# fnothaft/adam

Hardware: AMD Instinct MI355X
Metric: BQSR bases/sec (observe+apply) at 1/2/4/8 MI355X; % HBM roofline (higher is better)
Workload: dtype u8 in, int64 counts, f64 recalibration; 1 GPU; cfg2: synthetic 10M x 100 bp reads, 1 read group, no known sites (per GPU); reads_per_gpu=10000000, bases_per_gpu=1000000000, reads_total=10000000, read_groups=1, known_sites=0, parallelism=dp1: read shards per GPU, RCCL int64 table all-reduce

## Files before the change

### adam_amd/_capi.py

```python
from __future__ import annotations

import ctypes
import os
import threading

_HERE = os.path.dirname(os.path.abspath(__file__))
LIB_PATH = os.environ.get("ADAM_BQSR_LIB") or os.path.join(_HERE, "libadam_bqsr.so")

BQSR_OK = 0
STAGE_RESET, STAGE_KERNEL, STAGE_FOLD, STAGE_PREP, STAGE_LUT, STAGE_NO_LUT = 1, 2, 4, 8, 16, 32
STATUS_NAMES = ["OK", "NULL_RG", "MD_PARSE", "CIGAR_SHORT", "BAD_REVCOMP_BASE", "EMPTY_TABLE", "MISSING_KEY",
                "QUAL_RANGE", "NULL_FIELD", "SEQ_SHORT", "CIGAR_INVALID", "INVALID_ARG", "DEVICE", "UNSUPPORTED",
                "SAM_PARSE", "PILEUP", "ATTRIBUTE"]
(NULL_RG, MD_PARSE, CIGAR_SHORT, BAD_REVCOMP_BASE, EMPTY_TABLE, MISSING_KEY, QUAL_RANGE, NULL_FIELD, SEQ_SHORT,
 CIGAR_INVALID, INVALID_ARG, DEVICE, UNSUPPORTED, SAM_PARSE, PILEUP, ATTRIBUTE) = range(1, 17)
MPILEUP_STATUS_NAMES = ["UNSORTED", "REFERENCE_CONFLICT"]
UNSORTED, REFERENCE_CONFLICT = 17, 18

EXPORTS = [
    "bqsr_abi_version", "bqsr_last_error", "bqsr_last_error_read", "bqsr_status_name", "bqsr_context_create",
    "bqsr_context_destroy", "bqsr_context_tune", "bqsr_sites_create", "bqsr_sites_destroy", "bqsr_batch_create", "bqsr_batch_destroy",
    "bqsr_batch_reads", "bqsr_batch_bases", "bqsr_batch_dims", "bqsr_batch_relayout", "bqsr_batch_layout_times", "bqsr_batch_wrap_device", "bqsr_table_words",
    "bqsr_table_create", "bqsr_table_destroy", "bqsr_table_dims", "bqsr_table_device_ptr", "bqsr_table_download",
    "bqsr_table_upload", "bqsr_observe", "bqsr_observe_records", "bqsr_table_merge", "bqsr_finalize",
    "bqsr_lut_destroy", "bqsr_lut_stats", "bqsr_lut_shifts", "bqsr_apply", "bqsr_apply_records",
    "bqsr_stage_records", "bqsr_staged_destroy", "bqsr_staged_bytes", "bqsr_staged_reads", "bqsr_staged_bases",
    "bqsr_batch_create_staged", "bqsr_batch_upload_async", "bqsr_em_fold_async", "bqsr_batch_em_copy_async",
    "bqsr_finalize_device", "bqsr_observe_stage", "bqsr_apply_stage", "bqsr_job_reset_async", "bqsr_job_result", "bqsr_copy_async",
    "bqsr_job_errors_export_async", "bqsr_job_errors_import_async", "bqsr_job_status_async", "bqsr_job_status_get",
    "bqsr_copy_dyn_async", "bqsr_compact_outputs_async", "bqsr_batch_exception_count_ptr",
    "bqsr_batch_fold_stats",
    "bqsr_sort_order", "bqsr_sam_sort",
    "bqsr_sam_flagstat", "bqsr_flagstat_arrow", "bqsr_flagstat_arrow_device",
    "bqsr_bgzf_inflate", "bqsr_sam_bam_form", "bqsr_sam_markdup_path",
    "bqsr_sam_pileup_prepare", "bqsr_sam_pileup_columns", "bqsr_arrow_pileup_prepare", "bqsr_arrow_pileup_columns",
    "bqsr_pileup_kernel_times",
    "bqsr_sam_mpileup_prepare", "bqsr_sam_mpileup_text", "bqsr_arrow_mpileup_prepare", "bqsr_arrow_mpileup_text",
    "bqsr_mpileup_kernel_times",
    "bqsr_sam_realign_targets_prepare", "bqsr_sam_realign_targets_fetch", "bqsr_arrow_realign_targets_prepare",
    "bqsr_arrow_realign_targets_fetch", "bqsr_realign_targets_kernel_times",
    "bqsr_pileup_agg_create", "bqsr_pileup_agg_destroy", "bqsr_pileup_agg_add_host", "bqsr_sam_pileup_agg_add",
    "bqsr_arrow_pileup_agg_add", "bqsr_pileup_agg_run", "bqsr_pileup_agg_fetch", "bqsr_pileup_agg_kernel_times",
    "bqsr_sam_bam_prepare", "bqsr_sam_bam_records", "bqsr_sam_bam_header", "bqsr_bgzf_compress",
    "bqsr_bam_kernel_times",
    "bqsr_bgzf_deflate", "bqsr_bgzf_deflate_host", "bqsr_sam_bam_members", "bqsr_deflate_code_lengths",
    "bqsr_bgzf_deflate_times",
    "bqsr_compare_create", "bqsr_compare_destroy", "bqsr_compare_check_terms", "bqsr_compare_sam", "bqsr_compare_sides",
    "bqsr_compare_values", "bqsr_compare_baseqs", "bqsr_compare_rows", "bqsr_compare_kernel_times",
    "bqsr_sam_tag_counts", "bqsr_arrow_tag_counts", "bqsr_sam_tag_values", "bqsr_arrow_tag_values",
    "bqsr_tag_values_fetch", "bqsr_tags_kernel_times",
]


class NativeLibraryMissing(RuntimeError):
    pass


class BQSRError(RuntimeError):

    def __init__(self, status: int, message: str = "", read: int = -1):
        names = STATUS_NAMES + MPILEUP_STATUS_NAMES
        name = names[status] if 0 <= status < len(names) else str(status)
        super().__init__("%s: %s" % (name, message))
        self.status = status
        self.name = name
        self.read = read


class Dims(ctypes.Structure):
    _fields_ = [("n_rg", ctypes.c_int32), ("max_len", ctypes.c_int32)]


class FinalStats(ctypes.Structure):
    _fields_ = [("average_reported_error", ctypes.c_double), ("global_error", ctypes.c_double),
                ("global_obs", ctypes.c_int64), ("global_mm", ctypes.c_int64), ("n_groups", ctypes.c_int32)]


class FoldStats(ctypes.Structure):
    _fields_ = [("n_tiles", ctypes.c_int64), ("stream_used", ctypes.c_int64), ("stream_cap", ctypes.c_int64),
                ("lds_stream", ctypes.c_int64), ("n_blocks", ctypes.c_int32), ("reads_per_tile", ctypes.c_int32),
                ("cand_blocks", ctypes.c_int32), ("nobase_blocks", ctypes.c_int32),
                ("nobase_between", ctypes.c_int32), ("tileless_blocks", ctypes.c_int32),
                ("longest_run", ctypes.c_int32), ("capped_blocks", ctypes.c_int32),
                ("segs_total", ctypes.c_int32), ("segs_run", ctypes.c_int32), ("segs_event", ctypes.c_int32),
                ("segs_global", ctypes.c_int32), ("segs_refused", ctypes.c_int32), ("lds_segs", ctypes.c_int32)]


class DeviceReads(ctypes.Structure):
    _fields_ = [("n_reads", ctypes.c_int64), ("n_slots", ctypes.c_int64), ("meta", ctypes.c_void_p),
                ("align", ctypes.c_void_p), ("qual", ctypes.c_void_p), ("bases", ctypes.c_void_p),
                ("cigar", ctypes.c_void_p), ("md", ctypes.c_void_p), ("dims", Dims),
                ("slots_aligned", ctypes.c_int32)]


vp, i32, i64, dbl = ctypes.c_void_p, ctypes.c_int32, ctypes.c_int64, ctypes.c_double
pp, i64p, dblp = ctypes.POINTER(vp), ctypes.POINTER(i64), ctypes.POINTER(dbl)

_lib = None
_lock = threading.Lock()


def lib():
    global _lib
    if _lib is not None:
        return _lib
    with _lock:
        if _lib is not None:
            return _lib
        if not os.path.exists(LIB_PATH):
            raise NativeLibraryMissing("%s is not built; run __graft_entry__.build()" % LIB_PATH)
        try:
            import torch
            if torch.cuda.is_available():
                torch.cuda.init()
        except ImportError:
            pass
        L = ctypes.CDLL(LIB_PATH)
        sig = {
            "bqsr_abi_version": (ctypes.c_int, []),
            "bqsr_last_error": (ctypes.c_char_p, []),
            "bqsr_last_error_read": (i64, []),
            "bqsr_status_name": (ctypes.c_char_p, [ctypes.c_int]),
            "bqsr_context_create": (ctypes.c_int, [ctypes.c_int, pp]),
            "bqsr_context_destroy": (None, [vp]),
            "bqsr_context_tune": (ctypes.c_int, [vp, ctypes.c_int, i64]),
            "bqsr_batch_relayout": (ctypes.c_int, [vp, vp, ctypes.POINTER(dbl)]),
            "bqsr_batch_layout_times": (ctypes.c_int, [vp, ctypes.POINTER(dbl), ctypes.POINTER(dbl)]),
            "bqsr_sites_create": (ctypes.c_int, [vp, vp, vp, vp, i32, pp]),
            "bqsr_sites_destroy": (None, [vp]),
            "bqsr_batch_create": (ctypes.c_int, [vp, vp, vp, pp]),
            "bqsr_batch_destroy": (None, [vp]),
            "bqsr_batch_reads": (i64, [vp]),
            "bqsr_batch_bases": (i64, [vp]),
            "bqsr_batch_slots": (i64, [vp]),
            "bqsr_batch_dims": (Dims, [vp]),
            "bqsr_batch_wrap_device": (ctypes.c_int, [vp, ctypes.POINTER(DeviceReads), pp]),
            "bqsr_stage_records": (ctypes.c_int, [vp, vp, pp]),
            "bqsr_staged_destroy": (None, [vp]),
            "bqsr_staged_bytes": (i64, [vp]),
            "bqsr_staged_reads": (i64, [vp]),
            "bqsr_staged_bases": (i64, [vp]),
            "bqsr_batch_create_staged": (ctypes.c_int, [vp, vp, pp]),
            "bqsr_batch_upload_async": (ctypes.c_int, [vp, vp, vp]),
            "bqsr_batch_set_window": (ctypes.c_int, [vp, i32, i32]),
            "bqsr_batch_reads_per_tile": (i32, [vp]),
            "bqsr_batch_fold_stats": (ctypes.c_int, [vp, ctypes.POINTER(FoldStats), vp]),
            "bqsr_table_words": (i64, [Dims]),
            "bqsr_table_create": (ctypes.c_int, [vp, Dims, vp, pp]),
            "bqsr_table_destroy": (None, [vp]),
            "bqsr_table_dims": (Dims, [vp]),
            "bqsr_table_device_ptr": (vp, [vp]),
            "bqsr_table_download": (ctypes.c_int, [vp, vp]),
            "bqsr_table_upload": (ctypes.c_int, [vp, vp]),
            "bqsr_observe": (ctypes.c_int, [vp, vp, vp, vp, ctypes.POINTER(dbl), vp]),
            "bqsr_observe_async": (ctypes.c_int, [vp, vp, vp, vp, vp]),
            "bqsr_observe_result": (ctypes.c_int, [vp, ctypes.POINTER(dbl), vp]),
            "bqsr_observe_stage": (ctypes.c_int, [vp, vp, vp, vp, i32, vp]),
            "bqsr_table_zero_async": (ctypes.c_int, [vp, vp]),
            "bqsr_batch_em_device_ptr": (vp, [vp]),
            "bqsr_apply_stage": (ctypes.c_int, [vp, vp, vp, vp, vp, vp, vp, i64, i32, vp]),
            "bqsr_observe_records": (ctypes.c_int, [vp, vp, vp, Dims, pp, ctypes.POINTER(dbl)]),
            "bqsr_table_merge": (ctypes.c_int, [vp, vp, ctypes.POINTER(dbl), dbl]),
            "bqsr_finalize": (ctypes.c_int, [vp, vp, dbl, pp]),
            "bqsr_finalize_async": (ctypes.c_int, [vp, vp, dbl, pp, vp]),
            "bqsr_finalize_result": (ctypes.c_int, [vp, vp]),
            "bqsr_finalize_device": (ctypes.c_int, [vp, vp, vp, pp, vp]),
            "bqsr_batch_em_copy_async": (ctypes.c_int, [vp, vp, vp]),
            "bqsr_em_fold_async": (ctypes.c_int, [vp, vp, i64, vp, vp]),
            "bqsr_lut_destroy": (None, [vp]),
            "bqsr_lut_stats": (ctypes.c_int, [vp, ctypes.POINTER(FinalStats)]),
            "bqsr_lut_group": (ctypes.c_int, [vp, i32, ctypes.POINTER(i64), ctypes.POINTER(i64)]),
            "bqsr_lut_shifts": (ctypes.c_int, [vp, i32, i32, i32, i32, vp, ctypes.POINTER(i32)]),
            "bqsr_phred_threshold_table": (i32, [vp, i32, ctypes.POINTER(i32)]),
            "bqsr_apply": (ctypes.c_int, [vp, vp, vp, vp, vp, vp, vp, i64, ctypes.POINTER(i64), vp]),
            "bqsr_apply_async": (ctypes.c_int, [vp, vp, vp, vp, vp, vp, vp, i64, vp]),
            "bqsr_apply_result": (ctypes.c_int, [vp, ctypes.POINTER(i64), vp]),
            "bqsr_apply_records": (ctypes.c_int, [vp, vp, vp, vp, vp]),
            "bqsr_job_reset_async": (ctypes.c_int, [vp, vp, vp]),
            "bqsr_job_result": (ctypes.c_int, [vp, vp, ctypes.POINTER(dbl), ctypes.POINTER(i64), vp]),
            "bqsr_copy_async": (ctypes.c_int, [vp, vp, vp, i64, vp]),
            "bqsr_copy_dyn_async": (ctypes.c_int, [vp, vp, vp, vp, i32, i64, i64, vp]),
            "bqsr_compact_outputs_async": (ctypes.c_int, [vp, vp, vp, vp, vp, vp, i64, vp, vp, vp, vp]),
            "bqsr_batch_exception_count_ptr": (vp, [vp]),
            "bqsr_job_errors_export_async": (ctypes.c_int, [vp, i64, vp, vp]),
            "bqsr_job_errors_import_async": (ctypes.c_int, [vp, vp, vp]),
            "bqsr_job_status_async": (ctypes.c_int, [vp, vp, i32, vp]),
            "bqsr_job_status_get": (ctypes.c_int, [vp, i32, i32, ctypes.POINTER(dbl), ctypes.POINTER(i64)]),
        }
        _lib = bind(L, sig)
    return _lib


def bind(L, sig):
    done = L.__dict__.setdefault("_sig_tables", {})
    if id(sig) not in done:
        for name, (res, args) in sig.items():
            f = getattr(L, name)
            f.restype = res
            f.argtypes = args
        done[id(sig)] = sig
    return L


def check(status: int):
    if status != BQSR_OK:
        L = lib()
        raise BQSRError(status, L.bqsr_last_error().decode(), L.bqsr_last_error_read())


def stage_times(fn, names, handle=None, array=False):
    v = (ctypes.c_double * len(names))()
    lead = [] if handle is None else [handle]
    at = ctypes.addressof(v)
    out = [v] if array else [ctypes.cast(at + 8 * i, ctypes.POINTER(ctypes.c_double)) for i in range(len(names))]
    check(fn(*(lead + out)))
    return dict(zip(names, v))
```

### adam_amd/bqsr.py

```python
from __future__ import annotations

import contextlib
import ctypes
from typing import Dict, Iterable, List, Optional, Sequence, Tuple

import numpy as np

from . import _capi
from ._capi import BQSRError, Dims, check, lib
from .records import (F_DUPLICATE, F_HAS_MD, F_MAPPED, F_PRIMARY, ADAMRecord, RecordBatch)

MAX_REASONABLE_QSCORE = 60


class Context:

    _by_device: Dict[int, "Context"] = {}

    def __init__(self, device: int = 0):
        h = ctypes.c_void_p()
        check(lib().bqsr_context_create(device, ctypes.byref(h)))
        self.handle = h
        self.device = device

    @classmethod
    def get(cls, device: int = 0) -> "Context":
        if device not in cls._by_device:
            cls._by_device[device] = Context(device)
        return cls._by_device[device]

    _KNOBS = {"order": 1, "fronts": 2, "key_major": 3, "bgzf": 5, "flagstat_grid": 6, "pileup_grid": 7}
    _DEFAULTS = {"order": -1, "fronts": -1, "key_major": 0, "bgzf": 1, "flagstat_grid": 0, "pileup_grid": 0}

    def tune(self, **knobs) -> Dict[str, int]:
        cur = getattr(self, "_tuned", dict(self._DEFAULTS))
        prev = {}
        for k, v in knobs.items():
            if v is None:
                continue
            if isinstance(v, str):
                v = {"auto": -1, "read": 0, "group": 1}[v]
            check(lib().bqsr_context_tune(self.handle, self._KNOBS[k], int(v)))
            prev[k] = cur[k]
            cur[k] = int(v)
        self._tuned = cur
        return prev

    @contextlib.contextmanager
    def tuned(self, **knobs):
        prev = self.tune(**knobs)
        try:
            yield self
        finally:
            self.tune(**prev)


class SnpTable:

    def __init__(self, table: Optional[Dict[str, Iterable[int]]] = None):
        self.table = {k: np.unique(np.asarray(list(v), dtype=np.int64)) for k, v in (table or {}).items()}
        self._handles: Dict[int, ctypes.c_void_p] = {}

    @property
    def contigs(self) -> List[str]:
        return list(self.table.keys())

    @staticmethod
    def from_vcf(path: str) -> "SnpTable":
        t: Dict[str, List[int]] = {}
        with open(path, "r", encoding="latin-1") as fh:
            for line in fh:
                line = line.rstrip("\n")
                if line.startswith("#"):
                    continue
                f = line.split("\t")
                t.setdefault(f[0], []).append(int(f[1]))
        return SnpTable(t)

    def handle(self, ctx: Context):
        if ctx.device not in self._handles:
            names = [c.encode() for c in self.contigs]
            arrs = [np.ascontiguousarray(self.table[c]) for c in self.contigs]
            n = len(arrs)
            cnames = (ctypes.c_char_p * max(1, n))(*names)
            cpos = (ctypes.c_void_p * max(1, n))(*[a.ctypes.data for a in arrs])
            cn = np.asarray([len(a) for a in arrs] or [0], dtype=np.uint64)
            h = ctypes.c_void_p()
            check(lib().bqsr_sites_create(ctx.handle, ctypes.cast(cnames, ctypes.c_void_p),
                                          ctypes.cast(cpos, ctypes.c_void_p), cn.ctypes.data, n, ctypes.byref(h)))
            self._handles[ctx.device] = h
        return self._handles[ctx.device]

    def __del__(self):
        L = _capi._lib
        if L is not None:
            for h in getattr(self, "_handles", {}).values():
                L.bqsr_sites_destroy(h)


def dims_of(batches: Sequence[RecordBatch]) -> Dims:
    n_rg = max([b.n_rg() for b in batches] or [1])
    max_len = max([b.max_len() for b in batches] or [1])
    return Dims(n_rg, max_len)


class ErrorCount:

    def __init__(self, bases_observed: int = 0, mismatches: int = 0):
        self.bases_observed = int(bases_observed)
        self.mismatches = int(mismatches)

    def __add__(self, other: "ErrorCount") -> "ErrorCount":
        return ErrorCount(self.bases_observed + other.bases_observed, self.mismatches + other.mismatches)

    def get_error_prob(self) -> Optional[float]:
        if self.bases_observed == 0:
            return None
        return max(10.0 ** (-60 / 10.0), self.mismatches / self.bases_observed)

    def __repr__(self):
        return "ErrorCount(%d, %d)" % (self.bases_observed, self.mismatches)


class RecalTable:

    def __init__(self, dims: Dims, ctx: Optional[Context] = None, expected_mismatch: float = 0.0):
        self.ctx = ctx or Context.get()
        self.dims = Dims(dims.n_rg, dims.max_len)
        h = ctypes.c_void_p()
        check(lib().bqsr_table_create(self.ctx.handle, self.dims, None, ctypes.byref(h)))
        self.handle = h
        self.expected_mismatch = float(expected_mismatch)

    def __del__(self):
        L = _capi._lib
        if L is not None and getattr(self, "handle", None):
            L.bqsr_table_destroy(self.handle)
            self.handle = None

    @property
    def K(self) -> int:
        return 60 * (self.dims.n_rg - 1) + 128

    @property
    def C(self) -> int:
        return 2 * self.dims.max_len + 1

    @property
    def cells(self) -> int:
        return self.C + 21

    def words(self) -> np.ndarray:
        w = np.zeros(lib().bqsr_table_words(self.dims), dtype=np.int64)
        check(lib().bqsr_table_download(self.handle, w.ctypes.data))
        return w

    def set_words(self, w: np.ndarray):
        w = np.ascontiguousarray(w, dtype=np.int64)
        check(lib().bqsr_table_upload(self.handle, w.ctypes.data))

    def counts(self) -> Tuple[np.ndarray, np.ndarray, np.ndarray]:
        w = self.words()
        K, cells = self.K, self.cells
        return w[:K], w[K:K + K * cells].reshape(K, cells), w[K + K * cells:].reshape(K, cells)

    def merge(self, other: "RecalTable") -> "RecalTable":
        out = RecalTable(self.dims, self.ctx)
        out.set_words(self.words())
        em = ctypes.c_double(self.expected_mismatch)
        check(lib().bqsr_table_merge(out.handle, other.handle, ctypes.byref(em), other.expected_mismatch))
        out.expected_mismatch = em.value
        return out

    def merge_into(self, other: "RecalTable"):
        em = ctypes.c_double(self.expected_mismatch)
        check(lib().bqsr_table_merge(self.handle, other.handle, ctypes.byref(em), other.expected_mismatch))
        self.expected_mismatch = em.value

    def finalize_table(self) -> "FinalizedTable":
        return FinalizedTable(self)


class FinalizedTable:

    def __init__(self, table: RecalTable):
        self.table = table
        h = ctypes.c_void_p()
        check(lib().bqsr_finalize(table.ctx.handle, table.handle, table.expected_mismatch, ctypes.byref(h)))
        self.handle = h
        st = _capi.FinalStats()
        check(lib().bqsr_lut_stats(h, ctypes.byref(st)))
        self.average_reported_error = st.average_reported_error
        self.global_error = st.global_error
        self.global_counts = ErrorCount(st.global_obs, st.global_mm)

    def __del__(self):
        L = _capi._lib
        if L is not None and getattr(self, "handle", None):
            L.bqsr_lut_destroy(self.handle)
            self.handle = None

    def read_group_counts(self, r: int) -> Optional[ErrorCount]:
        o, m = ctypes.c_int64(), ctypes.c_int64()
        k = lib().bqsr_lut_group(self.handle, r, ctypes.byref(o), ctypes.byref(m))
        if k < 0:
            check(_capi.DEVICE)
        return ErrorCount(o.value, m.value) if k == 1 else None

    def get_error_rate_shifts(self, qual_by_rg: int, qual: int, cycle: int, context: int):
        sh = np.zeros(4, dtype=np.float64)
        q = ctypes.c_int32()
        check(lib().bqsr_lut_shifts(self.handle, qual_by_rg, qual, cycle, context, sh.ctypes.data, ctypes.byref(q)))
        return sh, q.value

    def get_read_group_delta(self, qual_by_rg: int) -> float:
        num = qual_by_rg - 1
        r = num // MAX_REASONABLE_QSCORE if num >= 0 else -((-num) // MAX_REASONABLE_QSCORE)
        ec = self.read_group_counts(r)
        if ec is None:
            raise BQSRError(_capi.MISSING_KEY, "read group %d" % r)
        p = ec.get_error_prob()
        avg = self.average_reported_error
        return (p if p is not None else avg) - avg


class Partition:

    def __init__(self, batch: RecordBatch, chars: np.ndarray, out_len: np.ndarray):
        self.batch = batch
        self.chars = chars
        self.out_len = out_len

    def qual(self, r: int) -> str:
        o = int(self.batch.qual_offset[r])
        return "".join(map(chr, self.chars[o:o + int(self.out_len[r])]))

    def records(self) -> List[ADAMRecord]:
        recs = self.batch.to_records()
        for r, rec in enumerate(recs):
            if rec.qual is not None or self.out_len[r]:
                rec.qual = self.qual(r)
        return recs


class RecalibrateBaseQualities:

    def __init__(self, ctx: Optional[Context] = None, dims: Optional[Dims] = None):
        self.ctx = ctx or Context.get()
        self.dims = dims

    @staticmethod
    def usable_read(rec: ADAMRecord) -> bool:
        return rec.read_mapped and rec.primary_alignment and not rec.duplicate_read and \
            rec.mismatching_positions is not None

    @classmethod
    def apply(cls, partitions: Sequence[RecordBatch], dbsnp: Optional[SnpTable] = None,
              ctx: Optional[Context] = None) -> List[Partition]:
        parts = list(partitions)
        rbq = cls(ctx, dims_of(parts))
        table = rbq.compute_table(parts, dbsnp or SnpTable())
        return rbq.apply_table(table, parts)

    def _records(self, batch: RecordBatch, dbsnp: Optional[SnpTable]):
        return batch.c_struct(batch.contig_ids_for(dbsnp.contigs if dbsnp else None))

    def compute_table(self, partitions: Sequence[RecordBatch], dbsnp: SnpTable) -> RecalTable:
        dims = self.dims or dims_of(partitions)
        acc = RecalTable(dims, self.ctx)
        sites = dbsnp.handle(self.ctx) if dbsnp is not None else None
        for batch in partitions:
            s, keep = self._records(batch, dbsnp)
            h = ctypes.c_void_p()
            em = ctypes.c_double(0.0)
            check(lib().bqsr_observe_records(self.ctx.handle, ctypes.byref(s), sites, dims, ctypes.byref(h),
                                             ctypes.byref(em)))
            part = RecalTable.__new__(RecalTable)
            part.ctx, part.dims, part.handle, part.expected_mismatch = self.ctx, dims, h, em.value
            acc.merge_into(part)
        return acc

    def apply_table(self, table: RecalTable, partitions: Sequence[RecordBatch]) -> List[Partition]:
        fin = table.finalize_table()
        out = []
        for batch in partitions:
            s, keep = self._records(batch, None)
            chars = np.zeros(max(1, int(batch.qual_offset[-1])), dtype=np.uint16)
            out_len = np.zeros(max(1, batch.n_reads), dtype=np.uint32)
            check(lib().bqsr_apply_records(self.ctx.handle, ctypes.byref(s), fin.handle, chars.ctypes.data,
                                           out_len.ctypes.data))
            out.append(Partition(batch, chars, out_len))
        return out


def adam_bqsr(partitions: Sequence[RecordBatch], dbsnp: Optional[SnpTable] = None,
              ctx: Optional[Context] = None) -> List[Partition]:
    return RecalibrateBaseQualities.apply(partitions, dbsnp, ctx)
```

### adam_amd/csrc/bqsr_capi.cpp

```cpp
#include <hip/hip_runtime.h>

#include <algorithm>
#include <array>
#include <atomic>
#include <chrono>
#include <cmath>
#include <cstdio>
#include <cstdlib>
#include <cstring>
#include <dlfcn.h>
#include <memory>
#include <mutex>
#include <new>
#include <string>
#include <thread>
#include <vector>

#include <rocprim/rocprim.hpp>

#include "bqsr_internal.h"

using namespace bqsr;

#include "bqsr_kernels.hip"
#include "bqsr_observe_lean.hip"
#include "bqsr_fold.hip"
#include "bqsr_transport.hip"


namespace {
thread_local std::string g_err;
thread_local int64_t g_err_read = -1;

bqsr_status fail(bqsr_status s, const std::string& msg, int64_t read = -1) {
  g_err = msg;
  g_err_read = read;
  return s;
}
bqsr_status ok() {
  g_err.clear();
  g_err_read = -1;
  return BQSR_OK;
}

#define HIP_TRY(expr)                                                                          \
  do {                                                                                         \
    hipError_t e_ = (expr);                                                                    \
    if (e_ != hipSuccess)                                                                      \
      return fail(BQSR_ERR_DEVICE, std::string(#expr " failed: ") + hipGetErrorString(e_));    \
  } while (0)

hipStream_t S(void* s) { return s ? (hipStream_t)s : hipStreamPerThread; }

const char* kStatusNames[] = {"OK",          "NULL_RG",      "MD_PARSE",       "CIGAR_SHORT", "BAD_REVCOMP_BASE",
                              "EMPTY_TABLE", "MISSING_KEY",  "QUAL_RANGE",     "NULL_FIELD",  "SEQ_SHORT",
                              "CIGAR_INVALID", "INVALID_ARG", "DEVICE",        "UNSUPPORTED", "SAM_PARSE",
                              "PILEUP",      "ATTRIBUTE",    "UNSORTED",       "REFERENCE_CONFLICT"};

bqsr_status from_err_key(unsigned long long k, int64_t read_base) {
  if (k == kNoError) return ok();
  const int code = (int)(k & 0xF);
  const int64_t read = (int64_t)(k >> 28) + read_base;
  const uint32_t o = (uint32_t)((k >> 8) & 0xFFFFF);
  char buf[160];
  snprintf(buf, sizeof buf, "%s at read %lld, read offset %u", kStatusNames[code], (long long)read, o);
  return fail((bqsr_status)code, buf, read);
}


struct Pow10 {
  double v[256];
  Pow10() {
    for (int p = 0; p < 256; ++p) v[p] = std::pow(10.0, (double)(-p) / 10.0);
  }
};
const Pow10& pow10tab() {
  static Pow10 t;
  return t;
}

double cr_log10(double x) { return (double)log10l((long double)x); }
int32_t java_d2i(double d) {
  if (std::isnan(d)) return 0;
  if (d >= 2147483647.0) return INT32_MAX;
  if (d <= -2147483648.0) return INT32_MIN;
  return (int32_t)d;
}
int32_t phred_of(double p) { return java_d2i(-10.0 * cr_log10(p)); }

struct PhredThresholds {
  std::vector<double> thr;
  PhredThresholds() {
    thr.resize(kThrN);
    const uint64_t lo_bits = 1, hi_bits = 0x7FEFFFFFFFFFFFFFull;
    auto val = [](uint64_t b) {
      double d;
      memcpy(&d, &b, 8);
      return d;
    };
    for (int i = 0; i < kThrN; ++i) {
      const int n = kThrQmin + i;
      if (phred_of(val(hi_bits)) >= n) {
        thr[i] = val(hi_bits);
        continue;
      }
      if (phred_of(val(lo_bits)) < n) {
        thr[i] = 0.0;
        continue;
      }
      uint64_t a = lo_bits, b = hi_bits;
      while (b - a > 1) {
        const uint64_t m = a + (b - a) / 2;
        if (phred_of(val(m)) >= n) a = m; else b = m;
      }
      thr[i] = val(a);
    }
  }
};
const PhredThresholds& thresholds() {
  static PhredThresholds t;
  return t;
}

struct PhredBuckets {
  std::vector<double> thr;
  std::vector<int16_t> q;
  PhredBuckets() {
    thr.resize(kQbN);
    q.resize(kQbN);
    const auto& T = thresholds().thr;
    for (int i = 0; i < kQbN; ++i) {
      const int e = kQbElo + (i >> kQbBits), m = i & ((1 << kQbBits) - 1);
      const double lo = std::ldexp(1.0 + (double)m / (1 << kQbBits), e);
      const double hi = std::ldexp(1.0 + (double)(m + 1) / (1 << kQbBits), e);
      const double last = std::nextafter(hi, 0.0);
      const int qhi = phred_of(lo), qlo = phred_of(last);
      if (qhi - qlo > 1 || qhi - kThrQmin < 0 || qhi - kThrQmin >= kThrN || qhi > 32767 || qhi < -32767) {
        q[(size_t)i] = -32768;
        thr[(size_t)i] = 0.0;
      } else {
        q[(size_t)i] = (int16_t)qhi;
        thr[(size_t)i] = T[(size_t)(qhi - kThrQmin)];
      }
    }
  }
};
const PhredBuckets& buckets() {
  static PhredBuckets b;
  return b;
}

int64_t table_words(const bqsr_dims& d) {
  const int64_t K = 60LL * (d.n_rg - 1) + 128, cells = 2LL * d.max_len + 1 + kCtxSlots;
  return K + 2 * K * cells;
}
TableGeom geom(const bqsr_dims& d) {
  TableGeom g;
  g.K = 60 * (d.n_rg - 1) + 128;
  g.L = d.max_len;
  g.C = 2 * d.max_len + 1;
  g.cells = g.C + kCtxSlots;
  return g;
}

constexpr size_t kLdsMax = 163840;
size_t observe_lds(int qw, int wcells, bool table) {
  return (table ? (size_t)kCtxTabBytes : 0) + (size_t)qw * wcells * 8 + (size_t)qw * 4 + kQBins * 4 +
         (size_t)kMkWords * 4;
}
int64_t piece_bytes(int qw, int cw) { return ((int64_t)qw * cw * kCtxSlots + 15) & ~(int64_t)15; }
size_t apply_lds(int qw, int cw) { return 16 + (size_t)kMkWords * 4 + kCtxTabBytes + (size_t)piece_bytes(qw, cw); }
int lean_orow(int nc, int cw) {
  int o = nc * (cw + kCtxCells);
  while ((o & 3) != 2) ++o;
  return o;
}
size_t lean_lds(int qw, int orow, int wcells) { return ((size_t)qw * (orow + wcells) + qw + kQBins + 1) * 4; }
constexpr int kLeanCopiesMax = 4;
int observe_rows(int wcells, bool table) {
  int qw = kQBins;
  while (qw > 1 && observe_lds(qw, wcells, table) > kLdsMax) --qw;
  return qw;
}
constexpr bool align_slots() { return true; }
int fronts(int n_base, int n_cu, int64_t n_reads, int forced) {
  if (forced == 0) return 0;
  int f = forced;
  if (f < 0) {
    if (n_base > 4 * n_cu) return 0;
    f = (int)std::min<int64_t>((8 * n_cu + n_base - 1) / n_base, n_reads / (8192 * (int64_t)n_base));
    if ((int64_t)std::max(f, 1) * n_base < n_cu) return 0;
    f = std::max(f, 1);
  }
  while (f > 1 && (int64_t)f * n_base > 4096) --f;
  return f;
}
int apply_rows(int cw) {
  int qw = kQBins;
  while (qw > 1 && apply_lds(qw, cw) > kLdsMax) --qw;
  return qw;
}

}


struct bqsr_context {
  int device = 0;
  int n_cu = 256;
  double* d_pow10 = nullptr;
  double* d_thr = nullptr;
  double* d_qbt = nullptr;
  int16_t* d_qbq = nullptr;
  std::mutex stage_mu;
  uint8_t* stage[2] = {nullptr, nullptr};
  hipEvent_t stage_ev[2] = {nullptr, nullptr};
  int tune_order = -1;
  int tune_fronts = -1;
  int tune_keymajor = 0;
  int tune_bgzf = 1;
  int tune_flagstat_grid = 0;
  int tune_pileup_grid = 0;
  std::mutex flagstat_mu;
  unsigned long long* d_flagstat = nullptr;
};

namespace {
constexpr size_t kStageChunk = 64ull << 20;
bqsr_status stage_ring(bqsr_context* ctx) {
  for (int i = 0; i < 2; ++i) {
    if (!ctx->stage[i]) HIP_TRY(hipHostMalloc((void**)&ctx->stage[i], kStageChunk, hipHostMallocDefault));
    if (!ctx->stage_ev[i]) HIP_TRY(hipEventCreateWithFlags(&ctx->stage_ev[i], hipEventDisableTiming));
  }
  return BQSR_OK;
}
bqsr_status upload_staged(bqsr_context* ctx, void* dst, const void* src, size_t n, hipStream_t s) {
  hipPointerAttribute_t attr{};
  const bool pinned = hipPointerGetAttributes(&attr, src) == hipSuccess && attr.type == hipMemoryTypeHost;
  (void)hipGetLastError();
  if (pinned || n < 2 * kStageChunk) {
    HIP_TRY(hipMemcpyAsync(dst, src, n, hipMemcpyHostToDevice, s));
    HIP_TRY(hipStreamSynchronize(s));
    return BQSR_OK;
  }
  std::lock_guard<std::mutex> lock(ctx->stage_mu);
  bqsr_status st = stage_ring(ctx);
  if (st != BQSR_OK) return st;
  const int nth = (int)std::max(1u, std::min(8u, std::thread::hardware_concurrency()));
  const uint8_t* p = (const uint8_t*)src;
  uint8_t* d = (uint8_t*)dst;
  int k = 0;
  for (size_t off = 0; off < n; off += kStageChunk, k ^= 1) {
    const size_t len = std::min(kStageChunk, n - off);
    HIP_TRY(hipEventSynchronize(ctx->stage_ev[k]));
    std::vector<std::thread> th;
    for (int t = 0; t < nth; ++t)
      th.emplace_back([&, t] {
        const size_t a = len * (size_t)t / (size_t)nth, b = len * (size_t)(t + 1) / (size_t)nth;
        memcpy(ctx->stage[k] + a, p + off + a, b - a);
      });
    for (auto& x : th) x.join();
    HIP_TRY(hipMemcpyAsync(d + off, ctx->stage[k], len, hipMemcpyHostToDevice, s));
    HIP_TRY(hipEventRecord(ctx->stage_ev[k], s));
  }
  HIP_TRY(hipStreamSynchronize(s));
  return BQSR_OK;
}
}

struct bqsr_sites {
  bqsr_context* ctx = nullptr;
  std::vector<std::string> names;
  int64_t* pos = nullptr;
  uint64_t* off = nullptr;
  uint32_t* bucket = nullptr;
  uint64_t* bucket_off = nullptr;
  int64_t* bucket_base = nullptr;
  uint64_t* bm = nullptr;
  uint64_t* bm_off = nullptr;
  int64_t* bm_base = nullptr;
  int32_t n = 0;
  int32_t shift = 8;
  SitesDev dev() const { return SitesDev{pos, off, bucket, bucket_off, bucket_base, bm, bm_off, bm_base, n, shift}; }
};

struct bqsr_batch {
  bqsr_context* ctx = nullptr;
  bool owned = false;
  ReadsDev rd{};
  bqsr_dims dims{1, 1};
  int64_t n_slots = 0;
  int64_t n_bases = 0;
  int32_t q_lo = 0, rg_lo = 0;
  bool have_qhist = false;
  int64_t qhist[kQBins] = {0};
  int64_t qhigh = 0;
  std::vector<void*> allocs;
  std::vector<size_t> staged_cnt;
  const bqsr_staged* staged_src = nullptr;
  uint8_t* d_bases2 = nullptr;
  uint64_t* d_bexc = nullptr;
  uint64_t* d_qcodes = nullptr;
  uint8_t* d_qbase = nullptr;
  uint64_t* d_qexc = nullptr;
  ReadInfo* d_info = nullptr;
  uint64_t* d_sbits = nullptr;
  uint32_t* d_work = nullptr;
  int64_t sbits_words = 0;
  bool err_fresh = false;
  bool prepped = false;
  const bqsr_sites* prep_sites = nullptr;
  uint32_t* d_hq = nullptr;
  uint32_t* d_qmask = nullptr;
  bool hq_valid = false;
  FoldParams fold{};
  uint32_t* d_part = nullptr;
  size_t part_words = 0;
  uint8_t* d_chars = nullptr;
  const bqsr_lut* chars_lut = nullptr;
  uint64_t* d_off64 = nullptr;
  int64_t off64_n = -1;
  size_t chars_bytes = 0;
  unsigned long long* d_err = nullptr;
  double* d_em = nullptr;
  int32_t n_blocks = 0;
  bool bucketed = false;
  int32_t n_keys = 1;
  int32_t n_base = 1;
  int32_t fronts = 0;
  uint32_t* d_perm = nullptr;
  int64_t* d_key_off = nullptr;
  uint32_t* d_key_cnt = nullptr;
  uint32_t* d_cursor = nullptr;
  uint8_t *k_qual = nullptr, *k_bases = nullptr;
  uint64_t* d_kslot = nullptr;
  uint64_t* d_kspan = nullptr;
  void* d_ktemp = nullptr;
  size_t ktemp_bytes = 0;
  bool km_ready = false;
  double km_alloc_ms = -1.0, km_build_ms = -1.0;
  bool perm_static = false;
  OrderDev order() const {
    return bucketed ? OrderDev{d_perm, d_key_off, n_keys, fronts > 0 ? n_base : 0, km_ready ? d_kslot : nullptr}
                    : OrderDev{nullptr, nullptr, 1};
  }
  ReadsDev pass_rd() const {
    ReadsDev r = rd;
    if (bucketed && km_ready) {
      r.qual = k_qual;
      r.bases = k_bases;
    }
    return r;
  }
  int32_t pass_blocks() const { return bucketed && fronts > 0 ? n_keys : n_blocks; }
  uint64_t* h_status = nullptr;
  hipStream_t side = nullptr;
  hipEvent_t ev_obs = nullptr, ev_fold = nullptr;
  bool obs_pending = false;
  ~bqsr_batch() {
    if (side) (void)hipStreamDestroy(side);
    for (hipEvent_t e : {ev_obs, ev_fold})
      if (e) (void)hipEventDestroy(e);
    if (d_part) (void)hipFree(d_part);
    if (d_off64) (void)hipFree(d_off64);
    if (d_chars) (void)hipFree(d_chars);
    if (h_status) (void)hipHostFree(h_status);
    for (void* p : allocs) (void)hipFree(p);
  }
};

struct bqsr_table {
  bqsr_context* ctx = nullptr;
  bqsr_dims dims{1, 1};
  int64_t* words = nullptr;
  bool owned = false;
  ~bqsr_table() {
    if (owned && words) (void)hipFree(words);
  }
  TableGeom g() const { return geom(dims); }
  int64_t* touched() const { return words; }
  int64_t* obs() const { return words + g().K; }
  int64_t* mm() const { return words + g().K + (int64_t)g().K * g().cells; }
};

struct bqsr_lut {
  bqsr_context* ctx = nullptr;
  bqsr_dims dims{1, 1};
  int32_t n_groups = 0;
  std::vector<void*> allocs;
  int64_t *qk_obs = nullptr, *qk_mm = nullptr, *grp_obs = nullptr, *grp_mm = nullptr;
  uint8_t *grp_ok = nullptr, *key_ok = nullptr, *rq_ok = nullptr;
  double *a2 = nullptr, *s1 = nullptr, *d2 = nullptr;
  FinalOut* d_out = nullptr;
  FinalOut out{};
  bool out_pending = false;
  bool host_ready = false;
  std::vector<int64_t> h_words, h_qk_obs, h_qk_mm, h_grp_obs, h_grp_mm;
  std::vector<uint8_t> h_grp_ok;
  const bqsr_table* src = nullptr;
  ~bqsr_lut() {
    for (void* p : allocs) (void)hipFree(p);
  }
};

namespace {
template <class T>
bqsr_status dalloc(std::vector<void*>& v, T** p, size_t n) {
  void* q = nullptr;
  HIP_TRY(hipMalloc(&q, std::max<size_t>(n, 1) * sizeof(T)));
  v.push_back(q);
  *p = (T*)q;
  return BQSR_OK;
}
}


extern "C" {

int bqsr_abi_version(void) { return BQSR_ABI_VERSION; }
const char* bqsr_last_error(void) { return g_err.c_str(); }
int64_t bqsr_last_error_read(void) { return g_err_read; }
const char* bqsr_status_name(bqsr_status s) {
  if ((int)s < 0 || (int)s > 18) return "UNKNOWN";
  return kStatusNames[(int)s];
}

bqsr_status bqsr_context_tune(bqsr_context* ctx, int knob, int64_t value) {
  if (!ctx) return fail(BQSR_ERR_INVALID_ARG, "bqsr_context_tune: null context");
  switch (knob) {
    case BQSR_TUNE_ORDER:
      if (value < -1 || value > 1) break;
      ctx->tune_order = (int)value;
      return BQSR_OK;
    case BQSR_TUNE_FRONTS:
      if (value < -1 || value > 4096) break;
      ctx->tune_fronts = (int)value;
      return BQSR_OK;
    case BQSR_TUNE_KEYMAJOR:
      if (value < 0 || value > 1) break;
      ctx->tune_keymajor = (int)value;
      return BQSR_OK;
    case BQSR_TUNE_FUSED_PREP:
      if (value != 0) break;
      return BQSR_OK;
    case BQSR_TUNE_BGZF:
      if (value < 0 || value > 1) break;
      ctx->tune_bgzf = (int)value;
      return BQSR_OK;
    case BQSR_TUNE_FLAGSTAT_GRID:
      if (value < 0 || value > (1 << 20)) break;
      ctx->tune_flagstat_grid = (int)value;
      return BQSR_OK;
    case BQSR_TUNE_PILEUP_GRID:
      if (value < 0 || value > (1 << 20)) break;
      ctx->tune_pileup_grid = (int)value;
      return BQSR_OK;
    default:
      return fail(BQSR_ERR_INVALID_ARG, "bqsr_context_tune: unknown knob");
  }
  return fail(BQSR_ERR_INVALID_ARG, "bqsr_context_tune: value out of range");
}

bqsr_status bqsr_context_create(int device, bqsr_context** out) {
  if (!out) return fail(BQSR_ERR_INVALID_ARG, "null out");
  HIP_TRY(hipSetDevice(device));
  hipDeviceProp_t prop;
  HIP_TRY(hipGetDeviceProperties(&prop, device));
  bqsr_context* c = new bqsr_context;
  c->device = device;
  c->n_cu = prop.multiProcessorCount;
  hipError_t e = hipMalloc(&c->d_pow10, 256 * sizeof(double));
  if (e == hipSuccess) e = hipMalloc(&c->d_thr, kThrN * sizeof(double));
  if (e == hipSuccess) e = hipMemcpy(c->d_pow10, pow10tab().v, 256 * sizeof(double), hipMemcpyHostToDevice);
  if (e == hipSuccess) e = hipMemcpy(c->d_thr, thresholds().thr.data(), kThrN * sizeof(double), hipMemcpyHostToDevice);
  if (e == hipSuccess) e = hipMalloc(&c->d_qbt, kQbN * sizeof(double));
  if (e == hipSuccess) e = hipMalloc(&c->d_qbq, kQbN * sizeof(int16_t));
  if (e == hipSuccess) e = hipMemcpy(c->d_qbt, buckets().thr.data(), kQbN * sizeof(double), hipMemcpyHostToDevice);
  if (e == hipSuccess) e = hipMemcpy(c->d_qbq, buckets().q.data(), kQbN * sizeof(int16_t), hipMemcpyHostToDevice);
  for (const void* f : {(const void*)bqsr_apply_kernel, (const void*)bqsr_observe_chunks,
                        (const void*)bqsr_observe_lean<true, false>, (const void*)bqsr_observe_lean<true, true>})
    if (e == hipSuccess) e = hipFuncSetAttribute(f, hipFuncAttributeMaxDynamicSharedMemorySize, (int)kLdsMax);
  if (e == hipSuccess)
    e = hipFuncSetAttribute((const void*)bqsr_fold_hist, hipFuncAttributeMaxDynamicSharedMemorySize, (int)fold_hist_lds());
  if (e == hipSuccess)
    e = hipFuncSetAttribute((const void*)bqsr_fold_chain, hipFuncAttributeMaxDynamicSharedMemorySize,
                            (int)chain_lds(kMaxFoldBlocks));
  if (e != hipSuccess) {
    bqsr_context_destroy(c);
    return fail(BQSR_ERR_DEVICE, std::string("context: ") + hipGetErrorString(e));
  }
  *out = c;
  return ok();
}

void bqsr_context_destroy(bqsr_context* c) {
  if (!c) return;
  if (c->d_pow10) (void)hipFree(c->d_pow10);
  if (c->d_thr) (void)hipFree(c->d_thr);
  if (c->d_qbt) (void)hipFree(c->d_qbt);
  if (c->d_qbq) (void)hipFree(c->d_qbq);
  if (c->d_flagstat) (void)hipFree(c->d_flagstat);
  for (int i = 0; i < 2; ++i) {
    if (c->stage[i]) (void)hipHostFree(c->stage[i]);
    if (c->stage_ev[i]) (void)hipEventDestroy(c->stage_ev[i]);
  }
  delete c;
}


bqsr_status bqsr_sites_create(bqsr_context* ctx, const char* const* contigs, const int64_t* const* pos,
                              const uint64_t* n, int32_t n_contigs, bqsr_sites** out) {
  if (!ctx || !out || n_contigs < 0 || (n_contigs > 0 && (!contigs || !pos || !n)))
    return fail(BQSR_ERR_INVALID_ARG, "bqsr_sites_create: bad arguments");
  HIP_TRY(hipSetDevice(ctx->device));
  bqsr_sites* s = new bqsr_sites;
  s->ctx = ctx;
  s->n = n_contigs;
  std::vector<int64_t> all;
  std::vector<uint64_t> off(1, 0);
  std::vector<uint32_t> bucket;
  std::vector<uint64_t> boff(1, 0);
  std::vector<int64_t> bbase;
  std::vector<uint64_t> bm, bmoff(1, 0);
  std::vector<int64_t> bmbase;
  for (int32_t c = 0; c < n_contigs; ++c) {
    s->names.emplace_back(contigs[c] ? contigs[c] : "");
    std::vector<int64_t> v(pos[c], pos[c] + n[c]);
    std::sort(v.begin(), v.end());
    v.erase(std::unique(v.begin(), v.end()), v.end());
    const int64_t base = v.empty() ? 0 : v.front();
    const int64_t nb = v.empty() ? 0 : ((v.back() - base) >> s->shift) + 1;
    size_t j = 0;
    for (int64_t b = 0; b < nb; ++b) {
      const int64_t lo = base + (b << s->shift);
      while (j < v.size() && v[j] < lo) ++j;
      bucket.push_back((uint32_t)j);
    }
    bbase.push_back(base);
    boff.push_back(bucket.size());
    const int64_t b0 = v.empty() ? 0 : (int64_t)((uint64_t)base & ~(uint64_t)63);
    const int64_t nw = v.empty() ? 0 : ((v.back() - b0) >> 6) + 1;
    const bool dense = nw > 0 && nw <= 64 * (int64_t)v.size() + 64 && nw <= (int64_t(1) << 28);
    if (dense) {
      const size_t w0 = bm.size();
      bm.resize(w0 + (size_t)nw, 0ull);
      for (const int64_t p : v) bm[w0 + (size_t)((p - b0) >> 6)] |= 1ull << ((p - b0) & 63);
    }
    bmbase.push_back(dense ? b0 : 0);
    bmoff.push_back(bm.size());
    all.insert(all.end(), v.begin(), v.end());
    off.push_back(all.size());
  }
  std::vector<void*> keep;
  auto up = [&](auto** dst, const auto& src) -> hipError_t {
    using T = typename std::remove_reference<decltype(src[0])>::type;
    hipError_t e = hipMalloc((void**)dst, std::max<size_t>(src.size(), 1) * sizeof(T));
    if (e != hipSuccess) return e;
    if (!src.empty()) e = hipMemcpy(*dst, src.data(), src.size() * sizeof(T), hipMemcpyHostToDevice);
    return e;
  };
  hipError_t e = up(&s->pos, all);
  if (e == hipSuccess) e = up(&s->off, off);
  if (e == hipSuccess) e = up(&s->bucket, bucket);
  if (e == hipSuccess) e = up(&s->bucket_off, boff);
  if (e == hipSuccess) e = up(&s->bucket_base, bbase);
  if (e == hipSuccess) e = up(&s->bm, bm);
  if (e == hipSuccess) e = up(&s->bm_off, bmoff);
  if (e == hipSuccess) e = up(&s->bm_base, bmbase);
  if (e != hipSuccess) {
    bqsr_sites_destroy(s);
    return fail(BQSR_ERR_DEVICE, std::string("sites upload: ") + hipGetErrorString(e));
  }
  *out = s;
  return ok();
}

void bqsr_sites_destroy(bqsr_sites* s) {
  if (!s) return;
  for (void* p : {(void*)s->pos, (void*)s->off, (void*)s->bucket, (void*)s->bucket_off, (void*)s->bucket_base,
                  (void*)s->bm, (void*)s->bm_off, (void*)s->bm_base})
    if (p) (void)hipFree(p);
  delete s;
}


namespace {

inline uint8_t code_of(uint8_t c) {
  switch (c) {
    case 'A': return kCodeA;
    case 'C': return kCodeC;
    case 'G': return kCodeG;
    case 'T': return kCodeT;
    case 'N': return kCodeN;
    default: return kCodeOther;
  }
}

Window window_rows(const bqsr_batch* b, int max_rows);

bqsr_status finish_batch(bqsr_batch* b, int64_t max_slot_len) {
  if (max_slot_len > kMaxReadLen)
    return fail(BQSR_ERR_UNSUPPORTED, "reads longer than " + std::to_string(kMaxReadLen) + " bases are not supported");
  const int64_t n = b->rd.n_reads;
  b->rd.reads_per_tile = (int32_t)std::max<int64_t>(1, std::min<int64_t>(kMaxTileReads, kTileSlots / std::max<int64_t>(1, max_slot_len)));
  b->rd.n_tiles = (n + b->rd.reads_per_tile - 1) / b->rd.reads_per_tile;
  b->n_blocks = std::min(b->ctx->n_cu, kMaxFoldBlocks);
  bqsr_status st;
  if ((st = dalloc(b->allocs, &b->d_hq, (size_t)b->n_blocks * kQBins)) != BQSR_OK) return st;
  if ((st = dalloc(b->allocs, &b->d_qmask, 4)) != BQSR_OK) return st;
  {
    FoldParams& F = b->fold;
    const size_t nt = (size_t)std::max<int64_t>(1, b->rd.n_tiles), nbk = (size_t)b->n_blocks;
    F.stream_cap = std::max<int64_t>(1 << 20, std::min<int64_t>(16 << 20, b->rd.n_slots));
    if ((st = dalloc(b->allocs, &F.blk, nbk)) != BQSR_OK || (st = dalloc(b->allocs, &F.cand_list, nbk)) != BQSR_OK ||
        (st = dalloc(b->allocs, &F.n_cand, 1)) != BQSR_OK || (st = dalloc(b->allocs, &F.delta, 1)) != BQSR_OK ||
        (st = dalloc(b->allocs, &F.rtile, nt)) != BQSR_OK || (st = dalloc(b->allocs, &F.ntile, nt)) != BQSR_OK ||
        (st = dalloc(b->allocs, &F.dtile, nt * kSegBinades)) != BQSR_OK ||
        (st = dalloc(b->allocs, &F.seg, nbk * kFoldMaxSegs)) != BQSR_OK ||
        (st = dalloc(b->allocs, &F.seg_base, nbk)) != BQSR_OK || (st = dalloc(b->allocs, &F.nseg, nbk)) != BQSR_OK ||
        (st = dalloc(b->allocs, &F.seg_used, 1)) != BQSR_OK ||
        (st = dalloc(b->allocs, &F.streams, (size_t)F.stream_cap + 64)) != BQSR_OK ||
        (st = dalloc(b->allocs, &F.csum, (size_t)F.stream_cap / 64 * 2 + 2)) != BQSR_OK ||
        (st = dalloc(b->allocs, &F.stream_used, 1)) != BQSR_OK)
      return st;
  }
  if ((st = dalloc(b->allocs, &b->d_err, kErrWords)) != BQSR_OK) return st;
  if ((st = dalloc(b->allocs, &b->d_info, (size_t)std::max<int64_t>(1, n))) != BQSR_OK) return st;
  b->sbits_words = b->rd.slots_aligned ? (b->rd.n_slots / 16 + 8 + 1) / 2 : b->rd.n_slots / 32 + 5;
  if ((st = dalloc(b->allocs, &b->d_sbits, (size_t)b->sbits_words)) != BQSR_OK) return st;
  if ((st = dalloc(b->allocs, &b->d_em, 2)) != BQSR_OK) return st;
  if ((st = dalloc(b->allocs, &b->d_work,
                   (size_t)(n + kPrepChunk) + (size_t)std::max<int64_t>(n / kPrepChunk + 1, kMaxFoldBlocks))) != BQSR_OK)
    return st;
  if (b->ctx->tune_order >= 0) {
    b->bucketed = b->ctx->tune_order == 1;
  } else {
    b->bucketed = b->dims.n_rg > 1;
    if (!b->bucketed && b->have_qhist) {
      const int cw = geom(b->dims).C;
      const Window w = window_rows(b, apply_rows(cw));
      int64_t in = 0, all = 0;
      for (int q = 0; q < kQBins; ++q) {
        all += b->qhist[q];
        if (q >= w.q_lo && q < w.q_lo + w.qw) in += b->qhist[q];
      }
      b->bucketed = (double)(all - in) > 1e-3 * (double)all;
    }
  }
  if (b->bucketed) {
    b->n_base = 2 * std::max<int32_t>(1, b->dims.n_rg);
    b->fronts = fronts(b->n_base, b->ctx->n_cu, n, b->ctx->tune_fronts);
    b->n_keys = b->n_base * std::max(1, b->fronts);
    if ((st = dalloc(b->allocs, &b->d_perm, (size_t)std::max<int64_t>(1, n))) != BQSR_OK) return st;
    if ((st = dalloc(b->allocs, &b->d_key_off, (size_t)b->n_keys + 1)) != BQSR_OK) return st;
    if ((st = dalloc(b->allocs, &b->d_key_cnt, (size_t)b->n_keys)) != BQSR_OK) return st;
    if ((st = dalloc(b->allocs, &b->d_cursor, (size_t)b->n_keys)) != BQSR_OK) return st;
  }
  return BQSR_OK;
}

bool layout_wanted(const bqsr_batch* b) { return b->bucketed && b->rd.slots_aligned && b->rd.n_reads > 0; }
bool key_major_wanted(const bqsr_batch* b) { return layout_wanted(b) && b->ctx->tune_keymajor; }
bqsr_status key_major_alloc(bqsr_batch* b) {
  if (b->k_qual) return BQSR_OK;
  const int64_t n = b->rd.n_reads;
  bqsr_status st;
  size_t tb = 0;
  HIP_TRY(rocprim::exclusive_scan(nullptr, tb, (const uint64_t*)nullptr, (uint64_t*)nullptr, (uint64_t)0, (size_t)n + 1,
                                  rocprim::plus<uint64_t>(), (hipStream_t)0));
  b->ktemp_bytes = std::max<size_t>(tb, 1);
  if ((st = dalloc(b->allocs, &b->d_kslot, (size_t)(n + 1))) != BQSR_OK ||
      (st = dalloc(b->allocs, &b->d_kspan, (size_t)(n + 1))) != BQSR_OK ||
      (st = dalloc(b->allocs, (uint8_t**)&b->d_ktemp, b->ktemp_bytes)) != BQSR_OK ||
      (st = dalloc(b->allocs, &b->k_qual, (size_t)b->rd.n_slots + kColumnPad)) != BQSR_OK ||
      (st = dalloc(b->allocs, &b->k_bases, (size_t)b->rd.n_slots / 2 + 1 + kColumnPad)) != BQSR_OK)
    return st;
  return BQSR_OK;
}
void launch_key_sort(bqsr_batch* b, uint64_t* span, hipStream_t s) {
  const int64_t n = b->rd.n_reads;
  const int n_cu = b->ctx->n_cu;
  (void)hipMemsetAsync(b->d_key_cnt, 0, (size_t)b->n_keys * 4, s);
  const unsigned cb = (unsigned)std::min<int64_t>((n + 255) / 256, (int64_t)n_cu * 4);
  hipLaunchKernelGGL(bqsr_key_count, dim3(cb), dim3(256), 0, s, (const ReadMeta*)b->rd.meta, n, b->n_keys, b->n_base,
                     std::max(1, b->fronts), b->d_key_cnt);
  hipLaunchKernelGGL(bqsr_key_scan, dim3(1), dim3(1024), 0, s, (const uint32_t*)b->d_key_cnt, b->n_keys, b->d_key_off,
                     b->d_cursor);
  const unsigned sb = (unsigned)std::min<int64_t>((n + 4095) / 4096, (int64_t)n_cu * 8);
  hipLaunchKernelGGL(bqsr_key_scatter, dim3(sb), dim3(256), 0, s, (const ReadMeta*)b->rd.meta, n, b->n_keys, b->n_base,
                     std::max(1, b->fronts), b->d_cursor, b->d_perm, span);
}
bqsr_status layout_build(bqsr_batch* b, hipStream_t s) {
  if (!layout_wanted(b)) return BQSR_OK;
  const int64_t n = b->rd.n_reads;
  bqsr_context* ctx = b->ctx;
  const bool km = key_major_wanted(b);
  b->km_ready = false;
  const auto t0 = std::chrono::steady_clock::now();
  bqsr_status st = km ? key_major_alloc(b) : BQSR_OK;
  if (st != BQSR_OK) return st;
  const auto t1 = std::chrono::steady_clock::now();
  if (km) HIP_TRY(hipMemsetAsync(b->d_kspan + n, 0, 8, s));
  launch_key_sort(b, km ? b->d_kspan : nullptr, s);
  HIP_TRY(hipGetLastError());
  if (km) {
    size_t tb = b->ktemp_bytes;
    HIP_TRY(rocprim::exclusive_scan(b->d_ktemp, tb, b->d_kspan, b->d_kslot, (uint64_t)0, (size_t)n + 1,
                                    rocprim::plus<uint64_t>(), s));
    HIP_TRY(hipMemsetAsync(b->k_qual + b->rd.n_slots, 0, kColumnPad, s));
    HIP_TRY(hipMemsetAsync(b->k_bases + b->rd.n_slots / 2, 0, 1 + kColumnPad, s));
    const unsigned gw = (unsigned)std::min<int64_t>((n + 16 * kKmPer - 1) / (16 * kKmPer), (int64_t)ctx->n_cu * 64 / kKmPer);
    hipLaunchKernelGGL(bqsr_km_gather, dim3(gw), dim3(256), 0, s, b->rd, (const uint32_t*)b->d_perm,
                       (const uint64_t*)b->d_kslot, b->k_qual, b->k_bases);
    HIP_TRY(hipGetLastError());
  }
  HIP_TRY(hipStreamSynchronize(s));
  const auto t2 = std::chrono::steady_clock::now();
  b->km_alloc_ms = std::chrono::duration<double, std::milli>(t1 - t0).count();
  b->km_build_ms = std::chrono::duration<double, std::milli>(t2 - t1).count();
  b->km_ready = km;
  b->perm_static = true;
  return BQSR_OK;
}

struct Packed {
  std::vector<ReadMeta> meta;
  std::vector<ReadAlign> align;
  std::vector<uint8_t> qual, bases, md;
  std::vector<uint32_t> cigar;
  int64_t n_slots = 0, n_bases = 0, max_slot = 0;
  int32_t n_rg = 1, max_len = 1;
  int64_t qhist[256] = {0};
  std::vector<int64_t> rghist;
};

bqsr_status pack(const bqsr_records* R, Packed& P) {
  const int64_t n = R->n_reads;
  P.meta.resize((size_t)n);
  P.align.resize((size_t)n);
  uint64_t slot = 0, md_tot = 0, cig_tot = 0;
  for (int64_t r = 0; r < n; ++r) {
    const uint32_t f = R->flags[r];
    const uint64_t lq = (f & BQSR_F_HAS_QUAL) ? R->qual_offset[r + 1] - R->qual_offset[r] : 0;
    const uint64_t ls = (f & BQSR_F_HAS_SEQ) ? R->seq_offset[r + 1] - R->seq_offset[r] : 0;
    const uint64_t nmd = (f & BQSR_F_HAS_MD) ? R->md_offset[r + 1] - R->md_offset[r] : 0;
    const uint64_t ncig = (f & BQSR_F_HAS_CIGAR) ? R->cigar_offset[r + 1] - R->cigar_offset[r] : 0;
    if (lq > 65535 || ls > 65535 || nmd > 65535 || ncig > 65535)
      return fail(BQSR_ERR_UNSUPPORTED, "read field longer than 65535", r);
    if ((f & BQSR_F_HAS_RG) && (R->rg_id[r] < 0 || R->rg_id[r] > 65535))
      return fail(BQSR_ERR_UNSUPPORTED, "recordGroupId outside [0, 65535]", r);
    ReadMeta& m = P.meta[(size_t)r];
    m.slot = slot;
    m.lq = (uint16_t)lq;
    m.ls = (uint16_t)ls;
    m.flags = (uint16_t)(f & 0x7FFF);
    m.rg = (f & BQSR_F_HAS_RG) ? (uint16_t)R->rg_id[r] : 0;
    ReadAlign& a = P.align[(size_t)r];
    a.start = R->start[r];
    a.cigar_off = (uint32_t)cig_tot;
    a.md_off = (uint32_t)md_tot;
    a.contig = R->contig_id[r];
    a.n_cigar = (uint16_t)ncig;
    a.md_len = (uint16_t)nmd;
    const uint64_t sl = align_slots() ? slot_span(lq, ls) : std::max(lq, ls);
    slot += sl;
    P.max_slot = std::max<int64_t>(P.max_slot, (int64_t)sl);
    md_tot += nmd;
    cig_tot += ncig;
    P.n_bases += (int64_t)(R->seq_offset[r + 1] - R->seq_offset[r]);
    if (f & BQSR_F_HAS_RG) P.n_rg = std::max<int32_t>(P.n_rg, R->rg_id[r] + 1);
    P.max_len = std::max<int32_t>(P.max_len, (int32_t)ls);
  }
  if (md_tot > 0xFFFFFFFFull || cig_tot > 0xFFFFFFFFull)
    return fail(BQSR_ERR_UNSUPPORTED, "partition MD / CIGAR columns exceed 4 GiB");
  P.n_slots = (int64_t)slot;
  P.qual.assign((size_t)slot + kColumnPad, 0);
  P.bases.assign((size_t)slot / 2 + 1 + kColumnPad, 0);
  P.md.resize(md_tot + kColumnPad);
  P.cigar.resize(cig_tot + kColumnPad / 4);
  P.rghist.assign((size_t)P.n_rg, 0);
  const int nth = (int)std::max<int64_t>(1, std::min<int64_t>(16, n / 65536));
// ... 262 lines not shown
  if ((st = dalloc(b->allocs, &meta, S_->cnt[0])) != BQSR_OK || (st = dalloc(b->allocs, &align, S_->cnt[1])) != BQSR_OK ||
      (st = dalloc(b->allocs, &qual, S_->cnt[2])) != BQSR_OK || (st = dalloc(b->allocs, &bases, S_->cnt[3])) != BQSR_OK ||
      (st = dalloc(b->allocs, &md, S_->cnt[4])) != BQSR_OK || (st = dalloc(b->allocs, &cigar, S_->cnt[5])) != BQSR_OK)
    return st;
  b->rd.meta = meta;
  b->rd.align = align;
  b->rd.qual = qual;
  b->rd.bases = bases;
  b->rd.md = md;
  b->rd.cigar = cigar;
  b->rd.slots_aligned = align_slots();
  if ((st = dalloc(b->allocs, &b->d_bases2, S_->cnt[6] + 16)) != BQSR_OK ||
      (st = dalloc(b->allocs, &b->d_bexc, std::max<size_t>(S_->cnt[7], 1))) != BQSR_OK ||
      (st = dalloc(b->allocs, &b->d_qcodes, std::max<size_t>(S_->cnt[8], 1))) != BQSR_OK ||
      (st = dalloc(b->allocs, &b->d_qbase, std::max<size_t>(S_->cnt[9], 1))) != BQSR_OK ||
      (st = dalloc(b->allocs, &b->d_qexc, std::max<size_t>(S_->cnt[10], 1))) != BQSR_OK)
    return st;
  if ((st = finish_batch(b.get(), S_->max_slot)) != BQSR_OK) return st;
  b->staged_cnt.assign(S_->cnt, S_->cnt + kStagedCols);
  b->staged_src = S_;
  *out = b.release();
  return ok();
}

bqsr_status bqsr_batch_upload_async(bqsr_batch* b, const bqsr_staged* S_, void* stream) {
  if (!b || !S_) return fail(BQSR_ERR_INVALID_ARG, "bqsr_batch_upload_async: bad arguments");
  if (b->staged_src != S_ || b->staged_cnt.size() != kStagedCols ||
      !std::equal(b->staged_cnt.begin(), b->staged_cnt.end(), S_->cnt) || b->rd.n_reads != S_->n_reads)
    return fail(BQSR_ERR_INVALID_ARG, "bqsr_batch_upload_async: batch was not created from this staged partition");
  HIP_TRY(hipSetDevice(b->ctx->device));
  void* dst[kStagedCols] = {(void*)b->rd.meta,  (void*)b->rd.align,  nullptr,           nullptr,
                            (void*)b->rd.md,    (void*)b->rd.cigar,  (void*)b->d_bases2, (void*)b->d_bexc,
                            (void*)b->d_qcodes, (void*)b->d_qbase,   (void*)b->d_qexc};
  const size_t esz[kStagedCols] = {sizeof(ReadMeta), sizeof(ReadAlign), 1, 1, 1, sizeof(uint32_t), 1, 8, 8, 1, 8};
  hipStream_t s = S(stream);
  for (int i = 0; i < kStagedCols; ++i)
    if (S_->cnt[i] && dst[i])
      HIP_TRY(hipMemcpyAsync(dst[i], S_->host + S_->off[i], S_->cnt[i] * esz[i], hipMemcpyHostToDevice, s));
  const int64_t nw = (int64_t)(S_->cnt[3] + 7) / 8;
  const unsigned g = (unsigned)std::min<int64_t>(std::max<int64_t>(1, (nw + 255) / 256), (int64_t)b->ctx->n_cu * 16);
  hipLaunchKernelGGL(bqsr_bases_expand, dim3(g), dim3(256), 0, s, (const uint32_t*)b->d_bases2, (int64_t)S_->cnt[3],
                     (uint8_t*)b->rd.bases);
  if (S_->cnt[7]) {
    const unsigned ge = (unsigned)std::min<int64_t>(((int64_t)S_->cnt[7] + 255) / 256, (int64_t)b->ctx->n_cu * 16);
    hipLaunchKernelGGL(bqsr_bases_exceptions, dim3(ge), dim3(256), 0, s, (const uint64_t*)b->d_bexc,
                       (int64_t)S_->cnt[7], (uint8_t*)b->rd.bases);
  }
  const int64_t n16 = (int64_t)S_->cnt[8];
  if (n16) {
    const unsigned gq = (unsigned)std::min<int64_t>((n16 + 255) / 256, (int64_t)b->ctx->n_cu * 16);
    hipLaunchKernelGGL(bqsr_quals_expand, dim3(gq), dim3(256), 0, s, (const uint64_t*)b->d_qcodes,
                       (const uint8_t*)b->d_qbase, n16, (int64_t)S_->cnt[2], (uint8_t*)b->rd.qual);
  }
  if (S_->cnt[10]) {
    const unsigned ge = (unsigned)std::min<int64_t>(((int64_t)S_->cnt[10] + 255) / 256, (int64_t)b->ctx->n_cu * 16);
    hipLaunchKernelGGL(bqsr_quals_exceptions, dim3(ge), dim3(256), 0, s, (const uint64_t*)b->d_qexc,
                       (int64_t)S_->cnt[10], (uint8_t*)b->rd.qual);
  }
  HIP_TRY(hipGetLastError());
  b->prepped = false;
  return ok();
}

bqsr_status bqsr_batch_wrap_device(bqsr_context* ctx, const bqsr_device_reads* dev, bqsr_batch** out) {
  if (!ctx || !dev || !out || dev->n_reads < 0 || dev->dims.n_rg < 1 || dev->dims.max_len < 1)
    return fail(BQSR_ERR_INVALID_ARG, "bqsr_batch_wrap_device: bad arguments");
  if (dev->dims.max_len > kMaxReadLen)
    return fail(BQSR_ERR_UNSUPPORTED, "reads longer than " + std::to_string(kMaxReadLen) + " bases are not supported");
  HIP_TRY(hipSetDevice(ctx->device));
  bqsr_batch* b = new bqsr_batch;
  b->ctx = ctx;
  b->rd.n_reads = dev->n_reads;
  b->rd.meta = (const ReadMeta*)dev->meta;
  b->rd.align = (const ReadAlign*)dev->align;
  b->rd.qual = dev->qual;
  b->rd.bases = dev->bases;
  b->rd.cigar = dev->cigar;
  b->rd.md = dev->md;
  b->n_slots = dev->n_slots;
  b->rd.n_slots = dev->n_slots;
  b->n_bases = -1;
  b->dims = dev->dims;
  b->q_lo = 0;
  b->rg_lo = 0;
  b->rd.slots_aligned = dev->slots_aligned != 0;
  bqsr_status st = finish_batch(b, b->rd.slots_aligned ? (int64_t)slot_span(0, (uint64_t)dev->dims.max_len)
                                                       : (int64_t)dev->dims.max_len);
  if (st != BQSR_OK) {
    delete b;
    return st;
  }
  *out = b;
  return ok();
}

void bqsr_batch_destroy(bqsr_batch* b) { delete b; }
int64_t bqsr_batch_reads(const bqsr_batch* b) { return b ? b->rd.n_reads : -1; }
int64_t bqsr_batch_bases(const bqsr_batch* b) { return b ? b->n_bases : -1; }
int64_t bqsr_batch_slots(const bqsr_batch* b) { return b ? b->n_slots : -1; }
bqsr_dims bqsr_batch_dims(const bqsr_batch* b) { return b ? b->dims : bqsr_dims{0, 0}; }

bqsr_status bqsr_batch_relayout(bqsr_batch* b, void* stream, double* ms) {
  if (!b) return fail(BQSR_ERR_INVALID_ARG, "bqsr_batch_relayout: null batch");
  hipStream_t s = (hipStream_t)stream;
  HIP_TRY(hipStreamSynchronize(s));
  const auto t0 = std::chrono::steady_clock::now();
  const bool has = b->perm_static;
  if (has) {
    b->perm_static = false;
    bqsr_status st = layout_build(b, s);
    if (st != BQSR_OK) return st;
  }
  HIP_TRY(hipStreamSynchronize(s));
  if (ms) *ms = has ? std::chrono::duration<double, std::milli>(std::chrono::steady_clock::now() - t0).count() : -1.0;
  return ok();
}

bqsr_status bqsr_batch_layout_times(const bqsr_batch* b, double* alloc_ms, double* build_ms) {
  if (!b) return fail(BQSR_ERR_INVALID_ARG, "bqsr_batch_layout_times: null batch");
  if (alloc_ms) *alloc_ms = b->km_alloc_ms;
  if (build_ms) *build_ms = b->km_build_ms;
  return ok();
}

bqsr_status bqsr_batch_set_window(bqsr_batch* b, int32_t q_lo, int32_t rg_lo) {
  if (!b || q_lo < 0 || q_lo >= kQBins || rg_lo < 0) return fail(BQSR_ERR_INVALID_ARG, "bad window");
  b->q_lo = q_lo;
  b->rg_lo = rg_lo;
  b->have_qhist = false;
  return ok();
}
int32_t bqsr_batch_reads_per_tile(const bqsr_batch* b) { return b ? b->rd.reads_per_tile : -1; }

bqsr_status bqsr_batch_fold_stats(bqsr_batch* b, bqsr_fold_stats* out, void* stream) {
  if (!b || !out) return fail(BQSR_ERR_INVALID_ARG, "bqsr_batch_fold_stats: null argument");
  if (!b->hq_valid) return fail(BQSR_ERR_INVALID_ARG, "bqsr_batch_fold_stats: no fold has run on this batch");
  HIP_TRY(hipSetDevice(b->ctx->device));
  hipStream_t s = S(stream);
  HIP_TRY(hipStreamSynchronize(s));
  const FoldParams& F = b->fold;
  const int nb = b->n_blocks;
  int32_t n_cand = 0;
  uint32_t seg_used = 0;
  unsigned long long stream_used = 0;
  std::vector<FoldBlock> blk((size_t)nb);
  HIP_TRY(hipMemcpy(&n_cand, F.n_cand, sizeof n_cand, hipMemcpyDeviceToHost));
  HIP_TRY(hipMemcpy(&seg_used, F.seg_used, sizeof seg_used, hipMemcpyDeviceToHost));
  HIP_TRY(hipMemcpy(&stream_used, F.stream_used, sizeof stream_used, hipMemcpyDeviceToHost));
  HIP_TRY(hipMemcpy(blk.data(), F.blk, blk.size() * sizeof(FoldBlock), hipMemcpyDeviceToHost));
  if (n_cand < 0 || n_cand > nb || (size_t)seg_used > (size_t)nb * kFoldMaxSegs)
    return fail(BQSR_ERR_DEVICE, "bqsr_batch_fold_stats: the fold's counters are out of range");
  std::vector<int32_t> nseg((size_t)n_cand), seg_base((size_t)n_cand);
  std::vector<FoldSeg> seg((size_t)seg_used);
  if (n_cand) {
    HIP_TRY(hipMemcpy(nseg.data(), F.nseg, nseg.size() * sizeof(int32_t), hipMemcpyDeviceToHost));
    HIP_TRY(hipMemcpy(seg_base.data(), F.seg_base, seg_base.size() * sizeof(int32_t), hipMemcpyDeviceToHost));
  }
  if (seg_used) HIP_TRY(hipMemcpy(seg.data(), F.seg, seg.size() * sizeof(FoldSeg), hipMemcpyDeviceToHost));
  bqsr_fold_stats st{};
  st.n_tiles = b->rd.n_tiles;
  st.stream_used = (int64_t)stream_used;
  st.stream_cap = F.stream_cap;
  st.lds_stream = kChainLdsStream;
  st.lds_segs = kChainLdsSegs;
  st.n_blocks = nb;
  st.reads_per_tile = b->rd.reads_per_tile;
  int first_live = nb, last_live = -1;
  for (int i = 0; i < nb; ++i) {
    const FoldBlock& B = blk[(size_t)i];
    const bool nobase = B.cidx < 0 && B.e == kFoldNoBase;
    if (B.cidx >= 0) ++st.cand_blocks;
    if (nobase) ++st.nobase_blocks;
    else {
      first_live = std::min(first_live, i);
      last_live = i;
      if (B.cidx < 0) st.longest_run = std::max(st.longest_run, -B.cidx);
    }
    if (b->rd.n_tiles * i / nb == b->rd.n_tiles * (i + 1) / nb) ++st.tileless_blocks;
  }
  for (int i = first_live + 1; i < last_live; ++i)
    if (blk[(size_t)i].cidx < 0 && blk[(size_t)i].e == kFoldNoBase) ++st.nobase_between;
  for (int c = 0; c < n_cand; ++c) {
    const int32_t ns = nseg[(size_t)c], s0 = seg_base[(size_t)c];
    if (ns < 0 || ns > kFoldMaxSegs || s0 < 0 || (int64_t)s0 + ns > (int64_t)seg_used)
      return fail(BQSR_ERR_DEVICE, "bqsr_batch_fold_stats: a segment list is out of range");
    if (ns == kFoldMaxSegs) ++st.capped_blocks;
    st.segs_total += ns;
    for (int32_t i = s0; i < s0 + ns; ++i) {
      const FoldSeg& G = seg[(size_t)i];
      if (G.kind == kSegRun) ++st.segs_run;
      else if (G.kind == kSegEvent) ++st.segs_event;
      else {
        ++st.segs_global;
        if (G.off < 0) ++st.segs_refused;
      }
    }
  }
  *out = st;
  return ok();
}


int64_t bqsr_table_words(bqsr_dims d) { return (d.n_rg < 1 || d.max_len < 1) ? -1 : table_words(d); }

bqsr_status bqsr_table_create(bqsr_context* ctx, bqsr_dims d, void* device_words, bqsr_table** out) {
  if (!ctx || !out || d.n_rg < 1 || d.max_len < 1 || d.max_len > 65535)
    return fail(BQSR_ERR_INVALID_ARG, "bqsr_table_create: bad arguments");
  HIP_TRY(hipSetDevice(ctx->device));
  bqsr_table* t = new bqsr_table;
  t->ctx = ctx;
  t->dims = d;
  const size_t bytes = (size_t)table_words(d) * 8;
  if (device_words) {
    t->words = (int64_t*)device_words;
  } else {
    hipError_t e = hipMalloc((void**)&t->words, bytes);
    if (e != hipSuccess) {
      delete t;
      return fail(BQSR_ERR_DEVICE, hipGetErrorString(e));
    }
    t->owned = true;
  }
  hipError_t e = hipMemset(t->words, 0, bytes);
  if (e != hipSuccess) {
    delete t;
    return fail(BQSR_ERR_DEVICE, hipGetErrorString(e));
  }
  *out = t;
  return ok();
}
void bqsr_table_destroy(bqsr_table* t) { delete t; }
bqsr_dims bqsr_table_dims(const bqsr_table* t) { return t ? t->dims : bqsr_dims{0, 0}; }
void* bqsr_table_device_ptr(bqsr_table* t) { return t ? t->words : nullptr; }

bqsr_status bqsr_table_download(const bqsr_table* t, int64_t* host) {
  if (!t || !host) return fail(BQSR_ERR_INVALID_ARG, "null");
  HIP_TRY(hipSetDevice(t->ctx->device));
  HIP_TRY(hipMemcpy(host, t->words, (size_t)table_words(t->dims) * 8, hipMemcpyDeviceToHost));
  return ok();
}
bqsr_status bqsr_table_upload(bqsr_table* t, const int64_t* host) {
  if (!t || !host) return fail(BQSR_ERR_INVALID_ARG, "null");
  HIP_TRY(hipSetDevice(t->ctx->device));
  HIP_TRY(hipMemcpy(t->words, host, (size_t)table_words(t->dims) * 8, hipMemcpyHostToDevice));
  return ok();
}

bqsr_status bqsr_table_merge(bqsr_table* acc, const bqsr_table* part, double* acc_em, double part_em) {
  if (!acc || !part || !acc_em) return fail(BQSR_ERR_INVALID_ARG, "null");
  if (acc->dims.n_rg != part->dims.n_rg || acc->dims.max_len != part->dims.max_len)
    return fail(BQSR_ERR_INVALID_ARG, "table dims differ");
  HIP_TRY(hipSetDevice(acc->ctx->device));
  const int64_t n = table_words(acc->dims);
  hipLaunchKernelGGL(bqsr_table_add, dim3((unsigned)std::min<int64_t>(4096, (n + 255) / 256)), dim3(256), 0,
                     hipStreamPerThread, acc->words, part->words, n);
  HIP_TRY(hipGetLastError());
  HIP_TRY(hipStreamSynchronize(hipStreamPerThread));
  *acc_em = *acc_em + part_em;
  return ok();
}


namespace {
Window window_rows(const bqsr_batch* b, int max_rows) {
  Window w{max_rows, std::min(b->q_lo, kQBins - 1), b->rg_lo};
  if (!b->have_qhist) {
    w.qw = std::min(w.qw, kQBins - w.q_lo);
    return w;
  }
  int lo = 0, hi = kQBins - 1;
  while (lo < kQBins - 1 && b->qhist[lo] == 0) ++lo;
  while (hi > lo && b->qhist[hi] == 0) --hi;
  if (hi - lo + 1 <= max_rows) {
    w.q_lo = lo;
    w.qw = hi - lo + 1;
  } else {
    w.q_lo = best_q_lo(b->qhist, max_rows);
  }
  w.qw = std::min(w.qw, kQBins - w.q_lo);
  return w;
}
int window_cw(const bqsr_batch* b, const TableGeom& g) { return b->bucketed ? g.L : g.C; }
int qual_span(const bqsr_batch* b) {
  if (!b->have_qhist) return kQBins;
  int lo = 0, hi = kQBins - 1;
  while (lo < kQBins - 1 && b->qhist[lo] == 0) ++lo;
  while (hi > lo && b->qhist[hi] == 0) --hi;
  return hi - lo + 1;
}
int lane_shift(const bqsr_batch* b) {
  const int c = (b->dims.max_len + kSuper - 1) / kSuper;
  int s = 0;
  while ((1 << s) < c && s < 6) ++s;
  return s;
}
bqsr_status check_dims(const bqsr_batch* b, const bqsr_table* t) {
  if (b->dims.n_rg > t->dims.n_rg || b->dims.max_len > t->dims.max_len)
    return fail(BQSR_ERR_INVALID_ARG, "table dims smaller than the batch's (n_rg / max_len)");
  return BQSR_OK;
}
}

namespace {
bqsr_status launch_prep(bqsr_context* ctx, bqsr_batch* b, const bqsr_sites* sites, hipStream_t s) {
  if (!b->err_fresh) HIP_TRY(hipMemsetAsync(b->d_err + kErrAppPrep, 0xFF, 8, s));
  b->err_fresh = false;
  b->hq_valid = false;
  if (b->rd.n_reads > 0) {
    PrepParams P{};
    P.rd = b->rd;
    if (sites) P.sites = sites->dev();
    const bool w32 = b->rd.slots_aligned;
    const bool store = w32 && b->dims.max_len <= 128 && P.sites.n_contigs > 0;
    P.info = b->d_info;
    P.sbits = b->d_sbits;
    P.err = b->d_err;
    P.work = b->d_work;
    P.n_work = b->d_work + b->rd.n_reads + kPrepChunk;
    const int64_t blocks = (b->rd.n_reads + kPrepChunk - 1) / kPrepChunk;
    if (store) {
      hipLaunchKernelGGL(bqsr_prep_kernel<kPrepStore>, dim3((unsigned)blocks), dim3(kPrepThreads), 0, s, P);
      hipLaunchKernelGGL(bqsr_prep_complex, dim3((unsigned)blocks), dim3(kComplexThreads), 0, s, P);
    } else if (w32) {
      hipLaunchKernelGGL(bqsr_prep_kernel<kPrepW32>, dim3((unsigned)blocks), dim3(kPrepThreads), 0, s, P);
    } else {
      hipLaunchKernelGGL(bqsr_prep_kernel<kPrepU64>, dim3((unsigned)blocks), dim3(kPrepThreads), 0, s, P);
    }
    HIP_TRY(hipGetLastError());
    if (b->bucketed && !b->perm_static) {
      launch_key_sort(b, nullptr, s);
      HIP_TRY(hipGetLastError());
    }
  }
  b->prepped = true;
  b->prep_sites = sites;
  return BQSR_OK;
}
}

bqsr_status bqsr_observe_stage(bqsr_context* ctx, bqsr_batch* b, const bqsr_sites* sites, bqsr_table* t,
                               int32_t stages, void* stream) {
  if (!ctx || !b || !t) return fail(BQSR_ERR_INVALID_ARG, "null");
  bqsr_status st = check_dims(b, t);
  if (st != BQSR_OK) return st;
  HIP_TRY(hipSetDevice(ctx->device));
  hipStream_t s = S(stream);
  if (stages & BQSR_STAGE_RESET) HIP_TRY(hipMemsetAsync(b->d_err + kErrObs, 0xFF, 8, s));
  if (stages & BQSR_STAGE_PREP) {
    if ((st = launch_prep(ctx, b, sites, s)) != BQSR_OK) return st;
  }
  if (b->rd.n_reads == 0) {
    if (stages & BQSR_STAGE_FOLD) HIP_TRY(hipMemsetAsync(b->d_em, 0, 8, s));
    return ok();
  }
  if ((stages & BQSR_STAGE_KERNEL) && (!b->prepped || b->prep_sites != sites))
    return fail(BQSR_ERR_INVALID_ARG, "observe kernel before the prep stage (or with other known sites)");
  if (stages & BQSR_STAGE_KERNEL) {
    ObserveParams P{};
    P.rd = b->pass_rd();
    P.ord = b->order();
    P.info = b->d_info;
    P.sbits = b->d_sbits;
    P.g = geom(t->dims);
    const bool lean = !b->bucketed;
    P.wcells = window_cw(b, P.g) + (lean ? kCtxCells : kCtxSlots);
    while ((P.wcells & 3) != 2) ++P.wcells;
    if (lean) {
      const int cw = window_cw(b, P.g), span = qual_span(b);
      int best_rows = 0;
      for (int nc = kLeanCopiesMax; nc >= 1 && best_rows < span; --nc) {
        const int orow = lean_orow(nc, cw);
        int qw = kQBins;
        while (qw > 1 && lean_lds(qw, orow, P.wcells) > kLdsMax) --qw;
        if (qw > best_rows) {
          best_rows = qw;
          P.nc = nc;
          P.orow = orow;
        }
      }
      P.w = window_rows(b, best_rows);
      P.rows_all = b->have_qhist && b->qhigh == 0;
      for (int q = 0; q < kQBins && P.rows_all; ++q)
        if (b->qhist[q] && (q < P.w.q_lo || q >= P.w.q_lo + P.w.qw)) P.rows_all = 0;
    } else {
      P.w = window_rows(b, observe_rows(P.wcells, true));
    }
    P.touched = t->touched();
    P.obs = t->obs();
    P.mm = t->mm();
    P.part_stride = 2 * P.w.qw * P.wcells + P.w.qw;
    if (!lean) {
      if (!b->side) {
        HIP_TRY(hipStreamCreateWithFlags(&b->side, hipStreamNonBlocking));
        HIP_TRY(hipEventCreateWithFlags(&b->ev_obs, hipEventDisableTiming));
        HIP_TRY(hipEventCreateWithFlags(&b->ev_fold, hipEventDisableTiming));
      }
      HIP_TRY(hipEventRecord(b->ev_obs, s));
      b->obs_pending = true;
    }
    const size_t need = (size_t)P.part_stride * (b->pass_blocks() + b->n_keys - 1);
    if (b->part_words < need) {
      if (b->d_part) {
        HIP_TRY(hipStreamSynchronize(s));
        (void)hipFree(b->d_part);
        b->d_part = nullptr;
        b->part_words = 0;
      }
      HIP_TRY(hipMalloc((void**)&b->d_part, need * sizeof(uint32_t)));
      b->part_words = need;
    }
    P.part = b->d_part;
    P.hq_block = b->d_hq;
    P.err = b->d_err + kErrObs;
    P.n_blocks = lean ? b->n_blocks : b->pass_blocks();
    const size_t lds = lean ? lean_lds(P.w.qw, P.orow, P.wcells) : observe_lds(P.w.qw, P.wcells, true);
    if (lean) {
      if (P.rd.slots_aligned)
        hipLaunchKernelGGL((bqsr_observe_lean<true, true>), dim3(P.n_blocks), dim3(kBlockThreads), lds, s, P);
      else
        hipLaunchKernelGGL((bqsr_observe_lean<true, false>), dim3(P.n_blocks), dim3(kBlockThreads), lds, s, P);
    } else {
      hipLaunchKernelGGL(bqsr_observe_chunks, dim3(P.n_blocks), dim3(kBlockThreads), lds, s, P);
    }
    HIP_TRY(hipGetLastError());
    const int rb = (int)std::min<int64_t>(4096, ((int64_t)P.part_stride * (b->bucketed ? b->n_base : 1) + 255) / 256);
    const unsigned ry = b->bucketed ? 1u : (unsigned)((b->n_blocks + kRedSlabs - 1) / kRedSlabs);
    hipLaunchKernelGGL(bqsr_window_reduce, dim3(rb, ry), dim3(256), 0, s, (const uint32_t*)b->d_part, b->rd, P.ord,
                       P.n_blocks, P.part_stride, P.wcells, P.w, P.g, P.touched, P.obs, P.mm, lean ? kCtxJunk : 0);
    HIP_TRY(hipGetLastError());
  }
  if (stages & BQSR_STAGE_FOLD) {
    const hipStream_t caller = s;
    const bool fork = b->obs_pending;
    if (fork) {
      HIP_TRY(hipStreamWaitEvent(b->side, b->ev_obs, 0));
      s = b->side;
      b->obs_pending = false;
    }
    if (b->bucketed) {
      HIP_TRY(hipMemsetAsync(b->d_hq, 0, (size_t)b->n_blocks * kQBins * 4, s));
      hipLaunchKernelGGL(bqsr_fold_hist, dim3(b->n_blocks * kFhSplit), dim3(kFhWaves * 64), fold_hist_lds(), s, b->rd, (const ReadInfo*)b->d_info,
                         b->n_blocks, lane_shift(b), b->d_hq);
      HIP_TRY(hipGetLastError());
    }
    FoldParams F = b->fold;
    F.rd = b->rd;
    F.info = b->d_info;
    F.hq_block = b->d_hq;
    F.pow10 = ctx->d_pow10;
    F.n_blocks = b->n_blocks;
    F.em_out = b->d_em;
    F.qmask = b->d_qmask;
    hipLaunchKernelGGL(bqsr_fold_plan, dim3(1), dim3(1024), 0, s, F);
    const int64_t max_tpb = (b->rd.n_tiles + b->n_blocks - 1) / b->n_blocks + 1;
    hipLaunchKernelGGL(bqsr_fold_tiles, dim3(ctx->n_cu * 4), dim3(kFtWaves * 64), 0, s, F, max_tpb);
    hipLaunchKernelGGL(bqsr_fold_segs, dim3(b->n_blocks), dim3(kSegThreads), 0, s, F);
    hipLaunchKernelGGL(bqsr_fold_chain, dim3(1), dim3(1024), chain_lds(b->n_blocks), s, F);
    HIP_TRY(hipGetLastError());
    b->hq_valid = true;
    if (fork) {
      HIP_TRY(hipEventRecord(b->ev_fold, s));
      HIP_TRY(hipStreamWaitEvent(caller, b->ev_fold, 0));
    }
  }
  return ok();
}

bqsr_status bqsr_observe_async(bqsr_context* ctx, bqsr_batch* b, const bqsr_sites* sites, bqsr_table* t, void* stream) {
  return bqsr_observe_stage(ctx, b, sites, t, BQSR_STAGE_RESET | BQSR_STAGE_PREP | BQSR_STAGE_KERNEL | BQSR_STAGE_FOLD,
                            stream);
}

bqsr_status bqsr_table_zero_async(bqsr_table* t, void* stream) {
  if (!t) return fail(BQSR_ERR_INVALID_ARG, "null");
  HIP_TRY(hipSetDevice(t->ctx->device));
  HIP_TRY(hipMemsetAsync(t->words, 0, (size_t)table_words(t->dims) * 8, S(stream)));
  return ok();
}

void* bqsr_batch_em_device_ptr(bqsr_batch* b) { return b ? (void*)b->d_em : nullptr; }

bqsr_status bqsr_observe_result(bqsr_batch* b, double* em, void* stream) {
  HIP_TRY(hipSetDevice(b->ctx->device));
  hipStream_t s = S(stream);
  unsigned long long err = 0;
  double e = 0;
  HIP_TRY(hipMemcpyAsync(&err, b->d_err + kErrObs, 8, hipMemcpyDeviceToHost, s));
  HIP_TRY(hipMemcpyAsync(&e, b->d_em, 8, hipMemcpyDeviceToHost, s));
  HIP_TRY(hipStreamSynchronize(s));
  if (em) *em = e;
  return from_err_key(err, 0);
}

bqsr_status bqsr_observe(bqsr_context* ctx, bqsr_batch* b, const bqsr_sites* sites, bqsr_table* t,
                         double* expected_mismatch, void* stream) {
  bqsr_status st = bqsr_observe_async(ctx, b, sites, t, stream);
  if (st != BQSR_OK) return st;
  return bqsr_observe_result(b, expected_mismatch, stream);
}

bqsr_status bqsr_observe_records(bqsr_context* ctx, const bqsr_records* recs, const bqsr_sites* sites, bqsr_dims dims,
                                 bqsr_table** out_partial, double* out_em) {
  if (!out_partial || !out_em) return fail(BQSR_ERR_INVALID_ARG, "null out");
  bqsr_batch* b = nullptr;
  bqsr_status st = bqsr_batch_create(ctx, recs, nullptr, &b);
  if (st != BQSR_OK) return st;
  bqsr_table* t = nullptr;
  st = bqsr_table_create(ctx, dims, nullptr, &t);
  if (st == BQSR_OK) st = bqsr_observe(ctx, b, sites, t, out_em, nullptr);
  bqsr_batch_destroy(b);
  if (st != BQSR_OK) {
    bqsr_table_destroy(t);
    return st;
  }
  *out_partial = t;
  return ok();
}


namespace {
bqsr_status finalize_impl(bqsr_context* ctx, const bqsr_table* t, double em, const double* em_dev, bqsr_lut** out,
                          void* stream) {
  if (!ctx || !t || !out) return fail(BQSR_ERR_INVALID_ARG, "null");
  HIP_TRY(hipSetDevice(ctx->device));
  hipStream_t s = S(stream);
  const TableGeom g = geom(t->dims);
  const int n_rg = t->dims.n_rg;
  bqsr_lut* L = *out;
  const bool reuse = L && L->ctx == ctx && L->dims.n_rg == t->dims.n_rg && L->dims.max_len == t->dims.max_len;
  if (L && !reuse) {
    (void)hipStreamSynchronize(s);
    delete L;
    *out = nullptr;
  }
  if (!reuse) L = new bqsr_lut;
  L->ctx = ctx;
  L->dims = t->dims;
  L->src = t;
  L->host_ready = false;
  L->n_groups = (g.K - 1) / kMaxQ + 2;
  bqsr_status st;
  if (!reuse && ((st = dalloc(L->allocs, &L->qk_obs, g.K)) != BQSR_OK || (st = dalloc(L->allocs, &L->qk_mm, g.K)) != BQSR_OK ||
      (st = dalloc(L->allocs, &L->grp_obs, L->n_groups)) != BQSR_OK ||
      (st = dalloc(L->allocs, &L->grp_mm, L->n_groups)) != BQSR_OK ||
      (st = dalloc(L->allocs, &L->grp_ok, L->n_groups)) != BQSR_OK || (st = dalloc(L->allocs, &L->key_ok, g.K)) != BQSR_OK ||
      (st = dalloc(L->allocs, &L->rq_ok, (size_t)n_rg * kQBins)) != BQSR_OK ||
      (st = dalloc(L->allocs, &L->a2, (size_t)n_rg * kQBins)) != BQSR_OK ||
      (st = dalloc(L->allocs, &L->s1, (size_t)n_rg * kQBins * g.C)) != BQSR_OK ||
      (st = dalloc(L->allocs, &L->d2, (size_t)n_rg * kQBins * kCtxSlots)) != BQSR_OK ||
      (st = dalloc(L->allocs, &L->d_out, 1)) != BQSR_OK)) {
    delete L;
    return st;
  }
  hipLaunchKernelGGL(bqsr_final_keys, dim3((g.K + 3) / 4), dim3(256), 0, s, t->touched(), t->obs(), t->mm(), g, L->qk_obs,
                     L->qk_mm);
  hipLaunchKernelGGL(bqsr_final_groups, dim3(1), dim3(256), 0, s, t->touched(), L->qk_obs, L->qk_mm, g, n_rg, em,
                     em_dev, ctx->d_pow10, L->n_groups, L->grp_obs, L->grp_mm, L->grp_ok, L->key_ok, L->a2, L->rq_ok, L->d_out);
  const int64_t ncell = (int64_t)n_rg * kQBins * (g.C + kCtxSlots);
  hipLaunchKernelGGL(bqsr_final_tables, dim3((unsigned)std::min<int64_t>(8192, (ncell + 255) / 256)), dim3(256), 0, s,
                     t->obs(), t->mm(), g, n_rg, L->a2, L->rq_ok, pow10tab().v[kMaxQ], L->s1, L->d2);
  hipError_t e = hipGetLastError();
  L->out_pending = em_dev != nullptr;
  if (e == hipSuccess && !em_dev) e = hipMemcpyAsync(&L->out, L->d_out, sizeof(FinalOut), hipMemcpyDeviceToHost, s);
  if (e != hipSuccess) {
    if (!reuse) delete L;
    return fail(BQSR_ERR_DEVICE, hipGetErrorString(e));
  }
  *out = L;
  return ok();
}
}

bqsr_status bqsr_finalize_async(bqsr_context* ctx, const bqsr_table* t, double em, bqsr_lut** out, void* stream) {
  return finalize_impl(ctx, t, em, nullptr, out, stream);
}

bqsr_status bqsr_finalize_device(bqsr_context* ctx, const bqsr_table* t, const double* em_device, bqsr_lut** out,
                                 void* stream) {
  if (!em_device) return fail(BQSR_ERR_INVALID_ARG, "null em_device");
  return finalize_impl(ctx, t, 0.0, em_device, out, stream);
}

bqsr_status bqsr_em_fold_async(bqsr_context* ctx, const double* ems, int64_t n, double* out, void* stream) {
  if (!ctx || !out || n < 0 || (n > 0 && !ems)) return fail(BQSR_ERR_INVALID_ARG, "bqsr_em_fold_async: bad arguments");
  HIP_TRY(hipSetDevice(ctx->device));
  hipLaunchKernelGGL(bqsr_em_fold, dim3(1), dim3(64), 0, S(stream), ems, n, out);
  HIP_TRY(hipGetLastError());
  return ok();
}

bqsr_status bqsr_batch_em_copy_async(bqsr_batch* b, double* dst, void* stream) {
  if (!b || !dst) return fail(BQSR_ERR_INVALID_ARG, "null");
  HIP_TRY(hipSetDevice(b->ctx->device));
  HIP_TRY(hipMemcpyAsync(dst, b->d_em, sizeof(double), hipMemcpyDeviceToDevice, S(stream)));
  return ok();
}

bqsr_status bqsr_finalize_result(bqsr_lut* L, void* stream) {
  HIP_TRY(hipSetDevice(L->ctx->device));
  HIP_TRY(hipStreamSynchronize(S(stream)));
  if (L->out_pending) {
    HIP_TRY(hipMemcpy(&L->out, L->d_out, sizeof(FinalOut), hipMemcpyDeviceToHost));
    L->out_pending = false;
  }
  if (!L->out.any_key)
    return fail(BQSR_ERR_EMPTY_TABLE, "empty.reduceLeft: no usable base was observed");
  return ok();
}

bqsr_status bqsr_finalize(bqsr_context* ctx, const bqsr_table* t, double em, bqsr_lut** out) {
  if (!out) return fail(BQSR_ERR_INVALID_ARG, "null out");
  bqsr_lut* L = nullptr;
  bqsr_status st = bqsr_finalize_async(ctx, t, em, &L, nullptr);
  if (st != BQSR_OK) return st;
  st = bqsr_finalize_result(L, nullptr);
  if (st != BQSR_OK) {
    delete L;
    return st;
  }
  *out = L;
  return ok();
}

void bqsr_lut_destroy(bqsr_lut* l) { delete l; }

namespace {
bqsr_status lut_host(bqsr_lut* L) {
  if (L->host_ready) return BQSR_OK;
  HIP_TRY(hipSetDevice(L->ctx->device));
  if (L->out_pending) {
    HIP_TRY(hipDeviceSynchronize());
    HIP_TRY(hipMemcpy(&L->out, L->d_out, sizeof(FinalOut), hipMemcpyDeviceToHost));
    L->out_pending = false;
  }
  const TableGeom g = geom(L->dims);
  L->h_words.resize((size_t)table_words(L->dims));
  L->h_qk_obs.resize((size_t)g.K);
  L->h_qk_mm.resize((size_t)g.K);
  L->h_grp_obs.resize((size_t)L->n_groups);
  L->h_grp_mm.resize((size_t)L->n_groups);
  L->h_grp_ok.resize((size_t)L->n_groups);
  HIP_TRY(hipMemcpy(L->h_words.data(), L->src->words, L->h_words.size() * 8, hipMemcpyDeviceToHost));
  HIP_TRY(hipMemcpy(L->h_qk_obs.data(), L->qk_obs, (size_t)g.K * 8, hipMemcpyDeviceToHost));
  HIP_TRY(hipMemcpy(L->h_qk_mm.data(), L->qk_mm, (size_t)g.K * 8, hipMemcpyDeviceToHost));
  HIP_TRY(hipMemcpy(L->h_grp_obs.data(), L->grp_obs, (size_t)L->n_groups * 8, hipMemcpyDeviceToHost));
  HIP_TRY(hipMemcpy(L->h_grp_mm.data(), L->grp_mm, (size_t)L->n_groups * 8, hipMemcpyDeviceToHost));
  HIP_TRY(hipMemcpy(L->h_grp_ok.data(), L->grp_ok, (size_t)L->n_groups, hipMemcpyDeviceToHost));
  L->host_ready = true;
  return BQSR_OK;
}
bool eprob(int64_t obs, int64_t mm, double* v) {
  if (obs == 0) return false;
  const double x = (double)mm / (double)obs;
  *v = std::max(pow10tab().v[kMaxQ], x);
  return true;
}
}

bqsr_status bqsr_lut_stats(const bqsr_lut* lc, bqsr_final_stats* out) {
  bqsr_lut* L = const_cast<bqsr_lut*>(lc);
  if (!L || !out) return fail(BQSR_ERR_INVALID_ARG, "null");
  if (L->out_pending) {
    HIP_TRY(hipDeviceSynchronize());
    HIP_TRY(hipMemcpy(&L->out, L->d_out, sizeof(FinalOut), hipMemcpyDeviceToHost));
    L->out_pending = false;
  }
  out->average_reported_error = L->out.avg;
  out->global_error = L->out.global_error;
  out->global_obs = L->out.g_obs;
  out->global_mm = L->out.g_mm;
  out->n_groups = L->n_groups;
  return ok();
}

int bqsr_lut_group(const bqsr_lut* lc, int32_t r, int64_t* obs, int64_t* mm) {
  bqsr_lut* L = const_cast<bqsr_lut*>(lc);
  if (!L || lut_host(L) != BQSR_OK) return -1;
  if (r + 1 < 0 || r + 1 >= L->n_groups || !L->h_grp_ok[(size_t)(r + 1)]) return 0;
  *obs = L->h_grp_obs[(size_t)(r + 1)];
  *mm = L->h_grp_mm[(size_t)(r + 1)];
  return 1;
}

bqsr_status bqsr_lut_shifts(const bqsr_lut* lc, int32_t key, int32_t qual, int32_t cyc, int32_t ctx, double sh[4],
                            int32_t* new_q) {
  bqsr_lut* L = const_cast<bqsr_lut*>(lc);
  if (!L || !sh || !new_q) return fail(BQSR_ERR_INVALID_ARG, "null");
  bqsr_status st = lut_host(L);
  if (st != BQSR_OK) return st;
  const TableGeom g = geom(L->dims);
  if (cyc < -g.L || cyc > g.L || ctx < -4 || ctx > 16) return fail(BQSR_ERR_INVALID_ARG, "covariate out of range");
  const int64_t r = ((int64_t)key - 1) / kMaxQ;
  if (r + 1 < 0 || r + 1 >= L->n_groups || !L->h_grp_ok[(size_t)(r + 1)])
    return fail(BQSR_ERR_MISSING_KEY, "read group missing");
  const double avg = L->out.avg;
  double v;
  const double rgd = (eprob(L->h_grp_obs[(size_t)(r + 1)], L->h_grp_mm[(size_t)(r + 1)], &v) ? v : avg) - avg;
  if (key < 0 || key >= g.K || L->h_words[(size_t)key] == 0) return fail(BQSR_ERR_MISSING_KEY, "key missing");
  if (qual < 0 || qual > 255) return fail(BQSR_ERR_QUAL_RANGE, "qual out of range");
  const double e = pow10tab().v[qual];
  const double a1 = e + rgd;
  const double qd = (eprob(L->h_qk_obs[(size_t)key], L->h_qk_mm[(size_t)key], &v) ? v : a1) - a1;
  const double a2 = a1 + qd;
  const int64_t* obs = L->h_words.data() + g.K;
  const int64_t* mm = obs + (int64_t)g.K * g.cells;
  const int64_t c1 = (int64_t)key * g.cells + cyc + g.L, c2 = (int64_t)key * g.cells + g.C + ctx + 4;
  const double cd = (eprob(obs[c1], mm[c1], &v) ? v : a2) - a2;
  const double xd = (eprob(obs[c2], mm[c2], &v) ? v : a2) - a2;
  sh[0] = rgd;
  sh[1] = qd;
  sh[2] = cd;
  sh[3] = xd;
  double p = e;
  for (int i = 0; i < 4; ++i) p = p + sh[i];
  *new_q = phred_of(p);
  return ok();
}

int32_t bqsr_phred_threshold_table(double* out, int32_t cap, int32_t* qmin) {
  const auto& t = thresholds().thr;
  if (qmin) *qmin = kThrQmin;
  if (out) memcpy(out, t.data(), sizeof(double) * (size_t)std::min<int32_t>(cap, (int32_t)t.size()));
  return (int32_t)t.size();
}



bqsr_status bqsr_apply_stage(bqsr_context* ctx, bqsr_batch* b, const bqsr_lut* L, uint8_t* out_qual,
                             uint32_t* out_start, uint32_t* out_len, uint64_t* exceptions, int64_t max_exceptions,
                             int32_t stages, void* stream) {
  if (!ctx || !b || !L || !out_qual || !out_start || !out_len) return fail(BQSR_ERR_INVALID_ARG, "null");
  if (b->dims.n_rg > L->dims.n_rg || b->dims.max_len > L->dims.max_len)
    return fail(BQSR_ERR_INVALID_ARG, "table dims smaller than the batch's");
  HIP_TRY(hipSetDevice(ctx->device));
  hipStream_t s = S(stream);
  if (stages & BQSR_STAGE_RESET) {
    HIP_TRY(hipMemsetAsync(b->d_err + kErrAppKern, 0xFF, 8, s));
    HIP_TRY(hipMemsetAsync(b->d_err + kNExc, 0, 8, s));
  }
  if (!b->prepped || (stages & BQSR_STAGE_PREP)) {
    bqsr_status st = launch_prep(ctx, b, nullptr, s);
    if (st != BQSR_OK) return st;
  }
  if (b->rd.n_reads == 0 || !(stages & (BQSR_STAGE_KERNEL | BQSR_STAGE_LUT))) return ok();
  ApplyParams P{};
  P.rd = b->pass_rd();
  P.ord = b->order();
  P.info = b->d_info;
  P.g = geom(L->dims);
  const int cw = window_cw(b, P.g);
  P.w = window_rows(b, apply_rows(cw));
  P.n_rg = L->dims.n_rg;
  P.s1 = L->s1;
  P.d2 = L->d2;
  P.rq_ok = L->rq_ok;
  P.key_ok = L->key_ok;
  P.grp_ok = L->grp_ok;
  P.n_groups = L->n_groups;
  P.thr = ctx->d_thr;
  P.thr_qmin = kThrQmin;
  P.thr_n = kThrN;
  P.qb_thr = ctx->d_qbt;
  P.qb_q = ctx->d_qbq;
  P.out_qual = out_qual;
  P.out_start = out_start;
  P.out_len = out_len;
  P.exc = (unsigned long long*)exceptions;
  P.max_exc = exceptions ? max_exceptions : 0;
  P.n_exc = b->d_err + kNExc;
  P.err = b->d_err + kErrAppKern;
  P.piece_stride = piece_bytes(P.w.qw, cw);
  const size_t need = (size_t)P.piece_stride * (size_t)b->n_base + (size_t)b->n_base * 16;
  if (b->chars_bytes < need) {
    if (b->d_chars) {
      HIP_TRY(hipStreamSynchronize(s));
      (void)hipFree(b->d_chars);
      b->d_chars = nullptr;
      b->chars_bytes = 0;
    }
    HIP_TRY(hipMalloc((void**)&b->d_chars, need));
    b->chars_bytes = need;
    b->chars_lut = nullptr;
  }
  P.chars = b->d_chars;
  P.rowbad = (uint32_t*)(b->d_chars + (size_t)P.piece_stride * (size_t)b->n_base);
  P.qmask = b->hq_valid ? b->d_qmask : nullptr;
  const bool lut_stage = (stages & BQSR_STAGE_LUT) || ((stages & BQSR_STAGE_KERNEL) && !(stages & BQSR_STAGE_NO_LUT));
  if (lut_stage) {
    HIP_TRY(hipMemsetAsync(P.rowbad, 0, (size_t)b->n_base * 16, s));
    const unsigned cb = (unsigned)std::min<int64_t>(((int64_t)need + 255) / 256, (int64_t)ctx->n_cu * 16);
    hipLaunchKernelGGL(bqsr_apply_chars, dim3(cb), dim3(256), 0, s, P, b->d_chars);
    b->chars_lut = L;
  }
  if (stages & BQSR_STAGE_KERNEL) {
    if (b->chars_lut != L) return fail(BQSR_ERR_INVALID_ARG, "apply kernel before the LUT stage of this LUT");
    P.outs_apart = b->bucketed;
    hipLaunchKernelGGL(bqsr_apply_kernel, dim3(b->pass_blocks()), dim3(kBlockThreads), apply_lds(P.w.qw, cw), s, P);
    if (P.outs_apart) {
      ApplyParams Q = P;
      Q.rd = b->rd;
      hipLaunchKernelGGL(bqsr_apply_outs, dim3((unsigned)std::min<int64_t>((b->rd.n_reads + 255) / 256, (int64_t)ctx->n_cu * 8)),
                         dim3(256), 0, s, Q);
    }
  }
  HIP_TRY(hipGetLastError());
  return ok();
}

bqsr_status bqsr_apply_async(bqsr_context* ctx, bqsr_batch* b, const bqsr_lut* L, uint8_t* out_qual,
                             uint32_t* out_start, uint32_t* out_len, uint64_t* exceptions, int64_t max_exceptions,
                             void* stream) {
  return bqsr_apply_stage(ctx, b, L, out_qual, out_start, out_len, exceptions, max_exceptions,
                          BQSR_STAGE_RESET | BQSR_STAGE_KERNEL, stream);
}

bqsr_status bqsr_apply_result(bqsr_batch* b, int64_t* n_exceptions, void* stream) {
  HIP_TRY(hipSetDevice(b->ctx->device));
  hipStream_t s = S(stream);
  unsigned long long w[kErrWords];
  HIP_TRY(hipMemcpyAsync(w, b->d_err, sizeof w, hipMemcpyDeviceToHost, s));
  HIP_TRY(hipStreamSynchronize(s));
  if (n_exceptions) *n_exceptions = (int64_t)w[kNExc];
  return from_err_key(std::min(w[kErrAppPrep], w[kErrAppKern]), 0);
}

bqsr_status bqsr_apply(bqsr_context* ctx, bqsr_batch* b, const bqsr_lut* l, uint8_t* out_qual, uint32_t* out_start,
                       uint32_t* out_len, uint64_t* exceptions, int64_t max_exceptions, int64_t* n_exceptions,
                       void* stream) {
  bqsr_status st = bqsr_apply_async(ctx, b, l, out_qual, out_start, out_len, exceptions, max_exceptions, stream);
  if (st != BQSR_OK) return st;
  return bqsr_apply_result(b, n_exceptions, stream);
}

bqsr_status bqsr_apply_records(bqsr_context* ctx, const bqsr_records* R, const bqsr_lut* l, uint16_t* out_qual,
                               uint32_t* out_len) {
  if (!ctx || !R || !l || !out_qual || !out_len) return fail(BQSR_ERR_INVALID_ARG, "null");
  bqsr_batch* b = nullptr;
  bqsr_status st = bqsr_batch_create(ctx, R, nullptr, &b);
  if (st != BQSR_OK) return st;
  const int64_t n = R->n_reads;
  uint8_t* d_out = nullptr;
  uint32_t *d_start = nullptr, *d_len = nullptr;
  uint64_t* d_exc = nullptr;
  const int64_t max_exc = 1 << 16;
  std::vector<void*> tmp;
  if ((st = dalloc(tmp, &d_out, (size_t)b->n_slots + 16)) != BQSR_OK || (st = dalloc(tmp, &d_start, (size_t)n)) != BQSR_OK ||
      (st = dalloc(tmp, &d_len, (size_t)n)) != BQSR_OK || (st = dalloc(tmp, &d_exc, (size_t)max_exc)) != BQSR_OK) {
    for (void* p : tmp) (void)hipFree(p);
    bqsr_batch_destroy(b);
    return st;
  }
  int64_t n_exc = 0;
  st = bqsr_apply(ctx, b, l, d_out, d_start, d_len, d_exc, max_exc, &n_exc, nullptr);
  if (st == BQSR_OK && n_exc > max_exc) st = fail(BQSR_ERR_UNSUPPORTED, "too many non-byte quality chars");
  if (st == BQSR_OK) {
    std::vector<uint8_t> h_out((size_t)b->n_slots + 16);
    std::vector<uint32_t> h_start((size_t)std::max<int64_t>(n, 1)), h_len((size_t)std::max<int64_t>(n, 1));
    std::vector<uint64_t> h_exc((size_t)std::max<int64_t>(n_exc, 1));
    hipError_t e = hipMemcpy(h_out.data(), d_out, h_out.size(), hipMemcpyDeviceToHost);
    if (e == hipSuccess && n) e = hipMemcpy(h_start.data(), d_start, (size_t)n * 4, hipMemcpyDeviceToHost);
    if (e == hipSuccess && n) e = hipMemcpy(h_len.data(), d_len, (size_t)n * 4, hipMemcpyDeviceToHost);
    if (e == hipSuccess && n_exc) e = hipMemcpy(h_exc.data(), d_exc, (size_t)n_exc * 8, hipMemcpyDeviceToHost);
    if (e != hipSuccess) {
      st = fail(BQSR_ERR_DEVICE, hipGetErrorString(e));
    } else {
      std::vector<uint64_t> slot((size_t)n + 1, 0);
      for (int64_t r = 0; r < n; ++r) {
        const uint32_t f = R->flags[r];
        const uint64_t lq = (f & BQSR_F_HAS_QUAL) ? R->qual_offset[r + 1] - R->qual_offset[r] : 0;
        const uint64_t ls = (f & BQSR_F_HAS_SEQ) ? R->seq_offset[r + 1] - R->seq_offset[r] : 0;
        slot[(size_t)r + 1] = slot[(size_t)r] + (b->rd.slots_aligned ? slot_span(lq, ls) : std::max(lq, ls));
      }
      std::vector<uint16_t> wide;
      std::vector<std::pair<uint64_t, uint16_t>> ex;
      for (int64_t i = 0; i < n_exc; ++i) ex.push_back({h_exc[(size_t)i] >> 16, (uint16_t)(h_exc[(size_t)i] & 0xFFFF)});
      std::sort(ex.begin(), ex.end());
      for (int64_t r = 0; r < n; ++r) {
        uint16_t* dst = out_qual + R->qual_offset[r];
        const uint64_t s0 = slot[(size_t)r] + h_start[(size_t)r];
        for (uint32_t k = 0; k < h_len[(size_t)r]; ++k) {
          uint16_t v = h_out[s0 + k];
          if (!ex.empty()) {
            auto it = std::lower_bound(ex.begin(), ex.end(), std::make_pair(s0 + k, (uint16_t)0));
            if (it != ex.end() && it->first == s0 + k) v = it->second;
          }
          dst[k] = v;
        }
        out_len[r] = h_len[(size_t)r];
      }
    }
  }
  for (void* p : tmp) (void)hipFree(p);
  bqsr_batch_destroy(b);
  return st;
}


bqsr_status bqsr_job_reset_async(bqsr_batch* b, bqsr_table* t, void* stream) {
  if (!b || !t) return fail(BQSR_ERR_INVALID_ARG, "null");
  HIP_TRY(hipSetDevice(b->ctx->device));
  const int64_t n = table_words(t->dims);
  const unsigned g = (unsigned)std::min<int64_t>(std::max<int64_t>(1, (n + 255) / 256), (int64_t)b->ctx->n_cu * 8);
  hipLaunchKernelGGL(bqsr_job_reset_kernel, dim3(g), dim3(256), 0, S(stream), t->words, n, b->d_err);
  HIP_TRY(hipGetLastError());
  b->err_fresh = true;
  return ok();
}

bqsr_status bqsr_job_errors_export_async(bqsr_batch* b, int64_t read_base, int64_t* dst_device, void* stream) {
  if (!b || !dst_device || read_base < 0) return fail(BQSR_ERR_INVALID_ARG, "null / negative read base");
  HIP_TRY(hipSetDevice(b->ctx->device));
  hipLaunchKernelGGL(bqsr_job_err_export, dim3(1), dim3(64), 0, S(stream), (const unsigned long long*)b->d_err,
                     read_base, dst_device);
  HIP_TRY(hipGetLastError());
  return ok();
}

bqsr_status bqsr_job_errors_import_async(bqsr_batch* b, const int64_t* src_device, void* stream) {
  if (!b || !src_device) return fail(BQSR_ERR_INVALID_ARG, "null");
  HIP_TRY(hipSetDevice(b->ctx->device));
  hipLaunchKernelGGL(bqsr_job_err_import, dim3(1), dim3(64), 0, S(stream), (unsigned long long*)b->d_err, src_device);
  HIP_TRY(hipGetLastError());
  return ok();
}

bqsr_status bqsr_job_status_async(bqsr_batch* b, bqsr_lut* L, int32_t slot, void* stream) {
  if (!b || !L || slot < 0 || slot >= kStatusSlots) return fail(BQSR_ERR_INVALID_ARG, "null / bad slot");
  HIP_TRY(hipSetDevice(b->ctx->device));
  if (!b->h_status)
    HIP_TRY(hipHostMalloc((void**)&b->h_status, kJobStatusWords * 8 * (1 + kStatusSlots), hipHostMallocDefault));
  hipLaunchKernelGGL(bqsr_job_status_kernel, dim3(1), dim3(64), 0, S(stream), (const unsigned long long*)b->d_err,
                     (const double*)b->d_em, (const FinalOut*)L->d_out, b->h_status + kJobStatusWords * (1 + slot));
  HIP_TRY(hipGetLastError());
  return ok();
}

bqsr_status bqsr_job_status_get(const bqsr_batch* b, int32_t slot, int32_t part, double* em, int64_t* n_exceptions) {
  if (!b || !b->h_status || slot < 0 || slot >= kStatusSlots || part < 0 || part > 2)
    return fail(BQSR_ERR_INVALID_ARG, "no snapshot / bad slot or part");
  const uint64_t* h = b->h_status + kJobStatusWords * (1 + slot);
  if (em) std::memcpy(em, h + kErrWords, 8);
  if (n_exceptions) *n_exceptions = (int64_t)h[kNExc];
  if (part == 0) return from_err_key(h[kErrObs], 0);
  if (part == 1) {
    FinalOut fo;
    std::memcpy(&fo, h + kErrWords + 1, sizeof(FinalOut));
    return fo.any_key ? ok() : fail(BQSR_ERR_EMPTY_TABLE, "empty.reduceLeft: no usable base was observed");
  }
  return from_err_key(std::min(h[kErrAppPrep], h[kErrAppKern]), 0);
}

static int64_t copy_blocks(const bqsr_context* ctx) { return std::min<int64_t>(32, (int64_t)ctx->n_cu * 8); }
bqsr_status bqsr_copy_async(bqsr_context* ctx, void* dst, const void* src, int64_t bytes, void* stream) {
  if (!ctx || bytes < 0 || (bytes && (!dst || !src))) return fail(BQSR_ERR_INVALID_ARG, "bqsr_copy_async: bad arguments");
  if (!bytes) return ok();
  HIP_TRY(hipSetDevice(ctx->device));
  const bool vec = (((uintptr_t)dst | (uintptr_t)src) & 15) == 0;
  const int64_t n16 = vec ? bytes / 16 : 0;
  const int64_t head = 16 * n16, tail = bytes - head;
  const int64_t need = std::max<int64_t>((n16 + 255) / 256, (tail + 255) / 256);
  const unsigned g = (unsigned)std::max<int64_t>(1, std::min<int64_t>(need, copy_blocks(ctx)));
  hipLaunchKernelGGL(bqsr_copy16, dim3(g), dim3(256), 0, S(stream), (const uint4*)src, (uint4*)dst, n16,
                     (const uint8_t*)src + head, (uint8_t*)dst + head, tail);
  HIP_TRY(hipGetLastError());
  return ok();
}

bqsr_status bqsr_job_result(bqsr_batch* b, bqsr_lut* L, double* em, int64_t* n_exceptions, void* stream) {
  if (!b || !L) return fail(BQSR_ERR_INVALID_ARG, "null");
  HIP_TRY(hipSetDevice(b->ctx->device));
  hipStream_t s = S(stream);
  if (!b->h_status)
    HIP_TRY(hipHostMalloc((void**)&b->h_status, kJobStatusWords * 8 * (1 + kStatusSlots), hipHostMallocDefault));
  hipLaunchKernelGGL(bqsr_job_status_kernel, dim3(1), dim3(64), 0, s, (const unsigned long long*)b->d_err,
                     (const double*)b->d_em, (const FinalOut*)L->d_out, b->h_status);
  HIP_TRY(hipGetLastError());
  HIP_TRY(hipStreamSynchronize(s));
  const uint64_t* h = b->h_status;
  std::memcpy(&L->out, h + kErrWords + 1, sizeof(FinalOut));
  L->out_pending = false;
  if (em) std::memcpy(em, h + kErrWords, 8);
  if (n_exceptions) *n_exceptions = (int64_t)h[kNExc];
  bqsr_status st = from_err_key(h[kErrObs], 0);
  if (st != BQSR_OK) return st;
  if (!L->out.any_key) return fail(BQSR_ERR_EMPTY_TABLE, "empty.reduceLeft: no usable base was observed");
  return from_err_key(std::min(h[kErrAppPrep], h[kErrAppKern]), 0);
}

}

#include "device_job.h"
#include "sam_ingest.hip"
#include "bgzf_inflate.hip"
#include "bam_ingest.hip"
#include "mark_duplicates.cpp"
#include "adam_out.hip"
#include "bam_out.hip"
#include "bgzf_deflate.hip"
#include "sam_sort.hip"
#include "flagstat.hip"
#include "sam_batch.hip"
#include "arrow_ingest.hip"
#include "pileup.hip"
#include "mpileup.hip"
#include "realign_targets.hip"
#include "pileup_agg.hip"
#include "compare.hip"
#include "tags.hip"
#include "parquet_gzip.cpp"

extern "C" {

bqsr_status bqsr_compact_outputs_async(bqsr_context* ctx, bqsr_batch* b, const uint8_t* out_qual,
                                       const uint32_t* out_start, const uint32_t* out_len, uint64_t* exceptions,
                                       int64_t max_exceptions, uint8_t* chars, uint32_t* offsets, uint16_t* lengths,
                                       void* stream) {
  if (!ctx || !b || !out_qual || !out_start || !out_len || !chars || !offsets || max_exceptions < 0 ||
      (max_exceptions > 0 && !exceptions))
    return fail(BQSR_ERR_INVALID_ARG, "bqsr_compact_outputs_async: bad arguments");
  if (b->n_slots > (int64_t)UINT32_MAX) return fail(BQSR_ERR_UNSUPPORTED, "compacted chars above 4 GiB");
  HIP_TRY(hipSetDevice(ctx->device));
  hipStream_t s = S(stream);
  const int64_t n = b->rd.n_reads;
  if (!b->d_off64 || b->off64_n < n) {
    if (b->d_off64) {
      HIP_TRY(hipStreamSynchronize(s));
      (void)hipFree(b->d_off64);
      b->d_off64 = nullptr;
    }
    const size_t words = 2 * ((size_t)n + 1) + (size_t)n / samk::kScanChunk + 2;
    HIP_TRY(hipMalloc((void**)&b->d_off64, words * 8));
    b->off64_n = n;
  }
  uint64_t* len64 = b->d_off64;
  uint64_t* off64 = len64 + n + 1;
  uint64_t* part = off64 + n + 1;
  const unsigned g = (unsigned)std::max<int64_t>(1, std::min<int64_t>((n + 255) / 256, (int64_t)ctx->n_cu * 8));
  if (n > 0) hipLaunchKernelGGL(bqsr_compact_lens, dim3(g), dim3(256), 0, s, out_len, n, len64);
  bqsr_status st = sam_scan(len64, n, off64, part, s);
  if (st != BQSR_OK) return st;
  if (n > 0) {
    hipLaunchKernelGGL(bqsr_compact_chars, dim3(g), dim3(256), 0, s, (const ReadMeta*)b->rd.meta, out_qual, out_start,
                       (const uint64_t*)off64, n, chars, offsets, lengths);
    if (max_exceptions > 0)
      hipLaunchKernelGGL(bqsr_compact_exceptions, dim3(4), dim3(256), 0, s, (const ReadMeta*)b->rd.meta, n, out_start,
                         (const uint64_t*)off64, (unsigned long long*)exceptions,
                         (const unsigned long long*)(b->d_err + kNExc), max_exceptions);
  } else {
    HIP_TRY(hipMemsetAsync(offsets, 0, 4, s));
  }
  HIP_TRY(hipGetLastError());
  return ok();
}

const void* bqsr_batch_exception_count_ptr(const bqsr_batch* b) { return b ? (const void*)(b->d_err + kNExc) : nullptr; }

bqsr_status bqsr_copy_dyn_async(bqsr_context* ctx, void* dst, const void* src, const void* count, int32_t count_bytes,
                                int64_t scale, int64_t max_bytes, void* stream) {
  if (!ctx || !dst || !src || !count || (count_bytes != 4 && count_bytes != 8) || scale < 0 || max_bytes < 0)
    return fail(BQSR_ERR_INVALID_ARG, "bqsr_copy_dyn_async: bad arguments");
  HIP_TRY(hipSetDevice(ctx->device));
  const unsigned g = (unsigned)std::max<int64_t>(1, std::min<int64_t>((max_bytes / 16 + 255) / 256, copy_blocks(ctx)));
  hipLaunchKernelGGL(bqsr_copy_dyn, dim3(g), dim3(256), 0, S(stream), (const uint8_t*)src, (uint8_t*)dst, count,
                     count_bytes, scale, max_bytes);
  HIP_TRY(hipGetLastError());
  return ok();
}

}
```

### adam_amd/csrc/bqsr_internal.h

```cpp
#pragma once
#include <hip/hip_runtime.h>
#include <stdint.h>

#include "../../include/adam_bqsr.h"

namespace bqsr {

struct ReadMeta {
  uint64_t slot;
  uint16_t lq;
  uint16_t ls;
  uint16_t flags;
  uint16_t rg;
};
static_assert(sizeof(ReadMeta) == 16, "ReadMeta must be 16 B");

struct ReadAlign {
  int64_t start;
  uint32_t cigar_off;
  uint32_t md_off;
  int32_t contig;
  uint16_t n_cigar;
  uint16_t md_len;
};
static_assert(sizeof(ReadAlign) == 24, "ReadAlign must be 24 B");

struct alignas(8) ReadInfo {
  uint16_t st;
  uint16_t en;
  uint16_t fl;
  uint16_t pad;
};
static_assert(sizeof(ReadInfo) == 8 && alignof(ReadInfo) == 8, "ReadInfo must be one aligned 8-B word");
__device__ __forceinline__ ReadInfo info_load(const ReadInfo* p) {
  const uint64_t v = __hip_atomic_load((const uint64_t*)p, __ATOMIC_RELAXED, __HIP_MEMORY_SCOPE_WORKGROUP);
  return ReadInfo{(uint16_t)v, (uint16_t)(v >> 16), (uint16_t)(v >> 32), (uint16_t)(v >> 48)};
}
__device__ __forceinline__ void info_store(ReadInfo* p, ReadInfo x) {
  const uint64_t v = (uint64_t)x.st | ((uint64_t)x.en << 16) | ((uint64_t)x.fl << 32) | ((uint64_t)x.pad << 48);
  __hip_atomic_store((uint64_t*)p, v, __ATOMIC_RELAXED, __HIP_MEMORY_SCOPE_WORKGROUP);
}
constexpr uint16_t kInfoObs = 1;
constexpr uint16_t kInfoObsCheck = 2;
constexpr uint16_t kInfoApp = 4;
constexpr uint16_t kInfoAppCheck = 8;
constexpr uint16_t kInfoNeg = 16;
constexpr uint16_t kInfoSecond = 32;
constexpr uint16_t kInfoPass = 64;
constexpr uint16_t kInfoCycNeg = 128;
constexpr uint16_t kInfoTrim = 256;
constexpr uint16_t kInfoNoBits = 512;

constexpr uint16_t kSeqOther = 1u << 15;

constexpr uint8_t kCodeA = 0, kCodeC = 1, kCodeG = 2, kCodeT = 3, kCodeN = 4, kCodeOther = 5;

constexpr int kMaxQ = 60;
constexpr int kCtxSlots = 21;
constexpr uint32_t kCtxTab = 4096;
constexpr int kCtxTabBytes = 2 * kCtxTab * 2;
constexpr int kQBins = 128;

constexpr int kTileSlots = 4096;
constexpr int kMaxTileReads = 64;
constexpr int kMaxFoldBlocks = 1024;
constexpr int kWaves = 16;
constexpr int kBlockThreads = 64 * kWaves;
constexpr int kMkWords = kWaves * 64;
constexpr int kMaxReadLen = 4096;
constexpr int kColumnPad = 32;
constexpr int kRedSlabs = 16;

constexpr uint64_t kNoError = ~0ull;
__host__ __device__ inline uint64_t err_key(uint64_t read, uint32_t o, uint32_t rank, uint32_t code) {
  return (read << 28) | ((uint64_t)(o & 0xFFFFF) << 8) | ((uint64_t)(rank & 0xF) << 4) | (code & 0xF);
}
enum : uint32_t {
  kRankCtor = 0,
  kRankCigar = 1,
  kRankMd = 2,
  kRankSnp = 3,
  kRankCov = 4,
  kRankTable = 5
};
enum { kErrObs = 0, kErrAppPrep = 1, kErrAppKern = 2, kNExc = 3, kErrWords = 4 };
constexpr int kJobStatusWords = 16;
constexpr int kStatusSlots = 4;

struct SitesDev {
  const int64_t* pos;
  const uint64_t* off;
  const uint32_t* bucket;
  const uint64_t* bucket_off;
  const int64_t* bucket_base;
  const uint64_t* bm;
  const uint64_t* bm_off;
  const int64_t* bm_base;
  int32_t n_contigs;
  int32_t shift;
};

struct TableGeom {
  int32_t K;
  int32_t C;
  int32_t L;
  int32_t cells;
};

struct Window {
  int32_t qw;
  int32_t q_lo;
  int32_t rg_lo;
};

struct ReadsDev {
  const ReadMeta* meta;
  const ReadAlign* align;
  const uint8_t* qual;
  const uint8_t* bases;
  const uint32_t* cigar;
  const uint8_t* md;
  int64_t n_reads;
  int64_t n_slots;
  int32_t reads_per_tile;
  int64_t n_tiles;
  int32_t slots_aligned;
};
__host__ __device__ inline uint64_t slot_span(uint64_t lq, uint64_t ls) {
  const uint64_t sl = lq > ls ? lq : ls;
  return (sl + 15) & ~(uint64_t)15;
}

struct PrepParams {
  ReadsDev rd;
  SitesDev sites;
  ReadInfo* info;
  uint64_t* sbits;
  unsigned long long* err;
  uint32_t* work;
  uint32_t* n_work;
};

struct OrderDev {
  const uint32_t* perm;
  const int64_t* key_off;
  int32_t n_keys;
  int32_t n_base = 0;
  const uint64_t* kslot = nullptr;
};

struct ObserveParams {
  ReadsDev rd;
  OrderDev ord;
  ReadInfo* info;
  const uint64_t* sbits;
  TableGeom g;
  Window w;
  int64_t* touched;
  int64_t* obs;
  int64_t* mm;
  uint32_t* part;
  int32_t part_stride;
  uint32_t* hq_block;
  unsigned long long* err;
  int32_t n_blocks;
  int32_t wcells;
  int32_t lane_shift;
  int32_t orow;
  int32_t nc;
  int32_t rows_all;
};

constexpr int32_t kFoldNoBase = INT32_MIN;
constexpr int kSegBinades = 32;
constexpr double kFoldTie = -1.0, kFoldUnknown = -2.0;
constexpr int kFoldMaxSegs = 64;
enum : int32_t { kSegRun = 0, kSegEvent = 1, kSegGlobal = 2 };

struct FoldBlock {
  double r0, r1;
  double inc;
  int32_t e;
  int32_t cidx;
};
static_assert(sizeof(FoldBlock) == 32, "FoldBlock is 4 words");

struct FoldSeg {
  int64_t inc;
  int32_t t0, t1;
  int32_t e;
  int32_t kind;
  int64_t off;
};
static_assert(sizeof(FoldSeg) == 32, "FoldSeg is 4 words");

struct FoldParams {
  ReadsDev rd;
  const ReadInfo* info;
  const uint32_t* hq_block;
  const double* pow10;
  int32_t n_blocks;
  FoldBlock* blk;
  int32_t* cand_list;
  int32_t* n_cand;
  double* delta;
  double* rtile;
  int32_t* ntile;
  double* dtile;
  FoldSeg* seg;
  int32_t* seg_base;
  int32_t* nseg;
  uint32_t* seg_used;
  uint8_t* streams;
  double* csum;
  int64_t stream_cap;
  unsigned long long* stream_used;
  double* em_out;
  uint32_t* qmask;
};

constexpr int kQbElo = -48;
constexpr int kQbEhi = 3;
constexpr int kQbBits = 5;
constexpr int kQbN = (kQbEhi - kQbElo + 1) << kQbBits;

struct ApplyParams {
  ReadsDev rd;
  OrderDev ord;
  const ReadInfo* info;
  TableGeom g;
  Window w;
  int32_t n_rg;
  const double* s1;
  const double* d2;
  const uint8_t* rq_ok;
  const uint8_t* key_ok;
  const uint8_t* grp_ok;
  int32_t n_groups;
  const double* thr;
  int32_t thr_qmin;
  int32_t thr_n;
  const double* qb_thr;
  const int16_t* qb_q;
  uint8_t* out_qual;
  uint32_t* out_start;
  uint32_t* out_len;
  unsigned long long* exc;
  int64_t max_exc;
  unsigned long long* n_exc;
  unsigned long long* err;
  int32_t lane_shift;
  int32_t outs_apart;
  const uint8_t* chars;
  int64_t piece_stride;
  uint32_t* rowbad;
  const uint32_t* qmask;
};

struct FinalOut {
  int64_t g_obs, g_mm;
  double avg, global_error;
  int32_t any_key;
  int32_t pad;
};
static_assert(kErrWords + 1 + sizeof(FinalOut) / 8 <= (size_t)kJobStatusWords, "job status words overflow");
static_assert(sizeof(FinalOut) % 8 == 0, "FinalOut is whole words");

constexpr int kThrQmin = -3100;
constexpr int kThrQmax = 3300;
constexpr int kThrN = kThrQmax - kThrQmin + 1;

}
```

### adam_amd/csrc/bqsr_kernels.hip

```cpp
#include <hip/hip_runtime.h>

#include "bqsr_internal.h"

namespace bqsr {


__device__ __forceinline__ void wave_sync() {
  __builtin_amdgcn_fence(__ATOMIC_SEQ_CST, "workgroup");
  __builtin_amdgcn_wave_barrier();
}

__device__ __forceinline__ bool usable_read(uint16_t f) {
  return (f & BQSR_F_MAPPED) && (f & BQSR_F_PRIMARY) && !(f & BQSR_F_DUPLICATE) && (f & BQSR_F_HAS_MD);
}
__device__ __forceinline__ bool eligible_read(uint16_t f) {
  return (f & BQSR_F_MAPPED) && (f & BQSR_F_PRIMARY) && !(f & BQSR_F_DUPLICATE);
}

__device__ __forceinline__ void report(unsigned long long* err, uint64_t key) { atomicMin(err, (unsigned long long)key); }

__device__ __forceinline__ uint32_t cig_op(uint32_t e) { return e & 0xFu; }
__device__ __forceinline__ uint32_t cig_len(uint32_t e) { return e >> 4; }
__device__ __forceinline__ bool is_seg_op(uint32_t op) {
  return op == BQSR_CIGAR_M || op == BQSR_CIGAR_X || op == BQSR_CIGAR_EQ || op == BQSR_CIGAR_S;
// ... 1804 lines not shown
  return true;
}

extern "C" __global__ void __launch_bounds__(256) bqsr_final_groups(const int64_t* touched, const int64_t* qk_obs,
                                                                      const int64_t* qk_mm, TableGeom g, int32_t n_rg,
                                                                      double em_host, const double* em_dev,
                                                                      const double* pow10, int32_t n_groups,
                                                                      int64_t* grp_obs, int64_t* grp_mm, uint8_t* grp_ok,
                                                                      uint8_t* key_ok, double* a2, uint8_t* rq_ok,
                                                                      FinalOut* out) {
  const int tid = threadIdx.x;
  __shared__ int64_t s_go[256], s_gm[256];
  __shared__ int s_any[256];
  const int lane = tid & 63;
  int64_t go = 0, gm = 0;
  int any = 0;
  for (int i = tid >> 6; i < n_groups; i += blockDim.x >> 6) {
    const int r = i - 1;
    int64_t so = 0, sm = 0;
    int ok = 0;
    if (r >= 0) {
      const int k0 = r == 0 ? 0 : kMaxQ * r + 1, k1 = min(g.K - 1, kMaxQ * r + kMaxQ);
      const int k = k0 + lane;
      if (k <= k1 && touched[k]) {
        ok = 1;
        so = qk_obs[k];
        sm = qk_mm[k];
      }
    }
    for (int off = 32; off > 0; off >>= 1) {
      so += __shfl_xor(so, off);
      sm += __shfl_xor(sm, off);
      ok |= __shfl_xor(ok, off);
    }
    if (lane == 0) {
      grp_obs[i] = so;
      grp_mm[i] = sm;
      grp_ok[i] = (uint8_t)ok;
      go += so;
      gm += sm;
      any |= ok;
    }
  }
  for (int k = tid; k < g.K; k += blockDim.x) key_ok[k] = touched[k] != 0;
  for (int off = 32; off > 0; off >>= 1) {
    go += __shfl_xor(go, off);
    gm += __shfl_xor(gm, off);
    any |= __shfl_xor(any, off);
  }
  if ((tid & 63) == 0) {
    s_go[tid >> 6] = go;
    s_gm[tid >> 6] = gm;
    s_any[tid >> 6] = any;
  }
  __syncthreads();
  if (tid == 0) {
    go = gm = 0;
    any = 0;
    for (int i = 0; i < (int)(blockDim.x >> 6); ++i) {
      go += s_go[i];
      gm += s_gm[i];
      any |= s_any[i];
    }
    out->g_obs = go;
    out->g_mm = gm;
    out->any_key = any;
    const double em = em_dev ? *em_dev : em_host;
    const double avg = em / (double)go;
    out->avg = avg;
    double ge;
    out->global_error = err_prob(go, gm, pow10[kMaxQ], &ge) ? ge : avg;
  }
  __syncthreads();
  const double avg = out->avg;
  const double mre = pow10[kMaxQ];
  for (int i = tid; i < n_rg * kQBins; i += blockDim.x) {
    const int rg = i / kQBins, q = i - rg * kQBins;
    const int key = q + kMaxQ * rg;
    const int r = (key - 1) / kMaxQ;
    const bool ok = key < g.K && touched[key] != 0 && grp_ok[r + 1];
    rq_ok[i] = ok;
    if (!ok) {
      a2[i] = 0.0;
      continue;
    }
    double v;
    const double rg_delta = (err_prob(grp_obs[r + 1], grp_mm[r + 1], mre, &v) ? v : avg) - avg;
    const double e = pow10[q];
    const double a1 = e + rg_delta;
    const double q_delta = (err_prob(qk_obs[key], qk_mm[key], mre, &v) ? v : a1) - a1;
    a2[i] = a1 + q_delta;
  }
}

extern "C" __global__ void bqsr_final_tables(const int64_t* obs, const int64_t* mm, TableGeom g, int32_t n_rg,
                                             const double* a2, const uint8_t* rq_ok, double mre, double* s1,
                                             double* d2) {
  const int64_t n1 = (int64_t)n_rg * kQBins * g.C, n2 = (int64_t)n_rg * kQBins * kCtxSlots;
  for (int64_t i = blockIdx.x * (int64_t)blockDim.x + threadIdx.x; i < n1 + n2; i += (int64_t)gridDim.x * blockDim.x) {
    int64_t rq, cell;
    if (i < n1) {
      rq = i / g.C;
      cell = i - rq * g.C;
    } else {
      rq = (i - n1) / kCtxSlots;
      cell = g.C + (i - n1 - rq * kCtxSlots);
    }
    if (!rq_ok[rq]) {
      if (i < n1) s1[i] = 0.0; else d2[i - n1] = 0.0;
      continue;
    }
    const int rg = (int)(rq / kQBins), q = (int)(rq - (int64_t)rg * kQBins);
    const int64_t key = q + (int64_t)kMaxQ * rg;
    const double x = a2[rq];
    double v;
    const int64_t gi = key * g.cells + cell;
    const double delta = (err_prob(obs[gi], mm[gi], mre, &v) ? v : x) - x;
    if (i < n1) s1[i] = x + delta; else d2[i - n1] = delta;
  }
}


__device__ __forceinline__ int32_t phred_q(double p, const double* qb_thr, const int16_t* qb_q, const double* thr,
                                           int qmin, int nthr) {
  const uint64_t b = (uint64_t)__double_as_longlong(p);
  if (b - 1ull < 0x7FEFFFFFFFFFFFFFull) {
    const int e = (int)(b >> 52) - 1023;
    if (e >= kQbElo && e <= kQbEhi) {
      const int idx = ((e - kQbElo) << kQbBits) | (int)((b >> (52 - kQbBits)) & ((1u << kQbBits) - 1u));
      const int q = qb_q[idx];
      if (q != -32768) return p <= qb_thr[idx] ? q : q - 1;
    }
    int lo = 0, hi = nthr - 1;
    while (lo < hi) {
      const int mid = (lo + hi + 1) >> 1;
      if (p <= thr[mid]) lo = mid; else hi = mid - 1;
    }
    return qmin + lo;
  }
  if (p != p) return 0;
  if (p == 0.0) return 2147483647;
  if (p < 0.0) return 0;
  return (int32_t)0x80000000;
}

struct ApplyPiece {
  const uint8_t* lut;
  int rg_lo, c_lo, cw, cw21, q_lo, qw;
  uint32_t tb;
  int clean_lo, clean_hi;
  bool all_cycles;
  bool folded_clean;
};

struct ChunkLoads {
  uint4 qs, cr;
};
__device__ __forceinline__ ChunkLoads apply_load(const ApplyParams& P, const LaneRead& x, int j, bool on) {
  ChunkLoads v{make_uint4(0, 0, 0, 0), make_uint4(0, 0, 0, 0)};
  if (on) {
    const int o0 = x.st + j;
    v.qs = *(const uint4*)(P.rd.qual + x.slot + o0);
    if (!(x.fl & kInfoPass)) v.cr = chunk_raw(P.rd, chunk_n0(x, o0));
  }
  return v;
}

typedef unsigned short u16x2 __attribute__((ext_vector_type(2)));


__device__ __forceinline__ uint4 apply_slow(const ApplyParams* Pp, LaneRead x, int o0, uint32_t slow, uint64_t x01,
                                         uint64_t x23, uint4 outv) {
  const ApplyParams& P = *Pp;
  const bool app = x.fl & kInfoApp;
  const uint8_t* qp = P.rd.qual + x.slot;
  uint64_t lo = ((uint64_t)outv.y << 32) | outv.x, hi = ((uint64_t)outv.w << 32) | outv.z;
  while (slow) {
    const int k = __builtin_ctz(slow);
    slow &= slow - 1;
    const int o = o0 + k;
    const int q = (int)(int8_t)qp[o];
    const int xs = (int)(((k < 8 ? x01 : x23) >> (8 * (k & 7))) & 0xFFu);
    const int64_t key = (int64_t)q + (int64_t)kMaxQ * x.rg;
    const int64_t gr = (key - 1) / kMaxQ;
    const bool grp = (gr + 1) >= 0 && (gr + 1) < P.n_groups && P.grp_ok[gr + 1];
    const bool kok = key >= 0 && key < P.g.K && P.key_ok[key];
    if (!grp || !kok) {
      report(P.err, err_key((uint64_t)x.ro, (uint32_t)o, kRankTable, BQSR_ERR_MISSING_KEY));
      continue;
    }
    if (q < 0) {
      report(P.err, err_key((uint64_t)x.ro, (uint32_t)o, kRankTable, BQSR_ERR_QUAL_RANGE));
      continue;
    }
    if (!app) continue;
    const int64_t rq = (int64_t)x.rg * kQBins + q;
    const int ccell = x.cell0 + __mul24(x.dir, o);
    const double p = P.s1[rq * P.g.C + ccell] + P.d2[rq * kCtxSlots + xs];
    const int32_t Q = phred_q(p, P.qb_thr, P.qb_q, P.thr, P.thr_qmin, P.thr_n);
    const uint32_t code = ((uint32_t)Q + 33u) & 0xFFFFu;
    if (code > 0xFFu) {
      const unsigned long long e = atomicAdd(P.n_exc, 1ull);
      if ((int64_t)e < P.max_exc) P.exc[e] = ((x.oslot + (uint64_t)o) << 16) | code;
    }
    const uint64_t m = 0xFFull << (8 * (k & 7)), v = (uint64_t)(code & 0xFFu) << (8 * (k & 7));
    if (k < 8) lo = (lo & ~m) | v; else hi = (hi & ~m) | v;
  }
  return make_uint4((uint32_t)lo, (uint32_t)(lo >> 32), (uint32_t)hi, (uint32_t)(hi >> 32));
}

template <bool kTest>
__device__ __forceinline__ void apply_chunk(const ApplyParams& P, const ApplyParams* Pp, const ApplyPiece& pc,
                                            const LaneRead& x, int j, int n, bool on, const ChunkLoads& ld) {
  if (!on) return;
  const bool app = x.fl & kInfoApp, pass = x.fl & kInfoPass;
  const int o0 = x.st + j;
  const uint4 qs = ld.qs;
  const uint32_t qd[4] = {qs.x, qs.y, qs.z, qs.w};
  uint32_t out[4];
  uint32_t slow = 0;
  uint32_t xo[4] = {4u, 4u, 4u, 4u};
  if (pass) {
#pragma unroll
    for (int i2 = 0; i2 < 4; ++i2) out[i2] = ((qd[i2] & 0x7F7F7F7Fu) + 0x21212121u) ^ (qd[i2] & 0x80808080u);
  } else {
    chunk_ctx(P.rd, x.fl & kInfoNeg, chunk_n0(x, o0), ld.cr, j, pc.tb, xo);
    const int wc0 = x.cell0 + __mul24(x.dir, o0) - pc.c_lo;
    const uint32_t nv = (uint32_t)min(kChunk, n - j);
    const int klo = j < 0 ? -j : 0;
    const bool cok = app && x.rg == pc.rg_lo &&
                     (pc.all_cycles || ((unsigned)(wc0 + __mul24(klo, x.dir)) < (unsigned)pc.cw &&
                                        (unsigned)(wc0 + __mul24((int)nv - 1, x.dir)) < (unsigned)pc.cw));
    const uint32_t vmask = (nv >= 16u ? 0xFFFFu : ((1u << nv) - 1u)) & (0xFFFFu << klo);
    const int dx = x.dir * kCtxSlots;
    const uint32_t lbase = (uint32_t)(uintptr_t)(LdsBytes)pc.lut;
    const uint32_t amax = lbase + (uint32_t)(pc.qw * pc.cw21 - 1);
    uint32_t ei[kChunk];
    uint32_t ek = lbase + (uint32_t)(wc0 * kCtxSlots - pc.q_lo * pc.cw21);
#pragma unroll
    for (int k = 0; k < kChunk; ++k) {
      const uint32_t q = __builtin_amdgcn_ubfe(qd[k >> 2], 8 * (k & 3), 8);
      const uint32_t xs = __builtin_amdgcn_ubfe(xo[k >> 2], 8 * (k & 3), 8);
      ei[k] = min((uint32_t)__mul24((int)q, pc.cw21) + ek + xs, amax);
      ek += (uint32_t)dx;
    }
#pragma unroll
    for (int w = 0; w < 4; ++w) {
      u16x2 a, b;
      a.x = *(LdsBytes)(uintptr_t)ei[4 * w];
      b.x = *(LdsBytes)(uintptr_t)ei[4 * w + 1];
      a.y = *(LdsBytes)(uintptr_t)ei[4 * w + 2];
      b.y = *(LdsBytes)(uintptr_t)ei[4 * w + 3];
      out[w] = __builtin_amdgcn_perm(__builtin_bit_cast(uint32_t, b), __builtin_bit_cast(uint32_t, a), 0x06020400u);
    }
    uint32_t badm = kTest ? 0u : ((x.fl & kInfoObs) ? 0u : 0xFFFFu);
    if (kTest) {
      const uint32_t lo4 = (uint32_t)pc.clean_lo * 0x01010101u, hi4 = (uint32_t)pc.clean_hi * 0x01010101u;
#pragma unroll
      for (int w = 0; w < 4; ++w) {
        const uint32_t v = qd[w] | 0x80808080u;
        const uint32_t bad = ((qd[w] | ~(v - lo4) | (v - hi4)) & 0x80808080u) >> 7;
        badm |= ((bad | (bad >> 7) | (bad >> 14) | (bad >> 21)) & 0xFu) << (4 * w);
      }
    }
    slow = vmask & (cok ? badm : 0xFFFFu);
  }
  if (__builtin_amdgcn_ballot_w64(slow != 0)) {
    if (slow) {
      const uint4 r = apply_slow(Pp, x, o0, slow, ((uint64_t)xo[1] << 32) | xo[0], ((uint64_t)xo[3] << 32) | xo[2],
                                 make_uint4(out[0], out[1], out[2], out[3]));
      out[0] = r.x;
      out[1] = r.y;
      out[2] = r.z;
      out[3] = r.w;
    }
  }
  if (app || pass) {
    uint8_t* op = P.out_qual + x.oslot;
    if (j + kChunk <= n || P.rd.slots_aligned) {
      *(uint4*)(op + o0) = make_uint4(out[0], out[1], out[2], out[3]);
    } else {
#pragma unroll
      for (int k = 0; k < kChunk; ++k)
        if (k < n - j) op[o0 + k] = (uint8_t)(out[k >> 2] >> (8 * (k & 3)));
    }
  }
}

constexpr int kApplyU = 4;

extern "C" __global__ void bqsr_apply_outs(ApplyParams P) {
  for (int64_t r = blockIdx.x * (int64_t)blockDim.x + threadIdx.x; r < P.rd.n_reads; r += (int64_t)gridDim.x * blockDim.x) {
    const LaneRead x = lane_read(P.rd, P.info, r, true, P.g.L);
    if (x.fl & kInfoPass) {
      P.out_start[r] = 0;
      P.out_len[r] = (uint32_t)x.en;
    } else {
      P.out_start[r] = (uint32_t)x.st;
      P.out_len[r] = (x.fl & kInfoApp) ? (uint32_t)(x.en - x.st) : 0u;
    }
  }
}

extern "C" __global__ void bqsr_apply_chars(ApplyParams P, uint8_t* chars) {
  const int nk = order_base_keys(P.ord), qw = P.w.qw, q_lo = P.w.q_lo;
  const int64_t total = (int64_t)nk * P.piece_stride;
  for (int64_t t = blockIdx.x * (int64_t)blockDim.x + threadIdx.x; t < total; t += (int64_t)gridDim.x * blockDim.x) {
    const int key = (int)(t / P.piece_stride);
    const int64_t e = t - (int64_t)key * P.piece_stride;
    const WinGeom gm = win_geom(P.ord, P.g, key);
    const int64_t cw21 = (int64_t)gm.cw * kCtxSlots;
    const bool pad = e >= (int64_t)qw * cw21;
    const int row = pad ? 0 : (int)(e / cw21);
    const int rem = (int)(e - row * cw21), c = rem / kCtxSlots, x = rem - c * kCtxSlots;
    const int rg = key_rg(P.ord, key, P.w.rg_lo);
    const int64_t rq = (int64_t)rg * kQBins + q_lo + row;
    uint8_t v = 0;
    if (!pad && rg < P.n_rg && q_lo + row < kQBins && P.rq_ok[rq]) {
      const int32_t Q = phred_q(P.s1[rq * P.g.C + gm.c_lo + c] + P.d2[rq * kCtxSlots + x], P.qb_thr, P.qb_q, P.thr,
                                P.thr_qmin, P.thr_n);
      const uint32_t code = ((uint32_t)Q + 33u) & 0xFFFFu;
      v = code <= 0xFFu ? (uint8_t)code : 0;
    }
    if (!pad) chars[t] = v;
    const int zr = (!pad && v == 0) ? key * kQBins + row : -1;
    const int prev = __shfl_up(zr, 1);
    if (zr >= 0 && ((threadIdx.x & 63) == 0 || prev != zr))
      atomicOr(&P.rowbad[(zr >> 7) * 4 + ((zr & 127) >> 5)], 1u << (zr & 31));
  }
}

extern "C" __global__ void __launch_bounds__(kBlockThreads) bqsr_apply_kernel(ApplyParams P) {
  extern __shared__ __align__(16) unsigned char smem[];
  const int qw = P.w.qw, C = P.g.C, L = P.g.L;
  uint32_t* clean_rows = (uint32_t*)smem;
  uint32_t* mk_all = (uint32_t*)(smem + 16);
  uint16_t* ctab = (uint16_t*)(smem + 16 + kMkWords * 4);
  uint8_t* lut = smem + 16 + kMkWords * 4 + kCtxTabBytes;
  const uint32_t tb = (uint32_t)(uintptr_t)(LdsHalves)ctab;

  const int tid = threadIdx.x;
  const int wave = __builtin_amdgcn_readfirstlane(tid >> 6);
  const int lane = tid & 63;
  uint32_t* mk = mk_all + wave * 64;
  const int q_lo = P.w.q_lo;
  const int G = gridDim.x;
  const int64_t wa = pass_begin(P.rd, P.ord, blockIdx.x, G), wb = pass_begin(P.rd, P.ord, blockIdx.x + 1, G);
  const int nk = order_keys(P.ord);
  ctx_table_fill(ctab, tid, blockDim.x);

  for (int key = wa < wb ? key_at(P.ord, wa) : nk; key < nk; ++key) {
    const int64_t p0 = max(wa, key_begin(P.ord, P.rd.n_reads, key));
    const int64_t p1 = min(wb, key_begin(P.ord, P.rd.n_reads, key + 1));
    if (p0 >= wb) break;
    if (p0 >= p1) continue;
    const int rg_lo = key_rg(P.ord, key, P.w.rg_lo);
    const WinGeom gm = win_geom(P.ord, P.g, key);
    __syncthreads();
    {
      const uint4* src = (const uint4*)(P.chars + (int64_t)base_key(P.ord, key) * P.piece_stride);
      uint4* dst = (uint4*)lut;
      const int n16 = (int)(P.piece_stride >> 4);
      for (int i = tid; i < n16; i += blockDim.x) dst[i] = src[i];
    }
    if (tid == 0) {
      const uint4 rb = *(const uint4*)(P.rowbad + base_key(P.ord, key) * 4);
      const uint32_t rw[4] = {rb.x, rb.y, rb.z, rb.w};
      int best_lo = 0, best_n = 0, run = 0;
      for (int r = 0; r < qw; ++r) {
        const bool bad = (rw[r >> 5] >> (r & 31)) & 1u;
        run = bad ? 0 : run + 1;
        if (run > best_n) {
          best_n = run;
          best_lo = r - run + 1;
        }
      }
      clean_rows[0] = (uint32_t)(q_lo + best_lo);
      clean_rows[1] = (uint32_t)(q_lo + best_lo + best_n);
      uint32_t fc = 0;
      if (P.qmask) {
        const uint4 qm = *(const uint4*)P.qmask;
        const uint32_t qw4[4] = {qm.x, qm.y, qm.z, qm.w};
        fc = 1;
        for (int q = 0; q < kQBins; ++q)
          if (((qw4[q >> 5] >> (q & 31)) & 1u) && (q < q_lo + best_lo || q >= q_lo + best_lo + best_n)) fc = 0;
      }
      clean_rows[2] = fc;
    }
    __syncthreads();
    const ApplyPiece pc{lut, rg_lo, gm.c_lo, gm.cw, gm.cw * kCtxSlots, q_lo, qw, tb, (int)clean_rows[0],
                        (int)clean_rows[1], gm.c_lo == 0 && gm.cw == C, clean_rows[2] != 0};
    const auto fread = [&](LaneRead& x, bool live) {
      if (!live || P.outs_apart) return;
      if (x.fl & kInfoPass) {
        P.out_start[x.ro] = 0;
        P.out_len[x.ro] = (uint32_t)x.en;
      } else {
        P.out_start[x.ro] = (uint32_t)x.st;
        P.out_len[x.ro] = (x.fl & kInfoApp) ? (uint32_t)(x.en - x.st) : 0u;
      }
    };
    const auto fload = [&](const LaneRead& x, int j, bool on) { return apply_load(P, x, j, on); };
    if (pc.folded_clean) {
      const auto fchunk = [&](const LaneRead& x, int j, int n, bool on, const ChunkLoads& ld) {
        apply_chunk<false>(P, &P, pc, x, j, n, on, ld);
      };
      chunk_walk<kInfoApp | kInfoAppCheck | kInfoPass, kApplyU, ChunkLoads, false>(
          P.rd, P.info, P.ord, p0 + 64 * wave, p1, 64 * kWaves, L, lane, mk, fread, fload, fchunk);
    } else {
      const auto fchunk = [&](const LaneRead& x, int j, int n, bool on, const ChunkLoads& ld) {
        apply_chunk<true>(P, &P, pc, x, j, n, on, ld);
      };
      chunk_walk<kInfoApp | kInfoAppCheck | kInfoPass, kApplyU, ChunkLoads, false>(
          P.rd, P.info, P.ord, p0 + 64 * wave, p1, 64 * kWaves, L, lane, mk, fread, fload, fchunk);
    }
  }
}


extern "C" __global__ void bqsr_em_fold(const double* ems, int64_t n, double* out) {
  if (threadIdx.x != 0) return;
  double s = 0.0;
  for (int64_t i = 0; i < n; ++i) s = s + ems[i];
  *out = s;
}

extern "C" __global__ void bqsr_job_reset_kernel(int64_t* words, int64_t n, unsigned long long* err) {
  for (int64_t i = blockIdx.x * (int64_t)blockDim.x + threadIdx.x; i < n; i += (int64_t)gridDim.x * blockDim.x)
    words[i] = 0;
  if (blockIdx.x == 0 && threadIdx.x < kErrWords) err[threadIdx.x] = threadIdx.x == kNExc ? 0ull : ~0ull;
}
extern "C" __global__ void bqsr_job_status_kernel(const unsigned long long* err, const double* em, const FinalOut* fo,
                                                  uint64_t* host) {
  const int t = threadIdx.x;
  if (t < kErrWords) host[t] = err[t];
  else if (t == kErrWords) host[t] = (uint64_t)__double_as_longlong(*em);
  else if (t < kErrWords + 1 + (int)(sizeof(FinalOut) / 8)) host[t] = ((const uint64_t*)fo)[t - kErrWords - 1];
}

extern "C" __global__ void bqsr_job_err_export(const unsigned long long* err, int64_t read_base, int64_t* out) {
  const int t = threadIdx.x;
  if (t >= 2) return;
  const unsigned long long k = t == 0 ? err[kErrObs] : min(err[kErrAppPrep], err[kErrAppKern]);
  out[t] = k == kNoError ? INT64_MAX : (int64_t)(k + ((unsigned long long)read_base << 28));
}
extern "C" __global__ void bqsr_job_err_import(unsigned long long* err, const int64_t* in) {
  const int t = threadIdx.x;
  if (t == 0) err[kErrObs] = in[0] == INT64_MAX ? kNoError : (unsigned long long)in[0];
  if (t == 1) err[kErrAppPrep] = in[1] == INT64_MAX ? kNoError : (unsigned long long)in[1];
  if (t == 2) err[kErrAppKern] = kNoError;
}

extern "C" __global__ void bqsr_table_add(int64_t* acc, const int64_t* part, int64_t n) {
  for (int64_t i = blockIdx.x * (int64_t)blockDim.x + threadIdx.x; i < n; i += (int64_t)gridDim.x * blockDim.x)
    acc[i] += part[i];
}

}
```

### adam_amd/job.py

```python
from __future__ import annotations

import ctypes
from typing import Dict, List, Optional

import numpy as np

from . import _capi, bqsr
from . import distributed as D
from ._capi import check
from .records import RecordBatch


class ResidentJob:
    STAGES = ("prep", "observe", "fold", "apply")

    def __init__(self, batch: Optional[RecordBatch], dims, snp: Optional["bqsr.SnpTable"] = None, device: int = 0,
                 max_exc: int = 1 << 16, read_base: Optional[int] = None, sam=None, handle=None):
        import torch
        self.torch = torch
        self.L = L = _capi.lib()
        self.dev = torch.device("cuda", device)
        self.ctx = bqsr.Context.get(device)
        self.stream = torch.cuda.current_stream(self.dev)
        self.sp = ctypes.c_void_p(self.stream.cuda_stream)
        self.batch = batch
        self.dims = dims
        self.snp = snp
        self.bh = ctypes.c_void_p()
        if sam is not None or handle is not None:
            self.bh = handle if handle is not None else sam.device_batch(snp.contigs if snp else None, self.sp)
            self.n_reads = int(L.bqsr_batch_reads(self.bh))
            self.n_bases = int(L.bqsr_batch_bases(self.bh))
            if dims is None:
                dims = L.bqsr_batch_dims(self.bh)
                self.dims = dims
        else:
            s, keep = batch.c_struct(batch.contig_ids_for(snp.contigs if snp else None))
            check(L.bqsr_batch_create(self.ctx.handle, ctypes.byref(s), self.sp, ctypes.byref(self.bh)))
            del keep
            self.n_reads = batch.n_reads
            self.n_bases = batch.n_bases
        self.n_slots = int(L.bqsr_batch_slots(self.bh))
        words = int(L.bqsr_table_words(dims))
        self.table = torch.zeros(words, dtype=torch.int64, device=self.dev)
        self.th = ctypes.c_void_p()
        check(L.bqsr_table_create(self.ctx.handle, dims, ctypes.c_void_p(self.table.data_ptr()), ctypes.byref(self.th)))
        self.sites_h = snp.handle(self.ctx) if snp else None
        self.out_qual = torch.empty(self.n_slots + 64, dtype=torch.uint8, device=self.dev)
        self.out_start = torch.empty(max(1, self.n_reads), dtype=torch.int32, device=self.dev)
        self.out_len = torch.empty(max(1, self.n_reads), dtype=torch.int32, device=self.dev)
        self.max_exc = max_exc
        self.exc = torch.empty(max_exc, dtype=torch.int64, device=self.dev)
        self.em_part = torch.zeros(1, dtype=torch.float64, device=self.dev)
        self.lut = ctypes.c_void_p()
        self.world = D.dist.get_world_size() if D._multi() else 1
        if read_base is None and self.world > 1:
            raise ValueError("several ranks: read_base (reads of the ranks before this one) is required")
        self.read_base = int(read_base or 0)
        self.err_keys = torch.empty(2, dtype=torch.int64, device=self.dev)
        self.ev = [torch.cuda.Event(enable_timing=True) for _ in range(6)]
        self.kt: Dict[str, List[float]] = {k: [] for k in self.STAGES}
        self.n_exc = 0
        self.em = None
        torch.cuda.synchronize(self.dev)

    def _ptr(self, t):
        return ctypes.c_void_p(t.data_ptr())

    def layout_ms(self, reps: int = 3):
        ms = []
        for _ in range(reps):
            v = ctypes.c_double()
            check(self.L.bqsr_batch_relayout(self.bh, self.sp, ctypes.byref(v)))
            if v.value < 0:
                return None
            ms.append(v.value)
        return sum(ms) / len(ms)

    def layout_times(self):
        a, b = ctypes.c_double(), ctypes.c_double()
        check(self.L.bqsr_batch_layout_times(self.bh, ctypes.byref(a), ctypes.byref(b)))
        return None if b.value < 0 else (a.value, b.value)

    def step(self, record: bool = False):
        L, ctx, bh, th, sp, ev, stream = self.L, self.ctx.handle, self.bh, self.th, self.sp, self.ev, self.stream
        check(L.bqsr_job_reset_async(bh, th, sp))
        mark = (lambda i: ev[i].record(stream)) if record else (lambda i: None)
        mark(5)
        check(L.bqsr_observe_stage(ctx, bh, self.sites_h, th, _capi.STAGE_PREP, sp))
        mark(0)
        check(L.bqsr_observe_stage(ctx, bh, self.sites_h, th, _capi.STAGE_KERNEL, sp))
        mark(1)
        check(L.bqsr_observe_stage(ctx, bh, self.sites_h, th, _capi.STAGE_FOLD, sp))
        mark(2)
        if self.world > 1:
            check(L.bqsr_batch_em_copy_async(bh, self._ptr(self.em_part), sp))
            D.allreduce_table(self.table)
            self.em = D.fold_partition_ems_device(self.em_part, [1] * self.world, self.ctx, stream)
            em_ptr = self._ptr(self.em)
        else:
            self.em = None
            em_ptr = ctypes.c_void_p(L.bqsr_batch_em_device_ptr(bh))
        check(L.bqsr_finalize_device(ctx, th, em_ptr, ctypes.byref(self.lut), sp))
        args = (ctx, bh, self.lut, self._ptr(self.out_qual), self._ptr(self.out_start), self._ptr(self.out_len),
                self._ptr(self.exc), self.max_exc)
        if record:
            check(L.bqsr_apply_stage(*args, _capi.STAGE_LUT, sp))
            mark(3)
            check(L.bqsr_apply_stage(*args, _capi.STAGE_KERNEL | _capi.STAGE_NO_LUT, sp))
            mark(4)
        else:
            check(L.bqsr_apply_stage(*args, _capi.STAGE_KERNEL, sp))
        if self.world > 1:
            check(L.bqsr_job_errors_export_async(bh, self.read_base, self._ptr(self.err_keys), sp))
            D.allreduce_error_keys(self.err_keys)
            check(L.bqsr_job_errors_import_async(bh, self._ptr(self.err_keys), sp))
        em = ctypes.c_double()
        nexc = ctypes.c_int64()
        check(L.bqsr_job_result(bh, self.lut, ctypes.byref(em), ctypes.byref(nexc), sp))
        self.n_exc = int(nexc.value)
        if self.n_exc > self.max_exc:
            raise _capi.BQSRError(_capi.UNSUPPORTED, "%d chars above 0xFF exceed the exception list" % self.n_exc)
        if record:
            self.kt["prep"].append(ev[5].elapsed_time(ev[0]))
            self.kt["observe"].append(ev[0].elapsed_time(ev[1]))
            self.kt["fold"].append(ev[1].elapsed_time(ev[2]))
            self.kt["apply"].append(ev[3].elapsed_time(ev[4]))

    def kernel_ms(self) -> Dict[str, float]:
        return {k: float(np.mean(v)) if v else float("nan") for k, v in self.kt.items()}

    def expected_mismatch(self) -> float:
        if self.em is not None:
            return float(self.em.cpu()[0])
        v = ctypes.c_double()
        check(self.L.bqsr_observe_result(self.bh, ctypes.byref(v), self.sp))
        return v.value

    def results(self):
        self.torch.cuda.synchronize(self.dev)
        return (self.table.cpu().numpy(), self.expected_mismatch(), self.out_qual.cpu().numpy()[:self.n_slots],
                self.out_start.cpu().numpy()[:self.n_reads], self.out_len.cpu().numpy()[:self.n_reads],
                self.exc.cpu().numpy()[:self.n_exc])

    def close(self):
        L = self.L
        if self.lut:
            L.bqsr_lut_destroy(self.lut)
            self.lut = ctypes.c_void_p()
        if self.th:
            L.bqsr_table_destroy(self.th)
            self.th = ctypes.c_void_p()
        if self.bh:
            L.bqsr_batch_destroy(self.bh)
            self.bh = ctypes.c_void_p()
```

### include/adam_bqsr.h

```cpp
#ifndef ADAM_BQSR_H
#define ADAM_BQSR_H

#include <stddef.h>
#include <stdint.h>

#ifdef __cplusplus
extern "C" {
#endif

#define BQSR_ABI_VERSION 1

typedef enum bqsr_status {
  BQSR_OK = 0,
  BQSR_ERR_NULL_RG = 1,
  BQSR_ERR_MD_PARSE = 2,
  BQSR_ERR_CIGAR_SHORT = 3,
  BQSR_ERR_BAD_REVCOMP_BASE = 4,
  BQSR_ERR_EMPTY_TABLE = 5,
  BQSR_ERR_MISSING_KEY = 6,
  BQSR_ERR_QUAL_RANGE = 7,
  BQSR_ERR_NULL_FIELD = 8,
  BQSR_ERR_SEQ_SHORT = 9,
  BQSR_ERR_CIGAR_INVALID = 10,
  BQSR_ERR_INVALID_ARG = 11,
  BQSR_ERR_DEVICE = 12,
  BQSR_ERR_UNSUPPORTED = 13,
  BQSR_ERR_SAM_PARSE = 14,
  BQSR_ERR_PILEUP = 15,
  BQSR_ERR_ATTRIBUTE = 16,
  BQSR_ERR_UNSORTED = 17,
  BQSR_ERR_REFERENCE_CONFLICT = 18
} bqsr_status;

enum {
  BQSR_F_PAIRED = 1u << 0,
  BQSR_F_MAPPED = 1u << 1,
  BQSR_F_NEG_STRAND = 1u << 2,
  BQSR_F_SECOND_OF_PAIR = 1u << 3,
  BQSR_F_PRIMARY = 1u << 4,
  BQSR_F_DUPLICATE = 1u << 5,
  BQSR_F_HAS_RG = 1u << 8,
  BQSR_F_HAS_MD = 1u << 9,
  BQSR_F_HAS_QUAL = 1u << 10,
  BQSR_F_HAS_SEQ = 1u << 11,
  BQSR_F_HAS_CIGAR = 1u << 12,
  BQSR_F_HAS_START = 1u << 13,
  BQSR_F_HAS_REFNAME = 1u << 14
};

enum { BQSR_CIGAR_M = 0, BQSR_CIGAR_I = 1, BQSR_CIGAR_D = 2, BQSR_CIGAR_N = 3, BQSR_CIGAR_S = 4,
       BQSR_CIGAR_H = 5, BQSR_CIGAR_P = 6, BQSR_CIGAR_EQ = 7, BQSR_CIGAR_X = 8 };

#define BQSR_CONTIG_UNKNOWN (-1)

typedef struct bqsr_records {
  int64_t n_reads;
  const uint32_t* flags;
  const int32_t* rg_id;
  const int32_t* contig_id;
  const int64_t* start;
  const uint64_t* seq_offset;
  const uint8_t* seq;
  const uint64_t* qual_offset;
  const uint8_t* qual;
  const uint64_t* cigar_offset;
  const uint32_t* cigar;
  const uint64_t* md_offset;
  const uint8_t* md;
} bqsr_records;

typedef struct bqsr_dims {
  int32_t n_rg;
  int32_t max_len;
} bqsr_dims;

typedef struct bqsr_context bqsr_context;
typedef struct bqsr_sites bqsr_sites;
typedef struct bqsr_batch bqsr_batch;
typedef struct bqsr_table bqsr_table;
typedef struct bqsr_lut bqsr_lut;

int bqsr_abi_version(void);
const char* bqsr_last_error(void);
int64_t bqsr_last_error_read(void);
const char* bqsr_status_name(bqsr_status s);

bqsr_status bqsr_context_create(int device, bqsr_context** out);
void bqsr_context_destroy(bqsr_context* ctx);

enum {
  BQSR_TUNE_ORDER = 1,
  BQSR_TUNE_FRONTS = 2,
  BQSR_TUNE_KEYMAJOR = 3,
  BQSR_TUNE_FUSED_PREP = 4,
  BQSR_TUNE_BGZF = 5,
  BQSR_TUNE_FLAGSTAT_GRID = 6,
  BQSR_TUNE_PILEUP_GRID = 7
};
bqsr_status bqsr_context_tune(bqsr_context* ctx, int knob, int64_t value);

bqsr_status bqsr_sites_create(bqsr_context* ctx, const char* const* contigs, const int64_t* const* pos,
                              const uint64_t* n, int32_t n_contigs, bqsr_sites** out);
void bqsr_sites_destroy(bqsr_sites* s);

bqsr_status bqsr_batch_create(bqsr_context* ctx, const bqsr_records* recs, void* stream, bqsr_batch** out);
void bqsr_batch_destroy(bqsr_batch* b);
int64_t bqsr_batch_reads(const bqsr_batch* b);
int64_t bqsr_batch_bases(const bqsr_batch* b);
bqsr_dims bqsr_batch_dims(const bqsr_batch* b);
bqsr_status bqsr_batch_relayout(bqsr_batch* b, void* stream, double* ms);
bqsr_status bqsr_batch_layout_times(const bqsr_batch* b, double* alloc_ms, double* build_ms);

typedef struct bqsr_device_reads {
  int64_t n_reads;
  int64_t n_slots;
  const void* meta;
  const void* align;
  const uint8_t* qual;
  const uint8_t* bases;
  const uint32_t* cigar;
  const uint8_t* md;
  bqsr_dims dims;
  int32_t slots_aligned;
} bqsr_device_reads;
bqsr_status bqsr_batch_wrap_device(bqsr_context* ctx, const bqsr_device_reads* dev, bqsr_batch** out);

typedef struct bqsr_staged bqsr_staged;
bqsr_status bqsr_stage_records(bqsr_context* ctx, const bqsr_records* recs, bqsr_staged** out);
void bqsr_staged_destroy(bqsr_staged* s);
int64_t bqsr_staged_bytes(const bqsr_staged* s);
int64_t bqsr_staged_reads(const bqsr_staged* s);
int64_t bqsr_staged_bases(const bqsr_staged* s);
bqsr_status bqsr_batch_create_staged(bqsr_context* ctx, const bqsr_staged* s, bqsr_batch** out);
bqsr_status bqsr_batch_upload_async(bqsr_batch* b, const bqsr_staged* s, void* stream);

int64_t bqsr_table_words(bqsr_dims d);
bqsr_status bqsr_table_create(bqsr_context* ctx, bqsr_dims d, void* device_words, bqsr_table** out);
void bqsr_table_destroy(bqsr_table* t);
bqsr_dims bqsr_table_dims(const bqsr_table* t);
void* bqsr_table_device_ptr(bqsr_table* t);
bqsr_status bqsr_table_download(const bqsr_table* t, int64_t* host_words);
bqsr_status bqsr_table_upload(bqsr_table* t, const int64_t* host_words);

bqsr_status bqsr_observe(bqsr_context* ctx, bqsr_batch* b, const bqsr_sites* sites, bqsr_table* table,
                         double* expected_mismatch, void* stream);

bqsr_status bqsr_observe_records(bqsr_context* ctx, const bqsr_records* recs, const bqsr_sites* sites,
                                 bqsr_dims dims, bqsr_table** out_partial, double* out_expected_mismatch);

bqsr_status bqsr_table_merge(bqsr_table* acc, const bqsr_table* part, double* acc_em, double part_em);

bqsr_status bqsr_finalize(bqsr_context* ctx, const bqsr_table* t, double expected_mismatch, bqsr_lut** out);
void bqsr_lut_destroy(bqsr_lut* l);
typedef struct bqsr_final_stats {
  double average_reported_error;
  double global_error;
  int64_t global_obs, global_mm;
  int32_t n_groups;
} bqsr_final_stats;
bqsr_status bqsr_lut_stats(const bqsr_lut* l, bqsr_final_stats* out);
bqsr_status bqsr_lut_shifts(const bqsr_lut* l, int32_t qual_by_rg, int32_t qual, int32_t cycle, int32_t context,
                            double shifts[4], int32_t* new_q);

bqsr_status bqsr_apply(bqsr_context* ctx, bqsr_batch* b, const bqsr_lut* l, uint8_t* out_qual,
                       uint32_t* out_start, uint32_t* out_len, uint64_t* exceptions, int64_t max_exceptions,
                       int64_t* n_exceptions, void* stream);

bqsr_status bqsr_apply_records(bqsr_context* ctx, const bqsr_records* recs, const bqsr_lut* l,
                               uint16_t* out_qual, uint32_t* out_len);

enum { BQSR_STAGE_RESET = 1, BQSR_STAGE_KERNEL = 2, BQSR_STAGE_FOLD = 4, BQSR_STAGE_PREP = 8,
       BQSR_STAGE_LUT = 16, BQSR_STAGE_NO_LUT = 32 };
bqsr_status bqsr_observe_stage(bqsr_context* ctx, bqsr_batch* b, const bqsr_sites* sites, bqsr_table* t,
                               int32_t stages, void* stream);
bqsr_status bqsr_observe_async(bqsr_context* ctx, bqsr_batch* b, const bqsr_sites* sites, bqsr_table* t,
                               void* stream);
bqsr_status bqsr_observe_result(bqsr_batch* b, double* expected_mismatch, void* stream);
void* bqsr_batch_em_device_ptr(bqsr_batch* b);
bqsr_status bqsr_table_zero_async(bqsr_table* t, void* stream);
bqsr_status bqsr_finalize_async(bqsr_context* ctx, const bqsr_table* t, double expected_mismatch, bqsr_lut** out,
                                void* stream);
bqsr_status bqsr_finalize_result(bqsr_lut* l, void* stream);
bqsr_status bqsr_finalize_device(bqsr_context* ctx, const bqsr_table* t, const double* em_device, bqsr_lut** out,
                                 void* stream);
bqsr_status bqsr_batch_em_copy_async(bqsr_batch* b, double* dst_device, void* stream);
bqsr_status bqsr_em_fold_async(bqsr_context* ctx, const double* ems_device, int64_t n, double* out_device,
                               void* stream);
bqsr_status bqsr_apply_stage(bqsr_context* ctx, bqsr_batch* b, const bqsr_lut* l, uint8_t* out_qual,
                             uint32_t* out_start, uint32_t* out_len, uint64_t* exceptions, int64_t max_exceptions,
                             int32_t stages, void* stream);
bqsr_status bqsr_apply_async(bqsr_context* ctx, bqsr_batch* b, const bqsr_lut* l, uint8_t* out_qual,
                             uint32_t* out_start, uint32_t* out_len, uint64_t* exceptions, int64_t max_exceptions,
                             void* stream);
bqsr_status bqsr_apply_result(bqsr_batch* b, int64_t* n_exceptions, void* stream);

bqsr_status bqsr_batch_set_window(bqsr_batch* b, int32_t q_lo, int32_t rg_lo);
int32_t bqsr_batch_reads_per_tile(const bqsr_batch* b);
typedef struct bqsr_fold_stats {
  int64_t n_tiles;
  int64_t stream_used;
  int64_t stream_cap;
  int64_t lds_stream;
  int32_t n_blocks;
  int32_t reads_per_tile;
  int32_t cand_blocks;
  int32_t nobase_blocks;
  int32_t nobase_between;
  int32_t tileless_blocks;
  int32_t longest_run;
  int32_t capped_blocks;
  int32_t segs_total;
  int32_t segs_run;
  int32_t segs_event;
  int32_t segs_global;
  int32_t segs_refused;
  int32_t lds_segs;
} bqsr_fold_stats;
bqsr_status bqsr_batch_fold_stats(bqsr_batch* b, bqsr_fold_stats* out, void* stream);
int64_t bqsr_batch_slots(const bqsr_batch* b);
int bqsr_lut_group(const bqsr_lut* l, int32_t r, int64_t* obs, int64_t* mm);
int32_t bqsr_phred_threshold_table(double* out, int32_t cap, int32_t* qmin);

bqsr_status bqsr_copy_async(bqsr_context* ctx, void* dst, const void* src, int64_t bytes, void* stream);
bqsr_status bqsr_copy_dyn_async(bqsr_context* ctx, void* dst, const void* src, const void* count, int32_t count_bytes,
                                int64_t scale, int64_t max_bytes, void* stream);
bqsr_status bqsr_compact_outputs_async(bqsr_context* ctx, bqsr_batch* b, const uint8_t* out_qual,
                                       const uint32_t* out_start, const uint32_t* out_len, uint64_t* exceptions,
                                       int64_t max_exceptions, uint8_t* chars, uint32_t* offsets, uint16_t* lengths,
                                       void* stream);
const void* bqsr_batch_exception_count_ptr(const bqsr_batch* b);

bqsr_status bqsr_job_reset_async(bqsr_batch* b, bqsr_table* t, void* stream);
bqsr_status bqsr_job_result(bqsr_batch* b, bqsr_lut* l, double* expected_mismatch, int64_t* n_exceptions,
                            void* stream);
bqsr_status bqsr_job_status_async(bqsr_batch* b, bqsr_lut* l, int32_t slot, void* stream);
bqsr_status bqsr_job_status_get(const bqsr_batch* b, int32_t slot, int32_t part, double* expected_mismatch,
                                int64_t* n_exceptions);
bqsr_status bqsr_job_errors_export_async(bqsr_batch* b, int64_t read_base, int64_t* dst_device, void* stream);
bqsr_status bqsr_job_errors_import_async(bqsr_batch* b, const int64_t* src_device, void* stream);

#ifdef __cplusplus
}
#endif
#endif
```

Before: 515.3 billion bases/s.

## Speculatively overlap fold/finalize with apply via forked side stream and redo check

```diff
diff --git a/adam_amd/_capi.py b/adam_amd/_capi.py
--- a/adam_amd/_capi.py
+++ b/adam_amd/_capi.py
@@ -8,7 +8,7 @@
 LIB_PATH = os.environ.get("ADAM_BQSR_LIB") or os.path.join(_HERE, "libadam_bqsr.so")
 
 BQSR_OK = 0
-STAGE_RESET, STAGE_KERNEL, STAGE_FOLD, STAGE_PREP, STAGE_LUT, STAGE_NO_LUT = 1, 2, 4, 8, 16, 32
+STAGE_RESET, STAGE_KERNEL, STAGE_FOLD, STAGE_PREP, STAGE_LUT, STAGE_NO_LUT, STAGE_FORK = 1, 2, 4, 8, 16, 32, 64
 STATUS_NAMES = ["OK", "NULL_RG", "MD_PARSE", "CIGAR_SHORT", "BAD_REVCOMP_BASE", "EMPTY_TABLE", "MISSING_KEY",
                 "QUAL_RANGE", "NULL_FIELD", "SEQ_SHORT", "CIGAR_INVALID", "INVALID_ARG", "DEVICE", "UNSUPPORTED",
                 "SAM_PARSE", "PILEUP", "ATTRIBUTE"]
@@ -23,10 +23,10 @@
     "bqsr_batch_reads", "bqsr_batch_bases", "bqsr_batch_dims", "bqsr_batch_relayout", "bqsr_batch_layout_times", "bqsr_batch_wrap_device", "bqsr_table_words",
     "bqsr_table_create", "bqsr_table_destroy", "bqsr_table_dims", "bqsr_table_device_ptr", "bqsr_table_download",
     "bqsr_table_upload", "bqsr_observe", "bqsr_observe_records", "bqsr_table_merge", "bqsr_finalize",
-    "bqsr_lut_destroy", "bqsr_lut_stats", "bqsr_lut_shifts", "bqsr_apply", "bqsr_apply_records",
+    "bqsr_lut_destroy", "bqsr_lut_stats", "bqsr_lut_tables", "bqsr_lut_shifts", "bqsr_apply", "bqsr_apply_records",
     "bqsr_stage_records", "bqsr_staged_destroy", "bqsr_staged_bytes", "bqsr_staged_reads", "bqsr_staged_bases",
     "bqsr_batch_create_staged", "bqsr_batch_upload_async", "bqsr_em_fold_async", "bqsr_batch_em_copy_async",
-    "bqsr_finalize_device", "bqsr_observe_stage", "bqsr_apply_stage", "bqsr_job_reset_async", "bqsr_job_result", "bqsr_copy_async",
+    "bqsr_finalize_device", "bqsr_observe_stage", "bqsr_apply_stage", "bqsr_job_reset_async", "bqsr_job_result", "bqsr_job_tail_async", "bqsr_job_tail_path", "bqsr_copy_async",
     "bqsr_job_errors_export_async", "bqsr_job_errors_import_async", "bqsr_job_status_async", "bqsr_job_status_get",
     "bqsr_copy_dyn_async", "bqsr_compact_outputs_async", "bqsr_batch_exception_count_ptr",
     "bqsr_batch_fold_stats",
@@ -178,6 +178,9 @@
             "bqsr_apply_records": (ctypes.c_int, [vp, vp, vp, vp, vp]),
             "bqsr_job_reset_async": (ctypes.c_int, [vp, vp, vp]),
             "bqsr_job_result": (ctypes.c_int, [vp, vp, ctypes.POINTER(dbl), ctypes.POINTER(i64), vp]),
+            "bqsr_job_tail_async": (ctypes.c_int, [vp, vp, vp, vp, ctypes.POINTER(vp), vp, vp, vp, vp, i64, vp]),
+            "bqsr_job_tail_path": (i32, [vp]),
+            "bqsr_lut_tables": (ctypes.c_int, [vp, vp, vp, vp]),
             "bqsr_copy_async": (ctypes.c_int, [vp, vp, vp, i64, vp]),
             "bqsr_copy_dyn_async": (ctypes.c_int, [vp, vp, vp, vp, i32, i64, i64, vp]),
             "bqsr_compact_outputs_async": (ctypes.c_int, [vp, vp, vp, vp, vp, vp, i64, vp, vp, vp, vp]),
diff --git a/adam_amd/bqsr.py b/adam_amd/bqsr.py
--- a/adam_amd/bqsr.py
+++ b/adam_amd/bqsr.py
@@ -29,8 +29,10 @@
             cls._by_device[device] = Context(device)
         return cls._by_device[device]
 
-    _KNOBS = {"order": 1, "fronts": 2, "key_major": 3, "bgzf": 5, "flagstat_grid": 6, "pileup_grid": 7}
-    _DEFAULTS = {"order": -1, "fronts": -1, "key_major": 0, "bgzf": 1, "flagstat_grid": 0, "pileup_grid": 0}
+    _KNOBS = {"order": 1, "fronts": 2, "key_major": 3, "bgzf": 5, "flagstat_grid": 6, "pileup_grid": 7,
+              "spec_tail": 8, "spec_reserve": 9}
+    _DEFAULTS = {"order": -1, "fronts": -1, "key_major": 0, "bgzf": 1, "flagstat_grid": 0, "pileup_grid": 0,
+                 "spec_tail": 1, "spec_reserve": 8}
 
     def tune(self, **knobs) -> Dict[str, int]:
         cur = getattr(self, "_tuned", dict(self._DEFAULTS))
diff --git a/adam_amd/csrc/bqsr_capi.cpp b/adam_amd/csrc/bqsr_capi.cpp
--- a/adam_amd/csrc/bqsr_capi.cpp
+++ b/adam_amd/csrc/bqsr_capi.cpp
@@ -220,6 +220,8 @@
   int tune_bgzf = 1;
   int tune_flagstat_grid = 0;
   int tune_pileup_grid = 0;
+  int tune_spec_tail = 1;
+  int tune_spec_reserve = 8;
   std::mutex flagstat_mu;
   unsigned long long* d_flagstat = nullptr;
 };
@@ -356,9 +358,14 @@
   hipStream_t side = nullptr;
   hipEvent_t ev_obs = nullptr, ev_fold = nullptr;
   bool obs_pending = false;
+  hipEvent_t ev_tiles = nullptr;
+  bool tail_fork = false;
+  bool tail_spec = false;
+  uint32_t* d_tail = nullptr;
+  double* d_em_spec = nullptr;
   ~bqsr_batch() {
     if (side) (void)hipStreamDestroy(side);
-    for (hipEvent_t e : {ev_obs, ev_fold})
+    for (hipEvent_t e : {ev_obs, ev_fold, ev_tiles})
       if (e) (void)hipEventDestroy(e);
     if (d_part) (void)hipFree(d_part);
     if (d_off64) (void)hipFree(d_off64);
@@ -390,6 +397,7 @@
   int64_t *qk_obs = nullptr, *qk_mm = nullptr, *grp_obs = nullptr, *grp_mm = nullptr;
   uint8_t *grp_ok = nullptr, *key_ok = nullptr, *rq_ok = nullptr;
   double *a2 = nullptr, *s1 = nullptr, *d2 = nullptr;
+  double *a2s = nullptr, *s1s = nullptr, *d2s = nullptr;
   FinalOut* d_out = nullptr;
   FinalOut out{};
   bool out_pending = false;
@@ -454,6 +462,14 @@
       if (value < 0 || value > (1 << 20)) break;
       ctx->tune_pileup_grid = (int)value;
       return BQSR_OK;
+    case BQSR_TUNE_SPEC_TAIL:
+      if (value < 0 || value > 3) break;
+      ctx->tune_spec_tail = (int)value;
+      return BQSR_OK;
+    case BQSR_TUNE_SPEC_RESERVE:
+      if (value < 1 || value > 64) break;
+      ctx->tune_spec_reserve = (int)value;
+      return BQSR_OK;
     default:
       return fail(BQSR_ERR_INVALID_ARG, "bqsr_context_tune: unknown knob");
   }
@@ -476,7 +492,7 @@
   if (e == hipSuccess) e = hipMalloc(&c->d_qbq, kQbN * sizeof(int16_t));
   if (e == hipSuccess) e = hipMemcpy(c->d_qbt, buckets().thr.data(), kQbN * sizeof(double), hipMemcpyHostToDevice);
   if (e == hipSuccess) e = hipMemcpy(c->d_qbq, buckets().q.data(), kQbN * sizeof(int16_t), hipMemcpyHostToDevice);
-  for (const void* f : {(const void*)bqsr_apply_kernel, (const void*)bqsr_observe_chunks,
+  for (const void* f : {(const void*)bqsr_apply_kernel, (const void*)bqsr_redo_apply, (const void*)bqsr_observe_chunks,
                         (const void*)bqsr_observe_lean<true, false>, (const void*)bqsr_observe_lean<true, true>})
     if (e == hipSuccess) e = hipFuncSetAttribute(f, hipFuncAttributeMaxDynamicSharedMemorySize, (int)kLdsMax);
   if (e == hipSuccess)
@@ -1345,6 +1361,17 @@
 }
 
 namespace {
+FoldParams fold_params(const bqsr_context* ctx, const bqsr_batch* b, bool qmask) {
+  FoldParams F = b->fold;
+  F.rd = b->rd;
+  F.info = b->d_info;
+  F.hq_block = b->d_hq;
+  F.pow10 = ctx->d_pow10;
+  F.n_blocks = b->n_blocks;
+  F.em_out = b->d_em;
+  F.qmask = qmask ? b->d_qmask : nullptr;
+  return F;
+}
 bqsr_status launch_prep(bqsr_context* ctx, bqsr_batch* b, const bqsr_sites* sites, hipStream_t s) {
   if (!b->err_fresh) HIP_TRY(hipMemsetAsync(b->d_err + kErrAppPrep, 0xFF, 8, s));
   b->err_fresh = false;
@@ -1432,15 +1459,18 @@
     P.obs = t->obs();
     P.mm = t->mm();
     P.part_stride = 2 * P.w.qw * P.wcells + P.w.qw;
+    const bool tail_fork = lean && (stages & BQSR_STAGE_FORK) && ctx->tune_spec_tail != 0;
+    if ((!lean || tail_fork) && !b->side) {
+      HIP_TRY(hipStreamCreateWithFlags(&b->side, hipStreamNonBlocking));
+      HIP_TRY(hipEventCreateWithFlags(&b->ev_obs, hipEventDisableTiming));
+      HIP_TRY(hipEventCreateWithFlags(&b->ev_fold, hipEventDisableTiming));
+      HIP_TRY(hipEventCreateWithFlags(&b->ev_tiles, hipEventDisableTiming));
+    }
     if (!lean) {
-      if (!b->side) {
-        HIP_TRY(hipStreamCreateWithFlags(&b->side, hipStreamNonBlocking));
-        HIP_TRY(hipEventCreateWithFlags(&b->ev_obs, hipEventDisableTiming));
-        HIP_TRY(hipEventCreateWithFlags(&b->ev_fold, hipEventDisableTiming));
-      }
       HIP_TRY(hipEventRecord(b->ev_obs, s));
       b->obs_pending = true;
     }
+    b->tail_fork = false;
     const size_t need = (size_t)P.part_stride * (b->pass_blocks() + b->n_keys - 1);
     if (b->part_words < need) {
       if (b->d_part) {
@@ -1466,6 +1496,10 @@
       hipLaunchKernelGGL(bqsr_observe_chunks, dim3(P.n_blocks), dim3(kBlockThreads), lds, s, P);
     }
     HIP_TRY(hipGetLastError());
+    if (tail_fork) {
+      HIP_TRY(hipEventRecord(b->ev_obs, s));
+      b->tail_fork = true;
+    }
     const int rb = (int)std::min<int64_t>(4096, ((int64_t)P.part_stride * (b->bucketed ? b->n_base : 1) + 255) / 256);
     const unsigned ry = b->bucketed ? 1u : (unsigned)((b->n_blocks + kRedSlabs - 1) / kRedSlabs);
     hipLaunchKernelGGL(bqsr_window_reduce, dim3(rb, ry), dim3(256), 0, s, (const uint32_t*)b->d_part, b->rd, P.ord,
@@ -1486,14 +1520,9 @@
                          b->n_blocks, lane_shift(b), b->d_hq);
       HIP_TRY(hipGetLastError());
     }
-    FoldParams F = b->fold;
-    F.rd = b->rd;
-    F.info = b->d_info;
-    F.hq_block = b->d_hq;
-    F.pow10 = ctx->d_pow10;
-    F.n_blocks = b->n_blocks;
-    F.em_out = b->d_em;
-    F.qmask = b->d_qmask;
+    b->tail_fork = false;
+    b->tail_spec = false;
+    const FoldParams F = fold_params(ctx, b, true);
     hipLaunchKernelGGL(bqsr_fold_plan, dim3(1), dim3(1024), 0, s, F);
     const int64_t max_tpb = (b->rd.n_tiles + b->n_blocks - 1) / b->n_blocks + 1;
     hipLaunchKernelGGL(bqsr_fold_tiles, dim3(ctx->n_cu * 4), dim3(kFtWaves * 64), 0, s, F, max_tpb);
@@ -1562,11 +1591,7 @@
 
 
 namespace {
-bqsr_status finalize_impl(bqsr_context* ctx, const bqsr_table* t, double em, const double* em_dev, bqsr_lut** out,
-                          void* stream) {
-  if (!ctx || !t || !out) return fail(BQSR_ERR_INVALID_ARG, "null");
-  HIP_TRY(hipSetDevice(ctx->device));
-  hipStream_t s = S(stream);
+bqsr_status lut_for(bqsr_context* ctx, const bqsr_table* t, bqsr_lut** out, hipStream_t s, bqsr_lut** Lp, bool* fresh) {
   const TableGeom g = geom(t->dims);
   const int n_rg = t->dims.n_rg;
   bqsr_lut* L = *out;
@@ -1595,6 +1620,24 @@
     delete L;
     return st;
   }
+  *Lp = L;
+  *fresh = !reuse;
+  return BQSR_OK;
+}
+bqsr_status finalize_impl(bqsr_context* ctx, const bqsr_table* t, double em, const double* em_dev, bqsr_lut** out,
+                          void* stream) {
+  if (!ctx || !t || !out) return fail(BQSR_ERR_INVALID_ARG, "null");
+  HIP_TRY(hipSetDevice(ctx->device));
+  hipStream_t s = S(stream);
+  const TableGeom g = geom(t->dims);
+  const int n_rg = t->dims.n_rg;
+  bqsr_lut* L = nullptr;
+  bool fresh = false;
+  {
+    const bqsr_status st = lut_for(ctx, t, out, s, &L, &fresh);
+    if (st != BQSR_OK) return st;
+  }
+  const bool reuse = !fresh;
   hipLaunchKernelGGL(bqsr_final_keys, dim3((g.K + 3) / 4), dim3(256), 0, s, t->touched(), t->obs(), t->mm(), g, L->qk_obs,
                      L->qk_mm);
   hipLaunchKernelGGL(bqsr_final_groups, dim3(1), dim3(256), 0, s, t->touched(), L->qk_obs, L->qk_mm, g, n_rg, em,
@@ -1713,6 +1756,17 @@
   out->global_obs = L->out.g_obs;
   out->global_mm = L->out.g_mm;
   out->n_groups = L->n_groups;
+  return ok();
+}
+
+bqsr_status bqsr_lut_tables(const bqsr_lut* L, double* a2, double* s1, double* d2) {
+  if (!L) return fail(BQSR_ERR_INVALID_ARG, "null");
+  HIP_TRY(hipSetDevice(L->ctx->device));
+  HIP_TRY(hipDeviceSynchronize());
+  const size_t rq = (size_t)L->dims.n_rg * kQBins;
+  if (a2) HIP_TRY(hipMemcpy(a2, L->a2, rq * 8, hipMemcpyDeviceToHost));
+  if (s1) HIP_TRY(hipMemcpy(s1, L->s1, rq * (size_t)geom(L->dims).C * 8, hipMemcpyDeviceToHost));
+  if (d2) HIP_TRY(hipMemcpy(d2, L->d2, rq * kCtxSlots * 8, hipMemcpyDeviceToHost));
   return ok();
 }
 
@@ -1768,25 +1822,12 @@
 }
 
 
-
-bqsr_status bqsr_apply_stage(bqsr_context* ctx, bqsr_batch* b, const bqsr_lut* L, uint8_t* out_qual,
-                             uint32_t* out_start, uint32_t* out_len, uint64_t* exceptions, int64_t max_exceptions,
-                             int32_t stages, void* stream) {
-  if (!ctx || !b || !L || !out_qual || !out_start || !out_len) return fail(BQSR_ERR_INVALID_ARG, "null");
-  if (b->dims.n_rg > L->dims.n_rg || b->dims.max_len > L->dims.max_len)
-    return fail(BQSR_ERR_INVALID_ARG, "table dims smaller than the batch's");
-  HIP_TRY(hipSetDevice(ctx->device));
+namespace {
+bqsr_status apply_params(bqsr_context* ctx, bqsr_batch* b, const bqsr_lut* L, uint8_t* out_qual, uint32_t* out_start,
+                         uint32_t* out_len, uint64_t* exceptions, int64_t max_exceptions, void* stream,
+                         ApplyParams* out) {
+  ApplyParams P{};
   hipStream_t s = S(stream);
-  if (stages & BQSR_STAGE_RESET) {
-    HIP_TRY(hipMemsetAsync(b->d_err + kErrAppKern, 0xFF, 8, s));
-    HIP_TRY(hipMemsetAsync(b->d_err + kNExc, 0, 8, s));
-  }
-  if (!b->prepped || (stages & BQSR_STAGE_PREP)) {
-    bqsr_status st = launch_prep(ctx, b, nullptr, s);
-    if (st != BQSR_OK) return st;
-  }
-  if (b->rd.n_reads == 0 || !(stages & (BQSR_STAGE_KERNEL | BQSR_STAGE_LUT))) return ok();
-  ApplyParams P{};
   P.rd = b->pass_rd();
   P.ord = b->order();
   P.info = b->d_info;
@@ -1813,7 +1854,7 @@
   P.n_exc = b->d_err + kNExc;
   P.err = b->d_err + kErrAppKern;
   P.piece_stride = piece_bytes(P.w.qw, cw);
-  const size_t need = (size_t)P.piece_stride * (size_t)b->n_base + (size_t)b->n_base * 16;
+  const size_t need = (size_t)P.piece_stride * (size_t)b->n_base + (size_t)b->n_base * 32;
   if (b->chars_bytes < need) {
     if (b->d_chars) {
       HIP_TRY(hipStreamSynchronize(s));
@@ -1828,6 +1869,35 @@
   P.chars = b->d_chars;
   P.rowbad = (uint32_t*)(b->d_chars + (size_t)P.piece_stride * (size_t)b->n_base);
   P.qmask = b->hq_valid ? b->d_qmask : nullptr;
+  *out = P;
+  return BQSR_OK;
+}
+}
+
+bqsr_status bqsr_apply_stage(bqsr_context* ctx, bqsr_batch* b, const bqsr_lut* L, uint8_t* out_qual,
+                             uint32_t* out_start, uint32_t* out_len, uint64_t* exceptions, int64_t max_exceptions,
+                             int32_t stages, void* stream) {
+  if (!ctx || !b || !L || !out_qual || !out_start || !out_len) return fail(BQSR_ERR_INVALID_ARG, "null");
+  if (b->dims.n_rg > L->dims.n_rg || b->dims.max_len > L->dims.max_len)
+    return fail(BQSR_ERR_INVALID_ARG, "table dims smaller than the batch's");
+  HIP_TRY(hipSetDevice(ctx->device));
+  hipStream_t s = S(stream);
+  if (stages & BQSR_STAGE_RESET) {
+    HIP_TRY(hipMemsetAsync(b->d_err + kErrAppKern, 0xFF, 8, s));
+    HIP_TRY(hipMemsetAsync(b->d_err + kNExc, 0, 8, s));
+  }
+  if (!b->prepped || (stages & BQSR_STAGE_PREP)) {
+    bqsr_status st = launch_prep(ctx, b, nullptr, s);
+    if (st != BQSR_OK) return st;
+  }
+  if (b->rd.n_reads == 0 || !(stages & (BQSR_STAGE_KERNEL | BQSR_STAGE_LUT))) return ok();
+  ApplyParams P{};
+  {
+    const bqsr_status st = apply_params(ctx, b, L, out_qual, out_start, out_len, exceptions, max_exceptions, stream, &P);
+    if (st != BQSR_OK) return st;
+  }
+  const int cw = window_cw(b, P.g);
+  const size_t need = (size_t)P.piece_stride * (size_t)b->n_base + (size_t)b->n_base * 16;
   const bool lut_stage = (stages & BQSR_STAGE_LUT) || ((stages & BQSR_STAGE_KERNEL) && !(stages & BQSR_STAGE_NO_LUT));
   if (lut_stage) {
     HIP_TRY(hipMemsetAsync(P.rowbad, 0, (size_t)b->n_base * 16, s));
@@ -1947,6 +2017,7 @@
   hipLaunchKernelGGL(bqsr_job_reset_kernel, dim3(g), dim3(256), 0, S(stream), t->words, n, b->d_err);
   HIP_TRY(hipGetLastError());
   b->err_fresh = true;
+  b->tail_spec = false;
   return ok();
 }
 
@@ -1973,7 +2044,8 @@
   if (!b->h_status)
     HIP_TRY(hipHostMalloc((void**)&b->h_status, kJobStatusWords * 8 * (1 + kStatusSlots), hipHostMallocDefault));
   hipLaunchKernelGGL(bqsr_job_status_kernel, dim3(1), dim3(64), 0, S(stream), (const unsigned long long*)b->d_err,
-                     (const double*)b->d_em, (const FinalOut*)L->d_out, b->h_status + kJobStatusWords * (1 + slot));
+                     (const double*)b->d_em, (const FinalOut*)L->d_out, (const uint32_t*)nullptr,
+                     b->h_status + kJobStatusWords * (1 + slot));
   HIP_TRY(hipGetLastError());
   return ok();
 }
@@ -2016,7 +2088,8 @@
   if (!b->h_status)
     HIP_TRY(hipHostMalloc((void**)&b->h_status, kJobStatusWords * 8 * (1 + kStatusSlots), hipHostMallocDefault));
   hipLaunchKernelGGL(bqsr_job_status_kernel, dim3(1), dim3(64), 0, s, (const unsigned long long*)b->d_err,
-                     (const double*)b->d_em, (const FinalOut*)L->d_out, b->h_status);
+                     (const double*)b->d_em, (const FinalOut*)L->d_out,
+                     (const uint32_t*)(b->tail_spec ? b->d_tail : nullptr), b->h_status);
   HIP_TRY(hipGetLastError());
   HIP_TRY(hipStreamSynchronize(s));
   const uint64_t* h = b->h_status;
@@ -2028,6 +2101,110 @@
   if (st != BQSR_OK) return st;
   if (!L->out.any_key) return fail(BQSR_ERR_EMPTY_TABLE, "empty.reduceLeft: no usable base was observed");
   return from_err_key(std::min(h[kErrAppPrep], h[kErrAppKern]), 0);
+}
+
+int32_t bqsr_job_tail_path(const bqsr_batch* b) {
+  if (!b || !b->h_status || !b->tail_spec) return 0;
+  return b->h_status[kErrWords + 1 + sizeof(FinalOut) / 8] ? 2 : 1;
+}
+
+bqsr_status bqsr_job_tail_async(bqsr_context* ctx, bqsr_batch* b, const bqsr_sites* sites, bqsr_table* t,
+                                bqsr_lut** lut, uint8_t* out_qual, uint32_t* out_start, uint32_t* out_len,
+                                uint64_t* exceptions, int64_t max_exceptions, void* stream) {
+  if (!ctx || !b || !t || !lut || !out_qual || !out_start || !out_len) return fail(BQSR_ERR_INVALID_ARG, "null");
+  const bool spec = ctx->tune_spec_tail != 0 && !b->bucketed && b->rd.n_reads > 0 && b->tail_fork;
+  b->tail_spec = false;
+  if (!spec) {
+    bqsr_status st = bqsr_observe_stage(ctx, b, sites, t, BQSR_STAGE_FOLD, stream);
+    if (st == BQSR_OK) st = bqsr_finalize_device(ctx, t, b->d_em, lut, stream);
+    if (st == BQSR_OK)
+      st = bqsr_apply_stage(ctx, b, *lut, out_qual, out_start, out_len, exceptions, max_exceptions, BQSR_STAGE_KERNEL, stream);
+    return st;
+  }
+  bqsr_status st = check_dims(b, t);
+  if (st != BQSR_OK) return st;
+  if (!b->prepped || b->prep_sites != sites)
+    return fail(BQSR_ERR_INVALID_ARG, "job tail before the prep and observe stages (or with other known sites)");
+  HIP_TRY(hipSetDevice(ctx->device));
+  hipStream_t s = S(stream);
+  b->tail_fork = false;
+  if (!b->d_tail && ((st = dalloc(b->allocs, &b->d_tail, kTailWords)) != BQSR_OK ||
+                     (st = dalloc(b->allocs, &b->d_em_spec, 1)) != BQSR_OK))
+    return st;
+  const TableGeom g = geom(t->dims);
+  const int n_rg = t->dims.n_rg;
+  bqsr_lut* L = nullptr;
+  bool fresh = false;
+  if ((st = lut_for(ctx, t, lut, s, &L, &fresh)) != BQSR_OK) return st;
+  *lut = L;
+  if (!L->a2s && ((st = dalloc(L->allocs, &L->a2s, (size_t)n_rg * kQBins)) != BQSR_OK ||
+                  (st = dalloc(L->allocs, &L->s1s, (size_t)n_rg * kQBins * g.C)) != BQSR_OK ||
+                  (st = dalloc(L->allocs, &L->d2s, (size_t)n_rg * kQBins * kCtxSlots)) != BQSR_OK))
+    return st;
+  ApplyParams P{};
+  if ((st = apply_params(ctx, b, L, out_qual, out_start, out_len, exceptions, max_exceptions, stream, &P)) != BQSR_OK) return st;
+  const int cw = window_cw(b, P.g);
+  const int rb_words = b->n_base * 4;
+  P.qmask = b->d_qmask;
+
+  HIP_TRY(hipStreamWaitEvent(b->side, b->ev_obs, 0));
+  const FoldParams F = fold_params(ctx, b, false);
+  hipLaunchKernelGGL(bqsr_fold_plan, dim3(1), dim3(1024), 0, b->side, F);
+  const int64_t max_tpb = (b->rd.n_tiles + b->n_blocks - 1) / b->n_blocks + 1;
+  hipLaunchKernelGGL(bqsr_fold_tiles, dim3(ctx->n_cu * 4), dim3(kFtWaves * 64), 0, b->side, F, max_tpb);
+  HIP_TRY(hipEventRecord(b->ev_tiles, b->side));
+  hipLaunchKernelGGL(bqsr_fold_segs, dim3(b->n_blocks), dim3(kSegThreads), 0, b->side, F);
+  hipLaunchKernelGGL(bqsr_fold_chain, dim3(1), dim3(1024), chain_lds(b->n_blocks), b->side, F);
+  HIP_TRY(hipGetLastError());
+  HIP_TRY(hipEventRecord(b->ev_fold, b->side));
+  b->hq_valid = true;
+
+  const int mode = ctx->tune_spec_tail;
+  hipLaunchKernelGGL(bqsr_tail_estimate, dim3(1), dim3(1024), 0, s, (const uint32_t*)b->d_hq, b->n_blocks,
+                     (const double*)ctx->d_pow10, mode == 3 ? 1.5 : 1.0, b->d_em_spec, b->d_qmask, b->d_tail, P.rowbad,
+                     2 * rb_words);
+  hipLaunchKernelGGL(bqsr_final_keys, dim3((g.K + 3) / 4), dim3(256), 0, s, t->touched(), t->obs(), t->mm(), g, L->qk_obs,
+                     L->qk_mm);
+  const int64_t ncell = (int64_t)n_rg * kQBins * (g.C + kCtxSlots);
+  const unsigned tb = (unsigned)std::min<int64_t>(8192, (ncell + 255) / 256);
+  const double mre = pow10tab().v[kMaxQ];
+  hipLaunchKernelGGL(bqsr_final_groups, dim3(1), dim3(256), 0, s, t->touched(), L->qk_obs, L->qk_mm, g, n_rg, 0.0,
+                     (const double*)b->d_em_spec, ctx->d_pow10, L->n_groups, L->grp_obs, L->grp_mm, L->grp_ok, L->key_ok,
+                     L->a2s, L->rq_ok, L->d_out);
+  hipLaunchKernelGGL(bqsr_final_tables, dim3(tb), dim3(256), 0, s, t->obs(), t->mm(), g, n_rg, L->a2s, L->rq_ok, mre,
+                     L->s1s, L->d2s);
+  const size_t chars_n = (size_t)P.piece_stride * (size_t)b->n_base + (size_t)b->n_base * 16;
+  const unsigned cb = (unsigned)std::min<int64_t>(((int64_t)chars_n + 255) / 256, (int64_t)ctx->n_cu * 16);
+  ApplyParams Ps = P;
+  Ps.s1 = L->s1s;
+  Ps.d2 = L->d2s;
+  hipLaunchKernelGGL(bqsr_apply_chars, dim3(cb), dim3(256), 0, s, Ps, b->d_chars);
+  b->chars_lut = nullptr;
+  HIP_TRY(hipGetLastError());
+  HIP_TRY(hipStreamWaitEvent(s, b->ev_tiles, 0));
+  const int grid = std::max(1, b->pass_blocks() - ctx->tune_spec_reserve);
+  hipLaunchKernelGGL(bqsr_apply_kernel, dim3(grid), dim3(kBlockThreads), apply_lds(P.w.qw, cw), s, Ps);
+  HIP_TRY(hipGetLastError());
+
+  HIP_TRY(hipStreamWaitEvent(s, b->ev_fold, 0));
+  hipLaunchKernelGGL(bqsr_final_groups, dim3(1), dim3(256), 0, s, t->touched(), L->qk_obs, L->qk_mm, g, n_rg, 0.0,
+                     (const double*)b->d_em, ctx->d_pow10, L->n_groups, L->grp_obs, L->grp_mm, L->grp_ok, L->key_ok, L->a2,
+                     L->rq_ok, L->d_out);
+  hipLaunchKernelGGL(bqsr_final_tables, dim3(tb), dim3(256), 0, s, t->obs(), t->mm(), g, n_rg, L->a2, L->rq_ok, mre, L->s1,
+                     L->d2);
+  hipLaunchKernelGGL(bqsr_tail_compare, dim3((unsigned)(n_rg * kQBins)), dim3(256), 0, s, P, (const double*)L->a2,
+                     (const double*)L->a2s, (const double*)L->s1s, (const double*)L->d2s, mode == 2 ? 1 : 0, b->d_tail);
+  ApplyParams Pr = P;
+  Pr.run_if = b->d_tail + kTailRedo;
+  Pr.rowbad = P.rowbad + rb_words;
+  Pr.redo_mark = b->d_tail + kTailRan;
+  hipLaunchKernelGGL(bqsr_redo_chars, dim3(cb), dim3(256), 0, s, Pr, b->d_chars);
+  hipLaunchKernelGGL(bqsr_redo_apply, dim3(b->pass_blocks()), dim3(kBlockThreads), apply_lds(P.w.qw, cw), s, Pr);
+  hipError_t e = hipGetLastError();
+  if (e != hipSuccess) return fail(BQSR_ERR_DEVICE, hipGetErrorString(e));
+  L->out_pending = true;
+  b->tail_spec = true;
+  return ok();
 }
 
 }
diff --git a/adam_amd/csrc/bqsr_internal.h b/adam_amd/csrc/bqsr_internal.h
--- a/adam_amd/csrc/bqsr_internal.h
+++ b/adam_amd/csrc/bqsr_internal.h
@@ -255,7 +255,10 @@
   int64_t piece_stride;
   uint32_t* rowbad;
   const uint32_t* qmask;
-};
+  const uint32_t* run_if;
+  uint32_t* redo_mark;
+};
+enum { kTailRedo = 0, kTailRan = 1, kTailWords = 2 };
 
 struct FinalOut {
   int64_t g_obs, g_mm;
@@ -263,7 +266,7 @@
   int32_t any_key;
   int32_t pad;
 };
-static_assert(kErrWords + 1 + sizeof(FinalOut) / 8 <= (size_t)kJobStatusWords, "job status words overflow");
+static_assert(kErrWords + 2 + sizeof(FinalOut) / 8 <= (size_t)kJobStatusWords, "job status words overflow");
 static_assert(sizeof(FinalOut) % 8 == 0, "FinalOut is whole words");
 
 constexpr int kThrQmin = -3100;
diff --git a/adam_amd/csrc/bqsr_kernels.hip b/adam_amd/csrc/bqsr_kernels.hip
--- a/adam_amd/csrc/bqsr_kernels.hip
+++ b/adam_amd/csrc/bqsr_kernels.hip
@@ -2130,7 +2130,7 @@
   }
 }
 
-extern "C" __global__ void bqsr_apply_chars(ApplyParams P, uint8_t* chars) {
+__device__ __forceinline__ void apply_chars_body(const ApplyParams& P, uint8_t* chars) {
   const int nk = order_base_keys(P.ord), qw = P.w.qw, q_lo = P.w.q_lo;
   const int64_t total = (int64_t)nk * P.piece_stride;
   for (int64_t t = blockIdx.x * (int64_t)blockDim.x + threadIdx.x; t < total; t += (int64_t)gridDim.x * blockDim.x) {
@@ -2158,7 +2158,7 @@
   }
 }
 
-extern "C" __global__ void __launch_bounds__(kBlockThreads) bqsr_apply_kernel(ApplyParams P) {
+__device__ __forceinline__ void apply_body(const ApplyParams& P) {
   extern __shared__ __align__(16) unsigned char smem[];
   const int qw = P.w.qw, C = P.g.C, L = P.g.L;
   uint32_t* clean_rows = (uint32_t*)smem;
@@ -2244,6 +2244,21 @@
     }
   }
 }
+extern "C" __global__ void bqsr_apply_chars(ApplyParams P, uint8_t* chars) { apply_chars_body(P, chars); }
+extern "C" __global__ void __launch_bounds__(kBlockThreads) bqsr_apply_kernel(ApplyParams P) { apply_body(P); }
+extern "C" __global__ void bqsr_redo_chars(ApplyParams P, uint8_t* chars) {
+  if (!*P.run_if) return;
+  if (blockIdx.x == 0 && threadIdx.x == 0) {
+    *P.err = kNoError;
+    *P.n_exc = 0ull;
+    *P.redo_mark = 1u;
+  }
+  apply_chars_body(P, chars);
+}
+extern "C" __global__ void __launch_bounds__(kBlockThreads) bqsr_redo_apply(ApplyParams P) {
+  if (!*P.run_if) return;
+  apply_body(P);
+}
 
 
 extern "C" __global__ void bqsr_em_fold(const double* ems, int64_t n, double* out) {
@@ -2259,11 +2274,69 @@
   if (blockIdx.x == 0 && threadIdx.x < kErrWords) err[threadIdx.x] = threadIdx.x == kNExc ? 0ull : ~0ull;
 }
 extern "C" __global__ void bqsr_job_status_kernel(const unsigned long long* err, const double* em, const FinalOut* fo,
-                                                  uint64_t* host) {
+                                                  const uint32_t* tail, uint64_t* host) {
   const int t = threadIdx.x;
   if (t < kErrWords) host[t] = err[t];
   else if (t == kErrWords) host[t] = (uint64_t)__double_as_longlong(*em);
   else if (t < kErrWords + 1 + (int)(sizeof(FinalOut) / 8)) host[t] = ((const uint64_t*)fo)[t - kErrWords - 1];
+  else if (t == kErrWords + 1 + (int)(sizeof(FinalOut) / 8)) host[t] = tail ? tail[kTailRan] : 0u;
+}
+
+
+extern "C" __global__ void __launch_bounds__(1024) bqsr_tail_estimate(const uint32_t* hq_block, int32_t n_blocks,
+                                                                       const double* pow10, double scale,
+                                                                       double* em_spec, uint32_t* qmask, uint32_t* tail,
+                                                                       uint32_t* rowbad, int32_t rowbad_words) {
+  __shared__ unsigned long long cnt[32][kQBins + 4];
+  __shared__ double wsum[16];
+  const int tid = threadIdx.x, part = tid & 31, row0 = tid >> 5;
+  unsigned long long c[4] = {0, 0, 0, 0};
+  for (int b = row0; b < n_blocks; b += 32) {
+    const uint4 v = *(const uint4*)(hq_block + (int64_t)b * kQBins + part * 4);
+    c[0] += v.x;
+    c[1] += v.y;
+    c[2] += v.z;
+    c[3] += v.w;
+  }
+#pragma unroll
+  for (int i = 0; i < 4; ++i) cnt[row0][part * 4 + i] = c[i];
+  if (tid < kTailWords) tail[tid] = 0u;
+  for (int i = tid; i < rowbad_words; i += blockDim.x) rowbad[i] = 0u;
+  __syncthreads();
+  double v = 0.0;
+  bool used = false;
+  if (tid < kQBins) {
+    unsigned long long n = 0;
+    for (int r = 0; r < 32; ++r) n += cnt[r][tid];
+    used = n != 0;
+    v = (double)n * pow10[tid];
+  }
+  const uint64_t um = __builtin_amdgcn_ballot_w64(used);
+  if (tid < kQBins && (tid & 63) == 0) {
+    qmask[tid >> 5] = (uint32_t)um;
+    qmask[(tid >> 5) + 1] = (uint32_t)(um >> 32);
+  }
+  for (int off = 32; off > 0; off >>= 1) v += __shfl_xor(v, off);
+  if ((tid & 63) == 0) wsum[tid >> 6] = v;
+  __syncthreads();
+  if (tid == 0) *em_spec = (wsum[0] + wsum[1]) * scale;
+}
+
+extern "C" __global__ void __launch_bounds__(256) bqsr_tail_compare(ApplyParams P, const double* a2, const double* a2s,
+                                                                     const double* s1s, const double* d2s, int32_t force,
+                                                                     uint32_t* tail) {
+  const int64_t rq = blockIdx.x;
+  if (force && rq == 0 && threadIdx.x == 0) atomicOr(&tail[kTailRedo], 1u);
+  if (!P.rq_ok[rq] || __double_as_longlong(a2[rq]) == __double_as_longlong(a2s[rq])) return;
+  const int C = P.g.C;
+  bool diff = false;
+  for (int i = threadIdx.x; i < C * kCtxSlots; i += blockDim.x) {
+    const int c = i / kCtxSlots, x = i - c * kCtxSlots;
+    const int32_t qa = phred_q(P.s1[rq * C + c] + P.d2[rq * kCtxSlots + x], P.qb_thr, P.qb_q, P.thr, P.thr_qmin, P.thr_n);
+    const int32_t qb = phred_q(s1s[rq * C + c] + d2s[rq * kCtxSlots + x], P.qb_thr, P.qb_q, P.thr, P.thr_qmin, P.thr_n);
+    diff |= qa != qb;
+  }
+  if (__builtin_amdgcn_ballot_w64(diff) && (threadIdx.x & 63) == 0) atomicOr(&tail[kTailRedo], 1u);
 }
 
 extern "C" __global__ void bqsr_job_err_export(const unsigned long long* err, int64_t read_base, int64_t* out) {
diff --git a/adam_amd/job.py b/adam_amd/job.py
--- a/adam_amd/job.py
+++ b/adam_amd/job.py
@@ -61,6 +61,7 @@
         self.ev = [torch.cuda.Event(enable_timing=True) for _ in range(6)]
         self.kt: Dict[str, List[float]] = {k: [] for k in self.STAGES}
         self.n_exc = 0
+        self.tail_path = 0
         self.em = None
         torch.cuda.synchronize(self.dev)
 
@@ -89,8 +90,36 @@
         mark(5)
         check(L.bqsr_observe_stage(ctx, bh, self.sites_h, th, _capi.STAGE_PREP, sp))
         mark(0)
-        check(L.bqsr_observe_stage(ctx, bh, self.sites_h, th, _capi.STAGE_KERNEL, sp))
+        tail = not record and self.world == 1
+        check(L.bqsr_observe_stage(ctx, bh, self.sites_h, th, _capi.STAGE_KERNEL | (_capi.STAGE_FORK if tail else 0), sp))
         mark(1)
+        args = (self._ptr(self.out_qual), self._ptr(self.out_start), self._ptr(self.out_len), self._ptr(self.exc),
+                self.max_exc)
+        if tail:
+            self.em = None
+            check(L.bqsr_job_tail_async(ctx, bh, self.sites_h, th, ctypes.byref(self.lut), *args, sp))
+        else:
+            self._serial_tail(record, mark, args)
+        if self.world > 1:
+            check(L.bqsr_job_errors_export_async(bh, self.read_base, self._ptr(self.err_keys), sp))
+            D.allreduce_error_keys(self.err_keys)
+            check(L.bqsr_job_errors_import_async(bh, self._ptr(self.err_keys), sp))
+        em = ctypes.c_double()
+        nexc = ctypes.c_int64()
+        st = L.bqsr_job_result(bh, self.lut, ctypes.byref(em), ctypes.byref(nexc), sp)
+        self.tail_path = int(L.bqsr_job_tail_path(bh))
+        check(st)
+        self.n_exc = int(nexc.value)
+        if self.n_exc > self.max_exc:
+            raise _capi.BQSRError(_capi.UNSUPPORTED, "%d chars above 0xFF exceed the exception list" % self.n_exc)
+        if record:
+            self.kt["prep"].append(ev[5].elapsed_time(ev[0]))
+            self.kt["observe"].append(ev[0].elapsed_time(ev[1]))
+            self.kt["fold"].append(ev[1].elapsed_time(ev[2]))
+            self.kt["apply"].append(ev[3].elapsed_time(ev[4]))
+
+    def _serial_tail(self, record, mark, outs):
+        L, ctx, bh, th, sp, stream = self.L, self.ctx.handle, self.bh, self.th, self.sp, self.stream
         check(L.bqsr_observe_stage(ctx, bh, self.sites_h, th, _capi.STAGE_FOLD, sp))
         mark(2)
         if self.world > 1:
@@ -102,8 +131,7 @@
             self.em = None
             em_ptr = ctypes.c_void_p(L.bqsr_batch_em_device_ptr(bh))
         check(L.bqsr_finalize_device(ctx, th, em_ptr, ctypes.byref(self.lut), sp))
-        args = (ctx, bh, self.lut, self._ptr(self.out_qual), self._ptr(self.out_start), self._ptr(self.out_len),
-                self._ptr(self.exc), self.max_exc)
+        args = (ctx, bh, self.lut) + outs
         if record:
             check(L.bqsr_apply_stage(*args, _capi.STAGE_LUT, sp))
             mark(3)
@@ -111,21 +139,6 @@
             mark(4)
         else:
             check(L.bqsr_apply_stage(*args, _capi.STAGE_KERNEL, sp))
-        if self.world > 1:
-            check(L.bqsr_job_errors_export_async(bh, self.read_base, self._ptr(self.err_keys), sp))
-            D.allreduce_error_keys(self.err_keys)
-            check(L.bqsr_job_errors_import_async(bh, self._ptr(self.err_keys), sp))
-        em = ctypes.c_double()
-        nexc = ctypes.c_int64()
-        check(L.bqsr_job_result(bh, self.lut, ctypes.byref(em), ctypes.byref(nexc), sp))
-        self.n_exc = int(nexc.value)
-        if self.n_exc > self.max_exc:
-            raise _capi.BQSRError(_capi.UNSUPPORTED, "%d chars above 0xFF exceed the exception list" % self.n_exc)
-        if record:
-            self.kt["prep"].append(ev[5].elapsed_time(ev[0]))
-            self.kt["observe"].append(ev[0].elapsed_time(ev[1]))
-            self.kt["fold"].append(ev[1].elapsed_time(ev[2]))
-            self.kt["apply"].append(ev[3].elapsed_time(ev[4]))
 
     def kernel_ms(self) -> Dict[str, float]:
         return {k: float(np.mean(v)) if v else float("nan") for k, v in self.kt.items()}
diff --git a/include/adam_bqsr.h b/include/adam_bqsr.h
--- a/include/adam_bqsr.h
+++ b/include/adam_bqsr.h
@@ -95,7 +95,9 @@
   BQSR_TUNE_FUSED_PREP = 4,
   BQSR_TUNE_BGZF = 5,
   BQSR_TUNE_FLAGSTAT_GRID = 6,
-  BQSR_TUNE_PILEUP_GRID = 7
+  BQSR_TUNE_PILEUP_GRID = 7,
+  BQSR_TUNE_SPEC_TAIL = 8,
+  BQSR_TUNE_SPEC_RESERVE = 9
 };
 bqsr_status bqsr_context_tune(bqsr_context* ctx, int knob, int64_t value);
 
@@ -170,7 +172,7 @@
                                uint16_t* out_qual, uint32_t* out_len);
 
 enum { BQSR_STAGE_RESET = 1, BQSR_STAGE_KERNEL = 2, BQSR_STAGE_FOLD = 4, BQSR_STAGE_PREP = 8,
-       BQSR_STAGE_LUT = 16, BQSR_STAGE_NO_LUT = 32 };
+       BQSR_STAGE_LUT = 16, BQSR_STAGE_NO_LUT = 32, BQSR_STAGE_FORK = 64 };
 bqsr_status bqsr_observe_stage(bqsr_context* ctx, bqsr_batch* b, const bqsr_sites* sites, bqsr_table* t,
                                int32_t stages, void* stream);
 bqsr_status bqsr_observe_async(bqsr_context* ctx, bqsr_batch* b, const bqsr_sites* sites, bqsr_table* t,
@@ -219,6 +221,7 @@
 bqsr_status bqsr_batch_fold_stats(bqsr_batch* b, bqsr_fold_stats* out, void* stream);
 int64_t bqsr_batch_slots(const bqsr_batch* b);
 int bqsr_lut_group(const bqsr_lut* l, int32_t r, int64_t* obs, int64_t* mm);
+bqsr_status bqsr_lut_tables(const bqsr_lut* l, double* a2, double* s1, double* d2);
 int32_t bqsr_phred_threshold_table(double* out, int32_t cap, int32_t* qmin);
 
 bqsr_status bqsr_copy_async(bqsr_context* ctx, void* dst, const void* src, int64_t bytes, void* stream);
@@ -233,6 +236,10 @@
 bqsr_status bqsr_job_reset_async(bqsr_batch* b, bqsr_table* t, void* stream);
 bqsr_status bqsr_job_result(bqsr_batch* b, bqsr_lut* l, double* expected_mismatch, int64_t* n_exceptions,
                             void* stream);
+bqsr_status bqsr_job_tail_async(bqsr_context* ctx, bqsr_batch* b, const bqsr_sites* sites, bqsr_table* t,
+                                bqsr_lut** lut, uint8_t* out_qual, uint32_t* out_start, uint32_t* out_len,
+                                uint64_t* exceptions, int64_t max_exceptions, void* stream);
+int32_t bqsr_job_tail_path(const bqsr_batch* b);
 bqsr_status bqsr_job_status_async(bqsr_batch* b, bqsr_lut* l, int32_t slot, void* stream);
 bqsr_status bqsr_job_status_get(const bqsr_batch* b, int32_t slot, int32_t part, double* expected_mismatch,
                                 int64_t* n_exceptions);
```

New measurement: 537.5 billion bases/s, median of 6. +4.3%, better.
